# carpedkm/disentangled-subject-to-vid

Measured on AMD Instinct MI355X. Metric: denoise steps/sec (CogVideoX-5B, 49f 720x480; one step = CFG-pair transformer forward + CFG + scheduler step), higher is better.
Workload: dtype bf16

## Files before the change

### disentangled-subject-to-vid_amd/build.py

```python
import hashlib
import os
import subprocess
import sys

HERE = os.path.dirname(os.path.abspath(__file__))
CSRC = os.path.join(HERE, "csrc")
LIB = os.path.join(HERE, "libs2v_hip.so")
SOURCES = ["api.hip", "gemm.hip", "gemm_g4.hip", "gemm_g4t.hip", "gemm_g4f.hip", "gemm_f32m.hip", "attention.hip", "attention_f32m.hip", "attention_q4.hip", "elementwise.hip", "vae.hip", "vae_api.hip", "t5.hip", "rccl.hip", "ulysses.hip"]
FLAGS = ["--offload-arch=gfx950", "-O3", "-std=c++17", "-fPIC", "-fvisibility=hidden", "-Wno-unused-result", "-Wno-unused-value", "-Wno-inline-asm"]
EXTRA = {"attention_q4.hip": ["-fno-slp-vectorize"], "gemm_g4.hip": ["-fno-slp-vectorize"], "gemm_g4t.hip": ["-fno-slp-vectorize"], "gemm_g4f.hip": ["-fno-slp-vectorize"], "elementwise.hip": ["-ffp-contract=off", "-DS2V_TU_FP_CONTRACT_OFF"], "vae.hip": ["-ffp-contract=off", "-DS2V_TU_FP_CONTRACT_OFF"],
         "t5.hip": ["-ffp-contract=off", "-DS2V_TU_FP_CONTRACT_OFF"]}


def _stale(out, deps):
    if not os.path.exists(out):
        return True
    t = os.path.getmtime(out)
    return any(os.path.getmtime(d) > t for d in deps)


def _digest(paths, extra=()):
    h = hashlib.sha256()
    for e in extra:
        h.update(str(e).encode() + b"\0")
    for p in sorted(paths):
        h.update(os.path.basename(p).encode() + b"\0")
        with open(p, "rb") as f:
            h.update(f.read())
    return h.hexdigest()


def _read(path):
    try:
        with open(path) as f:
            return f.read().strip()
    except OSError:
        return None


DIAG_LIB = os.path.join(HERE, "libs2v_hip_diag.so")
GENERATORS = [("gen_attn_q4.py", ["attn_q4_body.inc", "attn_q4h_body.inc", "attn_q4f_body.inc", "attn_q4fh_body.inc", "attn_q4hh_body.inc", "attn_q8_body.inc", "attn_q4_regs.h"]),
              ("gen_gemm_g4.py", ["gemm_g4_body.inc", "gemm_g4_body_f16.inc", "gemm_g4_sk_sum.inc", "gemm_g4_regs.h"]),
              ("gen_gemm_g4t.py", ["gemm_g4t_body_gelu.inc", "gemm_g4t_body_bias.inc", "gemm_g4t_body_qknorm.inc", "gemm_g4t_regs.h"]),
              ("gen_gemm_g4f.py", ["gemm_g4f_body_a3.inc", "gemm_g4f_body_mx.inc", "gemm_g4f_regs.h"])]


def build_library(force=False, verbose=True, diag=False):
    force = force or os.environ.get("S2V_FORCE_BUILD", "0") == "1"
    hipcc = os.environ.get("HIPCC", "/opt/rocm/bin/hipcc")
    objdir = os.path.join(HERE, "build_diag" if diag else "build")
    LIB = DIAG_LIB if diag else globals()["LIB"]
    FLAGS = globals()["FLAGS"] + (["-DS2V_DIAG"] if diag else [])
    gens = GENERATORS
    headers = [os.path.join(CSRC, h) for h in sorted(os.listdir(CSRC)) if h.endswith((".h", ".inc"))]
    headers.append(os.path.join(HERE, "..", "include", "s2v_hip.h"))
    srcs = [os.path.join(CSRC, s) for s in SOURCES if os.path.exists(os.path.join(CSRC, s))]
    gen_srcs = [os.path.join(CSRC, g) for g, _ in gens]
    whole = _digest(srcs + headers + gen_srcs, FLAGS + [f"{k}:{v}" for k, v in sorted(EXTRA.items())])
    if not force and os.path.exists(LIB) and _read(LIB + ".stamp") == whole:
        if verbose:
            print(f"up to date (content hash {whole[:12]}): {LIB}", flush=True)
        return LIB
    os.makedirs(objdir, exist_ok=True)
    for g, outs in gens:
        gp, ops = os.path.join(CSRC, g), [os.path.join(CSRC, o) for o in outs]
        stamp = os.path.join(objdir, g + ".stamp")
        d = _digest([gp])
        missing = [o for o in ops if not os.path.exists(o)]
        if force or missing or (_read(stamp) != d and any(_stale(o, [gp]) for o in ops)):
            if verbose:
                print(f"{sys.executable} {gp}", flush=True)
            subprocess.check_call([sys.executable, gp])
            with open(stamp, "w") as f:
                f.write(d)
    headers = [os.path.join(CSRC, h) for h in sorted(os.listdir(CSRC)) if h.endswith((".h", ".inc"))]
    headers.append(os.path.join(HERE, "..", "include", "s2v_hip.h"))
    whole = _digest(srcs + headers + gen_srcs, FLAGS + [f"{k}:{v}" for k, v in sorted(EXTRA.items())])
    objs = []
    procs = []
    for sp in srcs:
        src = os.path.basename(sp)
        obj = os.path.join(objdir, src.replace(".hip", ".o"))
        objs.append(obj)
        cmd = [hipcc] + FLAGS + EXTRA.get(src, []) + ["-c", sp, "-o", obj]
        d = _digest([sp] + headers, cmd[1:-3])
        if force or not os.path.exists(obj) or _read(obj + ".stamp") != d:
            if verbose:
                print(" ".join(cmd), flush=True)
            procs.append((src, obj, d, subprocess.Popen(cmd)))
    for src, obj, d, p in procs:
        if p.wait() != 0:
            raise RuntimeError(f"hipcc failed on {src}")
        with open(obj + ".stamp", "w") as f:
            f.write(d)
    cmd = [hipcc, "--offload-arch=gfx950", "-shared", "-fPIC", "-o", LIB] + objs
    if verbose:
        print(" ".join(cmd), flush=True)
    subprocess.check_call(cmd)
    with open(LIB + ".stamp", "w") as f:
        f.write(whole)
    if verbose:
        print(f"built {len(procs)} of {len(objs)} translation units, linked {LIB} (content hash {whole[:12]})", flush=True)
    return LIB


if __name__ == "__main__":
    print(build_library(force="--force" in sys.argv, diag="--diag" in sys.argv))
```

### disentangled-subject-to-vid_amd/csrc/api.hip

```cpp
#define S2V_HOST
#include "common.h"
#include "kernels.h"
#include "../../include/s2v_hip.h"

#include <algorithm>
#include <cstdio>
#include <cstring>
#include <string>
#include <unordered_map>
#include <vector>

thread_local std::string g_s2v_err;
int s2v_fail(const char* file, int line, const char* msg, int code) {
    char buf[512];
    snprintf(buf, sizeof(buf), "%s:%d: %s", file, line, msg);
    g_s2v_err = buf;
    return code;
}

static inline int64_t rup(int64_t x, int64_t m) { return (x + m - 1) / m * m; }

struct Slot {
    char* dst = nullptr;
    int64_t rows = 0, cols = 0, ld = 0;
// ... 457 lines not shown
        std::string m = std::string("s2v_weight_slot: unknown tensor name: ") + name;
        return s2v_fail(__FILE__, __LINE__, m.c_str(), -3);
    }
    const Slot& s = it->second;
    *offset_bytes = (int64_t)(s.dst - c->arena);
    *rows = s.rows; *cols = s.cols; *ld = s.ld;
    return 0;
}

extern "C" int s2v_weight_arena(s2v_ctx* c, void** dev_ptr, int64_t* bytes) {
    S2V_REQUIRE(c && dev_ptr && bytes, "s2v_weight_arena: null argument");
    *dev_ptr = c->arena;
    *bytes = c->arena_bytes;
    return 0;
}
extern "C" int s2v_mark_weights_loaded(s2v_ctx* c) {
    S2V_REQUIRE(c, "null context");
    S2V_REQUIRE(c->kind != S2V_CTX_ATTN_WORKSPACE, "s2v_mark_weights_loaded: a workspace context (S2V_CTX_ATTN_WORKSPACE) holds no weights");
    for (auto& kv : c->slots) kv.second.loaded = true;
    c->finalized = true;
    return 0;
}

static inline void shard_range(int n, int p, int r, int* begin, int* len) {
    const int b = (int)((int64_t)r * n / p), e = (int)((int64_t)(r + 1) * n / p);
    *begin = b; *len = e - b;
}

extern "C" int s2v_set_shard(s2v_ctx* c, int32_t world, int32_t rank) {
    S2V_REQUIRE(c, "null context");
    S2V_REQUIRE(c->kind == S2V_CTX_MODEL, "s2v_set_shard: attention-only contexts (S2V_CTX_ATTN_*) are not sharded");
    S2V_REQUIRE(world >= 1 && rank >= 0 && rank < world, "s2v_set_shard: need world >= 1 and 0 <= rank < world");
    S2V_REQUIRE(c->cfg.num_heads % world == 0, "s2v_set_shard: the world size must divide num_heads (attention runs num_heads / world heads per rank)");
    S2V_REQUIRE(c->cfg.weight_format == 0 || (c->D / world) % 128 == 0,
                "s2v_set_shard: fp8 weight formats need an even number of heads per rank, (inner_dim / world) % 128 == 0 (the MX block-scale dwords of "
                "the attention output hold two heads each)");
    S2V_REQUIRE(c->cfg.out_channels * 4 * c->esz % 16 == 0, "s2v_set_shard: the projected rows must be a multiple of 16 bytes (out_channels * 4 * element size)");
    if (c->shard && c->sp == world && c->sr == rank) return 0;
    S2V_CHECK_HIP(hipDeviceSynchronize());
    if (c->gexec) { hipGraphExecDestroy(c->gexec); c->gexec = nullptr; }
    if (c->ws) { hipFree(c->ws); c->ws = nullptr; }
    c->B = 0;
    c->shard = true; c->sp = world; c->sr = rank;
    c->sh_pending = 0;
    return 0;
}

static bool attn_mx_out(const s2v_ctx* c);

extern "C" int s2v_set_geometry(s2v_ctx* c, int32_t B, int32_t T, int32_t F, int32_t H, int32_t W) {
    S2V_REQUIRE(c, "null context");
    S2V_REQUIRE(c->kind != S2V_CTX_ATTN_WEIGHTS, "s2v_set_geometry: an attention-weights context (S2V_CTX_ATTN_WEIGHTS) never carves a workspace");
    S2V_REQUIRE(B >= 1 && B <= 4, "s2v_set_geometry: batch must be 1..4");
    S2V_REQUIRE(T >= 0 && F >= 1 && H >= 2 && W >= 2 && H % 2 == 0 && W % 2 == 0, "s2v_set_geometry: bad geometry");
    if (c->ws && B == c->B && T == c->gT && F == c->F && H == c->H && W == c->W) return 0;
    if (c->shard) S2V_REQUIRE(F * (H / 2) * (W / 2) >= c->sp, "s2v_set_geometry: every rank of a shard needs at least one video row");
    S2V_CHECK_HIP(hipDeviceSynchronize());
    if (c->gexec) { hipGraphExecDestroy(c->gexec); c->gexec = nullptr; }
    if (c->ws) { hipFree(c->ws); c->ws = nullptr; }
    c->B = B; c->T = T; c->F = F; c->H = H; c->W = W;
    c->R = (H / 2) * (W / 2);
    c->V = F * c->R;
    c->Ntok = T + c->R + c->V;
    c->gT = c->T; c->gR = c->R; c->gV = c->V; c->gN = c->Ntok;
    c->t0 = c->r0 = c->v0 = 0;
    if (c->shard) {
        shard_range(c->gT, c->sp, c->sr, &c->t0, &c->T);
        shard_range(c->gR, c->sp, c->sr, &c->r0, &c->R);
        shard_range(c->gV, c->sp, c->sr, &c->v0, &c->V);
        c->Ntok = c->T + c->R + c->V;
    }
    c->Vmax = (c->gV + c->sp - 1) / c->sp;
    c->sh_pending = 0;
    c->fp8_qk = c->cfg.weight_format == 2 || (c->cfg.weight_format == 3 && c->gN >= S2V_FP8_QK_AUTO_TOKENS);
    c->ntok_pad = (int)rup(c->gN, 64);
    c->M = (int64_t)B * c->Ntok;
    c->Mpad = rup(c->M, 256) + 256;
    c->have_rope = c->have_pos = c->have_cond = false;
    c->split_kind = -1;
    const int64_t D = c->D, E = c->esz;
    const int64_t Cin4 = c->cfg.in_channels * 4, Cout4 = c->cfg.out_channels * 4;
    const int64_t BVp = rup((int64_t)B * c->V, 256) + 256;
    const int64_t BVg = rup((int64_t)B * c->gV, 256) + 256;
    int64_t off = 0;
    auto carve = [&](int64_t bytes) { int64_t o = off; off += rup(bytes, 256); return o; };
    const int64_t oX = carve(c->Mpad * D * E), oXn = carve(c->Mpad * D * E), oQKV = carve(c->Mpad * 3 * D * E);
    const int64_t oH = carve(c->Mpad * 4 * D * E);
    const int64_t oVT = carve((int64_t)B * (c->cfg.num_heads / c->sp) * 64 * c->ntok_pad * 2);
    const int64_t oe0 = carve(rup((int64_t)B * T + 128, 128) * D * E), oe1 = carve(rup(c->gR + 128, 128) * D * E);
    const int64_t opat = carve(BVg * Cin4 * E), otail = carve(BVp * D * E), oproj = carve(BVp * Cout4 * E);
    const int64_t omod = carve((int64_t)B * c->mod_rows * E);
    const int64_t ote = carve(((int64_t)B * D + (int64_t)B * c->temb) * E), oemb = carve((int64_t)B * c->temb * E);
    const int64_t onp = carve((int64_t)std::max(B, 2) * F * c->cfg.out_channels * H * W * E);
    const int64_t ocos = carve((int64_t)(c->R + c->V) * 64 * 4), osin = carve((int64_t)(c->R + c->V) * 64 * 4);
    const int64_t opk = carve((int64_t)(c->R + c->V) * 64 * 4);
    const int64_t opos = carve((int64_t)c->V * D * E);
    const int64_t oaq = carve(c->fp8 ? c->Mpad * 4 * D : 0), oaqs = carve(c->fp8 ? c->Mpad * 4 : 0);
    const int64_t ohq = carve(c->fp8 ? c->Mpad * 4 * D : 0), ohs = carve(c->fp8 ? c->Mpad * 4 * D / 32 : 0);
    const int64_t BH = (int64_t)B * (c->cfg.num_heads / c->sp);
    const int64_t oq8 = carve(c->fp8_qk ? BH * c->gN * 64 : 0), oq8s = carve(c->fp8_qk ? BH * c->gN * 2 : 0);
    const int64_t ok8 = carve(c->fp8_qk ? BH * c->ntok_pad * 64 : 0), ok8s = carve(c->fp8_qk ? BH * c->ntok_pad * 4 : 0);
    c->sk_tiles = (!c->shard && c->mfma && ((c->M + 255) / 256) * ((D + 255) / 256) * 2 <= c->num_cus) ? c->num_cus : 0;
    const int64_t osk = carve((int64_t)c->sk_tiles * 262144), oskc = carve((int64_t)c->sk_tiles * 4);
    const int64_t P = c->sp, Dp = D / P, Mg = (int64_t)B * c->gN, Mgpad = rup(Mg, 256) + 256;
    c->o_mx = c->shard && attn_mx_out(c);
    const bool omx = c->o_mx;
    auto o_bytes = [&](int64_t n) { return omx ? n * Dp + rup(n * Dp / 32, 16) : n * Dp * E; };
    const int64_t oQh = carve(c->shard ? Mgpad * 3 * Dp * E : 0), oOh = carve(c->shard ? Mgpad * Dp * E : 0);
    const int64_t osb = carve(c->shard ? std::max(c->M * 3 * D * E, o_bytes(Mg) + 16 * P) : 0);
    const int64_t orb = carve(c->shard ? std::max(Mg * 3 * Dp * E, P * o_bytes(c->M)) : 0);
    const int64_t oOs = carve(omx ? Dp / 128 * Mgpad * 4 : 0), oomap = carve(omx ? 2 * Mg * 4 : 0);
    const int64_t ons = carve(c->shard ? (int64_t)B * c->Vmax * Cout4 * E : 0), onr = carve(c->shard ? P * B * c->Vmax * Cout4 * E : 0);
    const int64_t opf = carve(c->shard ? (int64_t)B * c->gV * Cout4 * E : 0);
    const int64_t ormap = carve(c->shard ? Mg * 4 : 0), onmap = carve(c->shard ? P * B * c->Vmax * 4 : 0);
    c->ws_bytes = off;
    S2V_CHECK_HIP(hipMalloc((void**)&c->ws, c->ws_bytes));
    S2V_CHECK_HIP(hipMemset(c->ws, 0, c->ws_bytes));
    char* w = c->ws;
    c->X = w + oX; c->Xn = w + oXn; c->QKV = w + oQKV; c->Hb = w + oH; c->VT = w + oVT; c->e0 = w + oe0; c->e1 = w + oe1;
    c->patches = w + opat; c->tailn = w + otail; c->proj = w + oproj; c->mod = w + omod; c->tmp_te = w + ote;
    c->emb = w + oemb; c->noise_pred = w + onp; c->rope_cos = (float*)(w + ocos); c->rope_sin = (float*)(w + osin);
    c->pos_tab = w + opos; c->rope_pk = (float*)(w + opk); c->rope_paired = false;
    c->aq = w + oaq; c->aq_scale = (float*)(w + oaqs);
    c->hq = (unsigned char*)(w + ohq); c->hs = (unsigned char*)(w + ohs);
    c->q8 = (unsigned char*)(w + oq8); c->q8s = (unsigned short*)(w + oq8s); c->k8 = (unsigned char*)(w + ok8); c->k8s = (unsigned*)(w + ok8s);
    c->sk_ws = (float*)(w + osk); c->sk_cnt = (unsigned*)(w + oskc);
    if (c->shard) {
        c->QKVh = w + oQh; c->Oh = w + oOh; c->sbuf = w + osb; c->rbuf = w + orb; c->nsend = w + ons; c->nrecv = w + onr; c->proj_full = w + opf;
        c->rmap = (int*)(w + ormap); c->nmap = (int*)(w + onmap);
        c->Os = omx ? (unsigned char*)(w + oOs) : nullptr; c->Os_rows = Mgpad; c->omap = omx ? (int*)(w + oomap) : nullptr;
        std::vector<int> rmap, nmap;
        rmap.reserve(Mg);
        nmap.assign((size_t)P * B * c->Vmax, -1);
        std::vector<int64_t> ntok(P);
        for (int g = 0; g < P; ++g) {
            int ts, tl, rs, rl, vs, vl;
            shard_range(c->gT, (int)P, g, &ts, &tl); shard_range(c->gR, (int)P, g, &rs, &rl); shard_range(c->gV, (int)P, g, &vs, &vl);
            ntok[g] = tl + rl + vl;
            for (int b = 0; b < B; ++b) {
                const int base = b * c->gN;
                for (int i = 0; i < tl; ++i) rmap.push_back(base + ts + i);
                for (int i = 0; i < rl; ++i) rmap.push_back(base + c->gT + rs + i);
                for (int i = 0; i < vl; ++i) rmap.push_back(base + c->gT + c->gR + vs + i);
                for (int i = 0; i < vl; ++i) nmap[((size_t)g * B + b) * c->Vmax + i] = b * c->gV + vs + i;
            }
        }
        S2V_CHECK_HIP(hipMemcpy(c->rmap, rmap.data(), rmap.size() * 4, hipMemcpyHostToDevice));
        S2V_CHECK_HIP(hipMemcpy(c->nmap, nmap.data(), nmap.size() * 4, hipMemcpyHostToDevice));
        for (auto& k : c->xcnt) for (auto& v : k) v.assign(P, 0);
        int64_t rq = 0, so = 0;
        std::vector<int> omap(omx ? 2 * Mg : 0);
        for (int g = 0, i = 0; g < P; ++g) {
            c->xcnt[0][0][g] = c->M * 3 * Dp * E; c->xcnt[0][1][g] = g * c->M * 3 * Dp * E;
            c->xcnt[0][2][g] = B * ntok[g] * 3 * Dp * E; c->xcnt[0][3][g] = rq; rq += c->xcnt[0][2][g];
            const int64_t n = B * ntok[g];
            if (omx)
                for (int64_t j = 0; j < n; ++j, ++i) { omap[i] = (int)((so + j * Dp) / 16); omap[Mg + i] = (int)((so + n * Dp) / 4 + j * (Dp / 128)); }
            c->xcnt[1][0][g] = o_bytes(n); c->xcnt[1][1][g] = so; so += c->xcnt[1][0][g];
            c->xcnt[1][2][g] = o_bytes(c->M); c->xcnt[1][3][g] = g * o_bytes(c->M);
            c->xcnt[2][0][g] = (int64_t)B * c->Vmax * Cout4 * E; c->xcnt[2][1][g] = 0;
            c->xcnt[2][2][g] = c->xcnt[2][0][g]; c->xcnt[2][3][g] = g * c->xcnt[2][0][g];
        }
        if (omx) S2V_CHECK_HIP(hipMemcpy(c->omap, omap.data(), omap.size() * 4, hipMemcpyHostToDevice));
    }
    return 0;
}

extern "C" int s2v_fp8_qk_active(s2v_ctx* c, int32_t* active) {
    S2V_REQUIRE(c && active, "s2v_fp8_qk_active: null argument");
    *active = c->fp8_qk ? 1 : 0;
    return 0;
}

extern "C" int s2v_set_rope(s2v_ctx* c, const float* cos_dev, const float* sin_dev, s2v_stream stream) {
    S2V_REQUIRE(c && c->ws, "s2v_set_rope: call s2v_set_geometry first");
    auto drop_graph = [&]() { if (c->gexec) { hipGraphExecDestroy(c->gexec); c->gexec = nullptr; } };
    if (!cos_dev || !sin_dev) {
        if (c->have_rope) drop_graph();
        c->have_rope = false;
        return 0;
    }
    const bool had_rope = c->have_rope, was_paired = c->rope_paired;
    const size_t bytes = (size_t)(c->R + c->V) * 64 * 4;
    if (c->shard) {
        const size_t row = 64 * 4, rb = (size_t)c->R * row, vb = (size_t)c->V * row;
        const size_t ro = (size_t)c->r0 * row, vo = ((size_t)c->gR + c->v0) * row;
        S2V_CHECK_HIP(hipMemcpyAsync(c->rope_cos, (const char*)cos_dev + ro, rb, hipMemcpyDeviceToDevice, (hipStream_t)stream));
        S2V_CHECK_HIP(hipMemcpyAsync(c->rope_sin, (const char*)sin_dev + ro, rb, hipMemcpyDeviceToDevice, (hipStream_t)stream));
        S2V_CHECK_HIP(hipMemcpyAsync((char*)c->rope_cos + rb, (const char*)cos_dev + vo, vb, hipMemcpyDeviceToDevice, (hipStream_t)stream));
        S2V_CHECK_HIP(hipMemcpyAsync((char*)c->rope_sin + rb, (const char*)sin_dev + vo, vb, hipMemcpyDeviceToDevice, (hipStream_t)stream));
    } else {
        S2V_CHECK_HIP(hipMemcpyAsync(c->rope_cos, cos_dev, bytes, hipMemcpyDeviceToDevice, (hipStream_t)stream));
        S2V_CHECK_HIP(hipMemcpyAsync(c->rope_sin, sin_dev, bytes, hipMemcpyDeviceToDevice, (hipStream_t)stream));
    }
    c->have_rope = true;
    const size_t n = (size_t)(c->R + c->V) * 64;
    std::vector<float> hc(n), hs(n), pk(n);
    S2V_CHECK_HIP(hipStreamSynchronize((hipStream_t)stream));
    S2V_CHECK_HIP(hipMemcpy(hc.data(), c->rope_cos, bytes, hipMemcpyDeviceToHost));
    S2V_CHECK_HIP(hipMemcpy(hs.data(), c->rope_sin, bytes, hipMemcpyDeviceToHost));
    bool paired = true;
    for (size_t i = 0; i < n && paired; i += 2) paired = hc[i] == hc[i + 1] && hs[i] == hs[i + 1];
    c->rope_paired = paired;
    if (!had_rope || was_paired != paired) drop_graph();
    if (paired) {
        for (size_t p = 0; p < n / 64; ++p)
            for (int k = 0; k < 32; ++k) {
                pk[p * 64 + k] = hc[p * 64 + 2 * k];
                pk[p * 64 + 32 + k] = hs[p * 64 + 2 * k];
            }
        S2V_CHECK_HIP(hipMemcpy(c->rope_pk, pk.data(), bytes, hipMemcpyHostToDevice));
    }
    return 0;
}

extern "C" int s2v_set_pos_embed(s2v_ctx* c, const void* table_dev, s2v_stream stream) {
    S2V_REQUIRE(c && c->ws, "s2v_set_pos_embed: call s2v_set_geometry first");
    if (!table_dev) { c->have_pos = false; return 0; }
    S2V_CHECK_HIP(hipMemcpyAsync(c->pos_tab, (const char*)table_dev + (size_t)c->v0 * c->D * c->esz, (size_t)c->V * c->D * c->esz,
                                 hipMemcpyDeviceToDevice, (hipStream_t)stream));
    c->have_pos = true;
    return 0;
}

static int linear(s2v_ctx* c, const GemmArgs& g0, int epi, hipStream_t st) {
    GemmArgs g = g0;
    g.clk = c->clk_cur;
    g.a_rows_padded = (int)(rup(g.M, 256));
    g.w_rows_padded = (int)(rup(g.N, 256));
    if ((c->mfma || c->h16) && g.K % 64 == 0 && g.lda % 8 == 0 && g.ldw % 8 == 0) {
        g.f16 = c->h16 ? 1 : 0;
        const GemmPlan p = gemm_plan(g, epi, c->num_cus, c->sk_tiles);
        g.tile = p.tile;
        if (p.splitk > 1) { g.splitk = p.splitk; g.sk_ws = c->sk_ws; g.sk_cnt = c->sk_cnt; }
        if (p.tail != GEMM_NONE) {
            GemmArgs gm = g, gt = g;
            gt.clk = nullptr;
            gm.M = p.m_main;
            gt.m_begin = p.m_main;
            S2V_CHECK_HIP(hipEventRecord(c->ev_fork, st));
            S2V_CHECK_HIP(hipStreamWaitEvent(c->side, c->ev_fork, 0));
            S2V_TRY(launch_gemm_bf16(gt, epi, c->side));
            S2V_CHECK_HIP(hipEventRecord(c->ev_join, c->side));
            S2V_TRY(launch_gemm_bf16(gm, epi, st));
            S2V_CHECK_HIP(hipStreamWaitEvent(st, c->ev_join, 0));
            return 0;
        }
        return launch_gemm_bf16(g, epi, st);
    }
    g.valu_only = c->cfg.force_simple;
    return launch_gemm_simple(g, epi, c->dtype, st);
}

static int linear_fp8(s2v_ctx* c, const GemmArgs& g0, int epi, const char* wq, const float* wscale, hipStream_t st, bool prequant = false) {
    GemmArgs g = g0;
    g.clk = c->clk_cur;
    g.a_scale = nullptr;
    if (!g.mx_a_s) {
        if (!prequant) S2V_TRY(launch_quant_rows_fp8(g.A, g.lda, g.M, g.K, c->aq, c->aq_scale, st));
        g.A = c->aq; g.a_scale = c->aq_scale;
    }
    g.lda = g.K; g.W = wq; g.ldw = g.K; g.w_scale = wscale;
    g.a_rows_padded = (int)rup(g.M, 256);
    g.w_rows_padded = (int)rup(g.N, 256);
    return launch_gemm_fp8(g, epi, st);
}

extern "C" int s2v_set_conditioning(s2v_ctx* c, const void* text_dev, const void* ref_latent_dev, s2v_stream stream) {
    S2V_REQUIRE(c && c->ws && c->finalized, "s2v_set_conditioning: geometry and weights must be set first");
    S2V_REQUIRE(text_dev && ref_latent_dev, "s2v_set_conditioning: null input");
    hipStream_t st = (hipStream_t)stream;
    const int D = c->D;
    const int TX = c->cfg.text_embed_dim;
    if (c->T > 0) {
        if (c->shard) {
            for (int b = 0; b < c->B; ++b)
                S2V_TRY(launch_convert2d((const char*)text_dev + ((int64_t)b * c->gT + c->t0) * TX * c->esz, c->dtype, TX,
                                         c->Hb + (int64_t)b * c->T * TX * c->esz, c->dtype, TX, c->T, TX, st));
        } else {
            S2V_TRY(launch_convert2d(text_dev, c->dtype, TX, c->Hb, c->dtype, TX, (int64_t)c->B * c->T, TX, st));
        }
        GemmArgs g{};
        g.A = c->Hb; g.lda = TX; g.W = c->text_w; g.ldw = TX; g.bias = c->text_b;
        g.C = c->e0; g.ldc = D; g.M = c->B * c->T; g.N = D; g.K = TX;
        S2V_TRY(linear(c, g, EPI_BIAS, st));
    }
    const int K = c->cfg.in_channels * 4;
    S2V_TRY(launch_patchify(ref_latent_dev, 0, 1, 1, c->cfg.in_channels, c->H, c->W, c->patches, c->dtype, st));
    GemmArgs g{};
    g.A = c->patches + (int64_t)c->r0 * K * c->esz; g.lda = K; g.W = c->patch_w; g.ldw = K; g.bias = c->patch_b;
    g.C = c->e1; g.ldc = D; g.M = c->R; g.N = D; g.K = K;
    if (c->R > 0) S2V_TRY(linear(c, g, EPI_BIAS, st));
    c->have_cond = true;
    return 0;
}

#ifdef S2V_DIAG
static int g_fp8_mx = 1;
extern "C" __attribute__((visibility("default"))) int s2v_set_fp8_mx(int on) { g_fp8_mx = on; return 0; }
static int g_fused_q8 = 1;
extern "C" __attribute__((visibility("default"))) int s2v_set_fused_q8(int on) { g_fused_q8 = on; return 0; }
static int g_fused_qk = 1;
extern "C" __attribute__((visibility("default"))) int s2v_set_fused_qk(int on) { g_fused_qk = on; return 0; }
extern "C" __attribute__((visibility("default"))) int s2v_diag_qkv_qknorm(const void* A, const void* W, const void* bias, const void* nq_w, const void* nq_b,
                                                                           const void* nk_w, const void* nk_b, const float* cs, void* C, int32_t M, int32_t D,
                                                                           int32_t K, int32_t tok_per_batch, int32_t text_len, float eps, s2v_stream stream) {
    S2V_REQUIRE(A && W && bias && C && nq_w && nq_b && nk_w && nk_b, "s2v_diag_qkv_qknorm: null argument");
    GemmArgs g{};
    g.A = A; g.lda = K; g.W = W; g.ldw = K; g.bias = bias; g.C = C; g.ldc = 3 * D; g.M = M; g.N = 3 * D; g.K = K;
    g.a_rows_padded = (int)rup(M, 256); g.w_rows_padded = (int)rup(3 * D, 256);
    g.tok_per_batch = tok_per_batch; g.text_len = text_len;
    g.qk_w[0] = nq_w; g.qk_b[0] = nq_b; g.qk_w[1] = nk_w; g.qk_b[1] = nk_b; g.qk_cs = cs; g.qk_D = D; g.qk_eps = eps;
    return launch_gemm_bf16(g, EPI_BIAS_QKNORM, (hipStream_t)stream);
}
#endif
static bool attn_mx_out(const s2v_ctx* c) {
    bool mx = c->fp8 && c->mfma && c->D % 128 == 0;
#ifdef S2V_DIAG
    mx = mx && g_fp8_mx;
#endif
    return mx;
}
static int run_attention(s2v_ctx* c, const LayerW& w, hipStream_t st, bool prequant = false) {
    const int D = c->D;
    GemmArgs g{};
    g.A = c->Xn; g.lda = D; g.W = w.wqkv; g.ldw = D; g.bias = w.bqkv;
    g.C = c->QKV; g.ldc = 3 * D; g.M = (int)c->M; g.N = 3 * D; g.K = D;
#ifdef S2V_DIAG
    const bool fuse_any = (c->mfma || c->h16) && D % 64 == 0 && (!c->have_rope || c->rope_paired) && g_fused_qk != 0;
    const bool norm_in_quant = fuse_any && c->fp8_qk && g_fused_qk != 3;
#else
    const bool fuse_any = (c->mfma || c->h16) && D % 64 == 0 && (!c->have_rope || c->rope_paired);
    const bool norm_in_quant = fuse_any && c->fp8_qk;
#endif
    const bool fused_qk = fuse_any && !norm_in_quant;
    if (fused_qk) {
        g.tok_per_batch = c->Ntok; g.text_len = c->T;
        g.qk_w[0] = w.nq_w; g.qk_b[0] = w.nq_b; g.qk_w[1] = w.nk_w; g.qk_b[1] = w.nk_b;
        g.qk_cs = c->have_rope ? c->rope_pk : nullptr;
        g.qk_D = D; g.qk_eps = 1e-6f;
    }
    {
        ProfScope ps(c, PK_QKV, st);
        const int epi = fused_qk ? EPI_BIAS_QKNORM : EPI_BIAS;
        if (c->fp8) S2V_TRY(linear_fp8(c, g, epi, w.q_qkv, w.s_qkv, st, prequant));
        else S2V_TRY(linear(c, g, epi, st));
    }
    const bool p16 = c->attn_p16 && c->mfma && (c->fp8_qk || attn_runs_q4(c->Ntok, attn_mx_out(c)));
    if (fused_qk || norm_in_quant) {
        ProfScope ps(c, PK_QKNORM, st);
        S2V_TRY(launch_v_transpose(c->QKV, 3 * D, c->B, c->cfg.num_heads, c->Ntok, c->VT, c->ntok_pad, st, p16));
    } else {
        QkNormRopeArgs q{};
        q.qkv = c->QKV; q.ld_qkv = 3 * D; q.B = c->B; q.H = c->cfg.num_heads; q.Ntok = c->Ntok; q.text_len = c->T;
        q.nq_w = w.nq_w; q.nq_b = w.nq_b; q.nk_w = w.nk_w; q.nk_b = w.nk_b; q.eps = 1e-6f;
        q.cos = c->have_rope ? c->rope_cos : nullptr; q.sin = c->have_rope ? c->rope_sin : nullptr;
        q.vt = (c->mfma || c->h16) ? c->VT : nullptr; q.ntok_pad = c->ntok_pad; q.vt_f16 = p16 ? 1 : 0;
        ProfScope ps(c, PK_QKNORM, st);
        S2V_TRY(launch_qk_norm_rope(q, c->dtype, st));
    }
    AttnArgs a{};
    a.qkv = c->QKV; a.ld_qkv = 3 * D; a.vt = c->VT; a.ntok_pad = c->ntok_pad; a.out = c->Xn; a.ld_out = D;
    a.B = c->B; a.H = c->cfg.num_heads; a.Ntok = c->Ntok; a.scale = 0.125f;
    a.queue = c->attn_queue; a.num_cus = c->num_cus;
    a.p16 = p16 ? 1 : 0;
    a.stats = c->attn_stats;
    a.valu_only = c->cfg.force_simple;
    a.stagger = c->attn_stagger;
    a.order = c->attn_order;
    if (attn_mx_out(c)) { a.mx_q = (unsigned char*)c->aq; a.mx_s = c->hs; a.mx_rows = (int)c->Mpad; }
    if (c->fp8_qk) {
        {
            ProfScope ps(c, PK_QKNORM, st);
            if (norm_in_quant) {
                QkNormRopeArgs q{};
                q.qkv = c->QKV; q.ld_qkv = 3 * D; q.B = c->B; q.H = c->cfg.num_heads; q.Ntok = c->Ntok; q.text_len = c->T; q.ntok_pad = c->ntok_pad;
                q.nq_w = w.nq_w; q.nq_b = w.nq_b; q.nk_w = w.nk_w; q.nk_b = w.nk_b; q.eps = 1e-6f;
                q.cos = c->have_rope ? c->rope_cos : nullptr; q.sin = c->have_rope ? c->rope_sin : nullptr;
                S2V_TRY(launch_qk_norm_quant_mx(q, a.scale * 1.4426950408889634f, c->q8, c->q8s, c->k8, c->k8s, st));
            } else {
                S2V_TRY(launch_qk_quant_mx(c->QKV, 3 * D, c->B, c->cfg.num_heads, c->Ntok, c->ntok_pad, a.scale * 1.4426950408889634f, c->q8, c->q8s, c->k8,
                                           c->k8s, st));
            }
        }
        a.q8 = c->q8; a.q8s = c->q8s; a.k8 = c->k8; a.k8s = c->k8s;
        ProfScope ps(c, PK_ATTN, st);
        a.clk = c->clk_cur;
        return launch_attn_q4f(a, true, st);
    }
    ProfScope ps(c, PK_ATTN, st);
    a.clk = c->clk_cur;
    if (c->mfma) S2V_TRY(launch_attn_bf16(a, st));
    else if (c->h16) S2V_TRY(launch_attn_f16(a, st));
    else S2V_TRY(launch_attn_simple(a, c->dtype, st));
    return 0;
}

static int block_norm(s2v_ctx* c, int l, int half, const char* mod_base , int64_t mod_stride,
                      hipStream_t st, bool* prequant_out) {
    const LayerW& w = c->layers[l];
    const int D = c->D;
    const int64_t E = c->esz;
    const char* mb = mod_base + (int64_t)half * c->mc * D * E;
    LnModArgs n{};
    n.x = c->X; n.ldx = D; n.y = c->Xn; n.ldy = D;
    n.w = half ? w.ln2_w : w.ln1_w; n.b = half ? w.ln2_b : w.ln1_b; n.eps = c->cfg.norm_eps;
    n.shift_vid = mb; n.scale_vid = mb + D * E; n.shift_txt = mb + 3 * D * E; n.scale_txt = mb + 4 * D * E;
    n.mod_stride = (int)mod_stride; n.B = c->B; n.Ntok = c->Ntok; n.text_len = c->T; n.D = D;
    if (c->mc == 9) { n.shift_ref = mb + 6 * D * E; n.scale_ref = mb + 7 * D * E; n.ref_len = c->R; }
    bool prequant = c->fp8;
#ifdef S2V_DIAG
    prequant = prequant && g_fused_q8;
#endif
    if (prequant) { n.q8 = c->aq; n.q8_scale = c->aq_scale; }
    *prequant_out = prequant;
    ProfScope ps(c, PK_LNMOD, st);
    return launch_ln_modulate(n, c->dtype, st);
}

static GemmArgs block_gate(const s2v_ctx* c, int half, const char* mod_base, int64_t mod_stride) {
    const int D = c->D;
    const int64_t E = c->esz;
    const char* mb = mod_base + (int64_t)half * c->mc * D * E;
    GemmArgs g{};
    g.X = c->X; g.ldx = D; g.gate_vid = mb + 2 * D * E; g.gate_txt = mb + 5 * D * E; g.gate_stride = (int)mod_stride;
    g.tok_per_batch = c->Ntok; g.text_len = c->T; g.M = (int)c->M; g.N = D;
    if (c->mc == 9) { g.gate_ref = mb + 8 * D * E; g.ref_len = c->R; }
    return g;
}

static int block_out_proj(s2v_ctx* c, int l, GemmArgs g, hipStream_t st) {
    const LayerW& w = c->layers[l];
    const int D = c->D;
    g.A = c->Xn; g.lda = D; g.W = w.wo; g.ldw = D; g.bias = w.bo; g.K = D;
    if (attn_mx_out(c)) { g.A = c->aq; g.mx_a_s = c->hs; g.mx_rows = (int)c->Mpad; }
    ProfScope ps(c, PK_OUT, st);
    if (c->fp8) return linear_fp8(c, g, EPI_BIAS_GATE_RES, w.q_o, w.s_o, st);
    return linear(c, g, EPI_BIAS_GATE_RES, st);
}

static int block_ff(s2v_ctx* c, int l, GemmArgs g, bool prequant, hipStream_t st) {
    const LayerW& w = c->layers[l];
    const int D = c->D;
    GemmArgs f{};
    f.A = c->Xn; f.lda = D; f.W = w.w1; f.ldw = D; f.bias = w.b1; f.C = c->Hb; f.ldc = 4 * D;
    f.M = (int)c->M; f.N = 4 * D; f.K = D;
    bool mx = c->fp8 && (4 * D) % 128 == 0;
#ifdef S2V_DIAG
    mx = mx && g_fp8_mx;
#endif
    if (mx) { f.mx_out_q = c->hq; f.mx_out_s = c->hs; f.mx_rows = (int)c->Mpad; }
    {
        ProfScope ps(c, PK_FF1, st);
        if (c->fp8) S2V_TRY(linear_fp8(c, f, EPI_BIAS_GELU, w.q_1, w.s_1, st, prequant));
        else S2V_TRY(linear(c, f, EPI_BIAS_GELU, st));
    }
    g.A = c->Hb; g.lda = 4 * D; g.W = w.w2; g.ldw = 4 * D; g.bias = w.b2; g.K = 4 * D;
    if (mx) { g.A = c->hq; g.mx_a_s = c->hs; g.mx_rows = (int)c->Mpad; }
    ProfScope ps(c, PK_FF2, st);
    if (c->fp8) return linear_fp8(c, g, EPI_BIAS_GATE_RES, w.q_2, w.s_2, st);
    return linear(c, g, EPI_BIAS_GATE_RES, st);
}

static int run_block(s2v_ctx* c, int l, const char* mod_base ,
                     int64_t mod_stride, hipStream_t st) {
    for (int half = 0; half < 2; ++half) {
        bool prequant = false;
        S2V_TRY(block_norm(c, l, half, mod_base, mod_stride, st, &prequant));
        const GemmArgs g = block_gate(c, half, mod_base, mod_stride);
        if (half == 0) {
            S2V_TRY(run_attention(c, c->layers[l], st, prequant));
            S2V_TRY(block_out_proj(c, l, g, st));
        } else {
            S2V_TRY(block_ff(c, l, g, prequant, st));
        }
    }
    return 0;
}

static int embed_streams(s2v_ctx* c, const void* latents, int64_t lat_bstride, const float* t_dev, hipStream_t st) {
    const int D = c->D, B = c->B;
    const int64_t E = c->esz;
    S2V_TRY(launch_time_embed(t_dev, B, D, c->te1_w, c->te1_b, c->te2_w, c->te2_b, c->temb, c->tmp_te, c->emb, c->dtype, st));
    {
        ProfScope ps(c, PK_OTHER, st);
        S2V_TRY(launch_mod_gemv(c->emb, B, c->temb, c->mod_w, c->mod_b, c->mod_rows, c->mod, c->dtype, st));
    }
    const int K = c->cfg.in_channels * 4;
    S2V_TRY(launch_patchify(latents, lat_bstride, B, c->F, c->cfg.in_channels, c->H, c->W, c->patches, c->dtype, st));
    for (int b = 0; b < B; ++b) {
        char* xb = c->X + (int64_t)b * c->Ntok * D * E;
        S2V_TRY(launch_copy_rows(c->e0 + (int64_t)b * c->T * D * E, D, nullptr, 0, xb, D, c->T, D, c->dtype, st));
        S2V_TRY(launch_copy_rows(c->e1, D, nullptr, 0, xb + (int64_t)c->T * D * E, D, c->R, D, c->dtype, st));
        char* xv = xb + (int64_t)(c->T + c->R) * D * E;
        GemmArgs g{};
        g.A = c->patches + ((int64_t)b * c->gV + c->v0) * K * E; g.lda = K; g.W = c->patch_w; g.ldw = K; g.bias = c->patch_b;
        g.C = xv; g.ldc = D; g.M = c->V; g.N = D; g.K = K;
        S2V_TRY(linear(c, g, EPI_BIAS, st));
        if (!c->cfg.use_rope) S2V_TRY(launch_copy_rows(xv, D, c->pos_tab, D, xv, D, c->V, D, c->dtype, st));
    }
    return 0;
}

static int tail_proj(s2v_ctx* c, hipStream_t st) {
    const int D = c->D, B = c->B;
    const int64_t E = c->esz;
    const char* mo = c->mod + (int64_t)2 * c->L * c->mc * D * E;
    TailNormArgs t{};
    t.x = c->X; t.ldx = D; t.y = c->tailn; t.ldy = D; t.w1 = c->nf_w; t.b1 = c->nf_b; t.w2 = c->no_w; t.b2 = c->no_b;
    t.eps = c->cfg.norm_eps; t.shift = mo; t.scale = mo + D * E; t.mod_stride = (int)c->mod_rows;
    t.B = B; t.Ntok = c->Ntok; t.row0 = c->T + c->R; t.V = c->V; t.D = D;
    S2V_TRY(launch_tail_norm(t, c->dtype, st));
    const int Co = c->cfg.out_channels * 4;
    GemmArgs g{};
    g.A = c->tailn; g.lda = D; g.W = c->po_w; g.ldw = D; g.bias = c->po_b; g.C = c->proj; g.ldc = Co;
    g.M = B * c->V; g.N = Co; g.K = D;
    return linear(c, g, EPI_BIAS, st);
}

static int forward_impl(s2v_ctx* c, const void* latents, int64_t lat_bstride, const float* t_dev, void* out,
                        hipStream_t st) {
    S2V_REQUIRE(c->ws && c->finalized && c->have_cond, "transformer_forward: geometry, weights and conditioning required");
    S2V_REQUIRE(!c->cfg.use_rope || c->have_rope, "transformer_forward: RoPE tables missing (s2v_set_rope)");
    S2V_REQUIRE(c->cfg.use_rope || c->have_pos, "transformer_forward: sincos table missing (s2v_set_pos_embed)");
    S2V_REQUIRE(!c->shard, "transformer_forward: a shard context (s2v_set_shard) runs the staged step only (s2v_shard_step_* / s2v_denoise_step_ulysses)");
    const int D = c->D;
    const int64_t E = c->esz;
    S2V_TRY(embed_streams(c, latents, lat_bstride, t_dev, st));
    for (int l = 0; l < c->L; ++l)
        S2V_TRY(run_block(c, l, c->mod + (int64_t)(2 * l) * c->mc * D * E, c->mod_rows, st));
    S2V_TRY(tail_proj(c, st));
    const int Co = c->cfg.out_channels * 4;
    S2V_TRY(launch_unpatchify(c->proj, Co, c->V, out, c->B, c->F, c->cfg.out_channels, c->H, c->W, c->dtype, st));
    return 0;
}

extern "C" int s2v_transformer_forward(s2v_ctx* c, const void* latents, int64_t lat_bstride, const float* timesteps_dev,
                                       void* out, s2v_stream stream) {
    S2V_REQUIRE(c && latents && timesteps_dev && out, "s2v_transformer_forward: null argument");
    return forward_impl(c, latents, lat_bstride, timesteps_dev, out, (hipStream_t)stream);
}

extern "C" int s2v_block_forward(s2v_ctx* c, int32_t layer, const void* hidden, const void* enc0, const void* enc1,
                                 const void* temb, void* out_hidden, void* out_enc0, void* out_enc1, s2v_stream stream) {
    S2V_REQUIRE(c && c->ws && c->finalized, "s2v_block_forward: geometry and weights required");
    S2V_REQUIRE(!c->shard, "s2v_block_forward: a shard context (s2v_set_shard) runs the staged step only");
    S2V_REQUIRE(layer >= 0 && layer < c->L, "s2v_block_forward: bad layer");
    S2V_REQUIRE(hidden && enc1 && temb && out_hidden && out_enc1, "s2v_block_forward: null argument");
    hipStream_t st = (hipStream_t)stream;
    const int D = c->D, B = c->B;
    const int64_t E = c->esz;
    const int64_t r0 = (int64_t)(2 * layer) * c->mc * D;
    char* modl = c->mod;
    S2V_TRY(launch_mod_gemv(temb, B, c->temb, c->mod_w + r0 * c->temb * E, c->mod_b + r0 * E, 2 * c->mc * D, modl, c->dtype, st));
    for (int b = 0; b < B; ++b) {
        char* xb = c->X + (int64_t)b * c->Ntok * D * E;
        if (c->T) S2V_TRY(launch_copy_rows((const char*)enc0 + (int64_t)b * c->T * D * E, D, nullptr, 0, xb, D, c->T, D, c->dtype, st));
        S2V_TRY(launch_copy_rows((const char*)enc1 + (int64_t)b * c->R * D * E, D, nullptr, 0, xb + (int64_t)c->T * D * E, D, c->R, D, c->dtype, st));
        S2V_TRY(launch_copy_rows((const char*)hidden + (int64_t)b * c->V * D * E, D, nullptr, 0, xb + (int64_t)(c->T + c->R) * D * E, D, c->V, D, c->dtype, st));
    }
    S2V_TRY(run_block(c, layer, modl, 2 * c->mc * D, st));
    for (int b = 0; b < B; ++b) {
        const char* xb = c->X + (int64_t)b * c->Ntok * D * E;
        if (c->T) S2V_TRY(launch_copy_rows(xb, D, nullptr, 0, (char*)out_enc0 + (int64_t)b * c->T * D * E, D, c->T, D, c->dtype, st));
        S2V_TRY(launch_copy_rows(xb + (int64_t)c->T * D * E, D, nullptr, 0, (char*)out_enc1 + (int64_t)b * c->R * D * E, D, c->R, D, c->dtype, st));
        S2V_TRY(launch_copy_rows(xb + (int64_t)(c->T + c->R) * D * E, D, nullptr, 0, (char*)out_hidden + (int64_t)b * c->V * D * E, D, c->V, D, c->dtype, st));
    }
    return 0;
}

static int attn_forward_impl(s2v_ctx* c, const LayerW& w, const void* hidden, const void* encoder, void* out_hidden, void* out_encoder,
                             hipStream_t st) {
    const int D = c->D, B = c->B, TR = c->T + c->R;
    const int64_t E = c->esz;
    for (int b = 0; b < B; ++b) {
        char* xb = c->Xn + (int64_t)b * c->Ntok * D * E;
        S2V_TRY(launch_copy_rows((const char*)encoder + (int64_t)b * TR * D * E, D, nullptr, 0, xb, D, TR, D, c->dtype, st));
        S2V_TRY(launch_copy_rows((const char*)hidden + (int64_t)b * c->V * D * E, D, nullptr, 0, xb + (int64_t)TR * D * E, D, c->V, D, c->dtype, st));
    }
    S2V_TRY(run_attention(c, w, st));
    GemmArgs g{};
    g.A = c->Xn; g.lda = D; g.W = w.wo; g.ldw = D; g.bias = w.bo; g.C = c->Hb; g.ldc = D; g.M = (int)c->M; g.N = D; g.K = D;
    if (attn_mx_out(c)) { g.A = c->aq; g.mx_a_s = c->hs; g.mx_rows = (int)c->Mpad; }
    if (c->fp8) S2V_TRY(linear_fp8(c, g, EPI_BIAS, w.q_o, w.s_o, st));
    else S2V_TRY(linear(c, g, EPI_BIAS, st));
    for (int b = 0; b < B; ++b) {
        const char* xb = c->Hb + (int64_t)b * c->Ntok * D * E;
        S2V_TRY(launch_copy_rows(xb, D, nullptr, 0, (char*)out_encoder + (int64_t)b * TR * D * E, D, TR, D, c->dtype, st));
        S2V_TRY(launch_copy_rows(xb + (int64_t)TR * D * E, D, nullptr, 0, (char*)out_hidden + (int64_t)b * c->V * D * E, D, c->V, D, c->dtype, st));
    }
    return 0;
}

extern "C" int s2v_attn_forward(s2v_ctx* c, int32_t layer, const void* hidden, const void* encoder, void* out_hidden,
                                void* out_encoder, s2v_stream stream) {
    S2V_REQUIRE(c && c->ws && c->finalized, "s2v_attn_forward: geometry and weights required");
    S2V_REQUIRE(!c->shard, "s2v_attn_forward: a shard context (s2v_set_shard) runs the staged step only");
    S2V_REQUIRE(layer >= 0 && layer < c->L, "s2v_attn_forward: bad layer");
    S2V_REQUIRE(hidden && encoder && out_hidden && out_encoder, "s2v_attn_forward: null argument");
    return attn_forward_impl(c, c->layers[layer], hidden, encoder, out_hidden, out_encoder, (hipStream_t)stream);
}

extern "C" int s2v_attn_forward_with(s2v_ctx* c, const s2v_ctx* wc, int32_t layer, const void* hidden, const void* encoder, void* out_hidden,
                                     void* out_encoder, s2v_stream stream) {
    S2V_REQUIRE(c && wc, "s2v_attn_forward_with: null context");
    S2V_REQUIRE(c->ws, "s2v_attn_forward_with: the workspace context has no geometry (s2v_set_geometry)");
    S2V_REQUIRE(!c->shard && !wc->shard, "s2v_attn_forward_with: a shard context (s2v_set_shard) runs the staged step only");
    S2V_REQUIRE(wc->finalized && wc->kind != S2V_CTX_ATTN_WORKSPACE, "s2v_attn_forward_with: the weights are not loaded (s2v_finalize_weights)");
    S2V_REQUIRE(wc->dtype == c->dtype, "s2v_attn_forward_with: the weights context has another dtype");
    S2V_REQUIRE(wc->cfg.num_heads == c->cfg.num_heads && wc->D == c->D, "s2v_attn_forward_with: the weights context has another num_heads / inner dim");
    S2V_REQUIRE(wc->cfg.weight_format == c->cfg.weight_format, "s2v_attn_forward_with: the weights context has another weight_format");
    S2V_REQUIRE(layer >= 0 && layer < (int)wc->layers.size(), "s2v_attn_forward_with: bad layer");
    S2V_REQUIRE(hidden && encoder && out_hidden && out_encoder, "s2v_attn_forward_with: null argument");
    return attn_forward_impl(c, wc->layers[layer], hidden, encoder, out_hidden, out_encoder, (hipStream_t)stream);
}

// ... 644 lines not shown
```

### disentangled-subject-to-vid_amd/csrc/gemm_epi.h

```cpp
#pragma once
#include "common.h"
#include "kernels.h"
#include <type_traits>

#pragma clang fp contract(off)

template <typename T, int EPI>
__device__ __forceinline__ void epilogue4(const GemmArgs& a, int m, int n, const float v[4]) {
    if (m >= a.M) return;
    const T* bias = (const T*)a.bias;
    float y[4];
#pragma unroll
    for (int i = 0; i < 4; ++i) {
        float bv = (bias && n + i < a.N) ? ET<T>::ld(bias + n + i) : 0.f;
        y[i] = ET<T>::rnd(v[i] + bv);
    }
    if (EPI == EPI_BIAS_GELU) {
#pragma unroll
        for (int i = 0; i < 4; ++i) y[i] = ET<T>::rnd(gelu_tanh_f(y[i]));
    }
    if (EPI == EPI_BIAS_GATE_RES) {
        const int b = m / a.tok_per_batch;
        const int r = m - b * a.tok_per_batch;
        const void* gsel = r < a.text_len ? a.gate_txt : (a.gate_ref != nullptr && r < a.text_len + a.ref_len) ? a.gate_ref : a.gate_vid;
        const T* gate = (const T*)gsel + (size_t)b * a.gate_stride;
        T* x = (T*)a.X + (size_t)m * a.ldx + n;
#pragma unroll
        for (int i = 0; i < 4; ++i) {
            if (n + i < a.N) {
                float t = ET<T>::rnd(ET<T>::ld(gate + n + i) * y[i]);
                ET<T>::st(x + i, ET<T>::ld(x + i) + t);
            }
        }
        return;
    }
    if (EPI == EPI_BIAS_ADD) {
        const T* r = (const T*)a.R + (size_t)m * a.ldr + n;
#pragma unroll
        for (int i = 0; i < 4; ++i)
            if (n + i < a.N) y[i] = y[i] + ET<T>::ld(r + i);
    }
    T* c = (T*)a.C + (size_t)m * a.ldc + n;
    if (n + 3 < a.N && (a.ldc & 3) == 0) {
        if constexpr (std::is_same<T, bf16_t>::value) {
            u32x2 p;
            p.x = pack2bf(y[0], y[1]);
            p.y = pack2bf(y[2], y[3]);
            *(u32x2*)c = p;
        } else if constexpr (std::is_same<T, f16_t>::value) {
            u32x2 p;
            p.x = pack2h(y[0], y[1]);
            p.y = pack2h(y[2], y[3]);
            *(u32x2*)c = p;
        } else {
            *(f32x4*)c = (f32x4){y[0], y[1], y[2], y[3]};
        }
    } else {
#pragma unroll
        for (int i = 0; i < 4; ++i)
            if (n + i < a.N) ET<T>::st(c + i, y[i]);
    }
}

__device__ __forceinline__ float oct_sum(float v) {
    v += __int_as_float(__builtin_amdgcn_update_dpp(0, __float_as_int(v), 0xB1, 0xf, 0xf, true));
    v += __int_as_float(__builtin_amdgcn_update_dpp(0, __float_as_int(v), 0x4E, 0xf, 0xf, true));
    v += __int_as_float(__builtin_amdgcn_update_dpp(0, __float_as_int(v), 0x141, 0xf, 0xf, true));
    return v;
}

__device__ __forceinline__ void load_bias64(const GemmArgs& a, int nw, int hi, u32x2 (&bvec)[8]) {
    const bf16_t* bias = (const bf16_t*)a.bias;
    if (bias && nw + 64 <= a.N) {
#pragma unroll
        for (int q = 0; q < 8; ++q) bvec[q] = *(const u32x2*)(bias + nw + (q >> 2) * 32 + 8 * (q & 3) + 4 * hi);
    } else {
#pragma unroll
        for (int q = 0; q < 8; ++q) {
            const int nl = (q >> 2) * 32 + 8 * (q & 3) + 4 * hi;
            unsigned short t[4] = {0, 0, 0, 0};
#pragma unroll
            for (int e = 0; e < 4; ++e)
                if (bias && nw + nl + e < a.N) t[e] = ((const unsigned short*)bias)[nw + nl + e];
            bvec[q] = u32x2{(unsigned)t[0] | ((unsigned)t[1] << 16), (unsigned)t[2] | ((unsigned)t[3] << 16)};
        }
    }
}

template <typename T16> struct H2;
template <> struct H2<bf16_t> {
    static __device__ __forceinline__ float lo(unsigned w) { return __uint_as_float(w << 16); }
    static __device__ __forceinline__ float hi(unsigned w) { return __uint_as_float(w & 0xffff0000u); }
    static __device__ __forceinline__ unsigned pack(float a, float b) { return pack2bf(a, b); }
    static __device__ __forceinline__ float rnd(float v) { return bf2f(f2bf(v)); }
};
template <> struct H2<f16_t> {
    static __device__ __forceinline__ float lo(unsigned w) { return (float)__builtin_bit_cast(f16x2_t, w)[0]; }
    static __device__ __forceinline__ float hi(unsigned w) { return (float)__builtin_bit_cast(f16x2_t, w)[1]; }
    static __device__ __forceinline__ unsigned pack(float a, float b) { return pack2h(a, b); }
    static __device__ __forceinline__ float rnd(float v) { return (float)(f16_t)v; }
};
template <int EPI, int MB, bool SC = false, int GRP = 4, typename T16 = bf16_t>
__device__ __forceinline__ void epilogue_wave_b(const GemmArgs& a, const f32x16 (&acc)[2][MB], int mw, int nw, char* patch, int lane,
                                                const u32x2 (&bvec)[8]) {
    const int fr = lane & 31, hi = lane >> 5;
    const int c16 = lane & 7;
    const bool qk_head = EPI == EPI_BIAS_QKNORM && nw < 2 * a.qk_D;
    const bool qk_rot = qk_head && a.qk_cs != nullptr;
    float qw[8], qb[8];
    f32x4 rc[2][GRP], rs[2][GRP];
    bool rope[2][GRP];
    auto rot_load = [&](int it0, int buf) {
        const float inv_tok = 1.0f / (float)a.tok_per_batch;
#pragma unroll
        for (int u = 0; u < GRP; ++u) {
            const int m = min(mw + (it0 + u) * 8 + (lane >> 3), a.M - 1);
            int b = (int)((float)m * inv_tok);
            int r = m - b * a.tok_per_batch;
            if (r < 0) r += a.tok_per_batch;
            if (r >= a.tok_per_batch) r -= a.tok_per_batch;
            rope[buf][u] = qk_rot && r >= a.text_len;
            const float* tp = a.qk_cs + (size_t)(rope[buf][u] ? r - a.text_len : 0) * 64 + c16 * 4;
            if (qk_rot) {
                rc[buf][u] = *(const f32x4*)tp;
                rs[buf][u] = *(const f32x4*)(tp + 32);
            }
        }
    };
    if (EPI == EPI_BIAS_QKNORM) {
        const int which = nw >= a.qk_D;
        const u32x4 w4 = *(const u32x4*)((const bf16_t*)a.qk_w[which] + c16 * 8), b4 = *(const u32x4*)((const bf16_t*)a.qk_b[which] + c16 * 8);
#pragma unroll
        for (int e = 0; e < 4; ++e) {
            qw[2 * e] = H2<T16>::lo(w4[e]); qw[2 * e + 1] = H2<T16>::hi(w4[e]);
            qb[2 * e] = H2<T16>::lo(b4[e]); qb[2 * e + 1] = H2<T16>::hi(b4[e]);
        }
        rot_load(0, 0);
    }
    constexpr bool PRE = EPI == EPI_BIAS_ADD && MB == 2;
    u32x4 xpre[PRE ? MB * 4 : 1];
    if (PRE) {
        const int npre = nw + c16 * 8 < a.N ? nw + c16 * 8 : 0;
#pragma unroll
        for (int it = 0; it < MB * 4; ++it)
            xpre[it] = *(const u32x4*)((const bf16_t*)a.R + (size_t)min(mw + it * 8 + (lane >> 3), a.M - 1) * a.ldr + npre);
        __builtin_amdgcn_sched_barrier(0);
    }
    float sa[MB];
#pragma unroll
    for (int j = 0; j < MB; ++j) sa[j] = (SC && a.a_scale) ? a.a_scale[min(mw + j * 32 + fr, a.M - 1)] : 1.f;
#pragma unroll
    for (int i = 0; i < 2; ++i)
#pragma unroll
        for (int rq = 0; rq < 4; ++rq) {
            const int nl = i * 32 + 8 * rq + 4 * hi;
            const u32x2 bq = bvec[i * 4 + rq];
            f32x4 sw = {1.f, 1.f, 1.f, 1.f};
            if (SC) sw = *(const f32x4*)(a.w_scale + nw + nl);
            const float bv[4] = {H2<T16>::lo(bq.x), H2<T16>::hi(bq.x), H2<T16>::lo(bq.y),
                                 H2<T16>::hi(bq.y)};
#pragma unroll
            for (int j = 0; j < MB; ++j) {
                float y[4];
#pragma unroll
                for (int e = 0; e < 4; ++e) y[e] = (SC ? acc[i][j][rq * 4 + e] * (sa[j] * sw[e]) : acc[i][j][rq * 4 + e]) + bv[e];
                const int row = j * 32 + fr;
                u32x2 p;
                p.x = H2<T16>::pack(y[0], y[1]);
                p.y = H2<T16>::pack(y[2], y[3]);
                if (EPI == EPI_BIAS_GELU) {
                    p.x = H2<T16>::pack(gelu_tanh_fast(H2<T16>::lo(p.x)), gelu_tanh_fast(H2<T16>::hi(p.x)));
                    p.y = H2<T16>::pack(gelu_tanh_fast(H2<T16>::lo(p.y)), gelu_tanh_fast(H2<T16>::hi(p.y)));
                }
                *(u32x2*)(patch + row * 128 + ((((nl >> 3) ^ (row & 7))) << 4) + (nl & 4) * 2) = p;
            }
        }
    const int n = nw + c16 * 8;
    const bool n_ok = n < a.N;
    const int nc = n_ok ? n : 0;
#pragma unroll
    for (int it0 = 0; it0 < MB * 4; it0 += GRP) {
        u32x4 v[GRP], g[GRP], xo[GRP];
        int mrow[GRP];
        const int cur = (it0 / GRP) & 1;
        if (EPI == EPI_BIAS_QKNORM && it0 + GRP < MB * 4) rot_load(it0 + GRP, cur ^ 1);
#pragma unroll
        for (int u = 0; u < GRP; ++u) {
            const int row = (it0 + u) * 8 + (lane >> 3);
            mrow[u] = mw + row;
            v[u] = *(const u32x4*)(patch + row * 128 + ((c16 ^ (row & 7)) << 4));
            const int m = min(mrow[u], a.M - 1);
            if (EPI == EPI_BIAS_GATE_RES) {
                const int b = m / a.tok_per_batch;
                const int r = m - b * a.tok_per_batch;
                const void* gsel = r < a.text_len ? a.gate_txt : (a.gate_ref != nullptr && r < a.text_len + a.ref_len) ? a.gate_ref : a.gate_vid;
                g[u] = *(const u32x4*)((const bf16_t*)gsel + (size_t)b * a.gate_stride + nc);
                xo[u] = *(const u32x4*)((const bf16_t*)a.X + (size_t)m * a.ldx + nc);
            } else if (EPI == EPI_BIAS_ADD) {
                if (PRE) xo[u] = xpre[PRE ? it0 + u : 0];
                else xo[u] = *(const u32x4*)((const bf16_t*)a.R + (size_t)m * a.ldr + nc);
            }
        }
#pragma unroll
        for (int u = 0; u < GRP; ++u) {
            u32x4 o = v[u];
            if (EPI == EPI_BIAS_QKNORM && qk_head) {
                float x[8];
#pragma unroll
                for (int e = 0; e < 4; ++e) { x[2 * e] = H2<T16>::lo(v[u][e]); x[2 * e + 1] = H2<T16>::hi(v[u][e]); }
                float s = 0.f;
#pragma unroll
                for (int e = 0; e < 8; ++e) s += x[e];
                s = oct_sum(s);
                const float mean = s * (1.0f / 64.0f);
                float q = 0.f;
#pragma unroll
                for (int e = 0; e < 8; ++e) { const float d = x[e] - mean; q += d * d; }
                q = oct_sum(q);
                const float rstd = 1.0f / sqrtf(q * (1.0f / 64.0f) + a.qk_eps);
#pragma unroll
                for (int e = 0; e < 8; ++e) x[e] = H2<T16>::rnd(((x[e] - mean) * rstd * qw[e] + qb[e]));
                if (rope[cur][u]) {
#pragma unroll
                    for (int e = 0; e < 8; e += 2) {
                        const float x0 = x[e], x1 = x[e + 1];
                        const float cc = rc[cur][u][e >> 1], ss = rs[cur][u][e >> 1];
                        x[e] = H2<T16>::rnd((x0 * cc + (-x1) * ss));
                        x[e + 1] = H2<T16>::rnd((x1 * cc + x0 * ss));
                    }
                }
#pragma unroll
                for (int e = 0; e < 4; ++e) o[e] = H2<T16>::pack(x[2 * e], x[2 * e + 1]);
            }
            if (EPI == EPI_BIAS_GATE_RES) {
#pragma unroll
                for (int e = 0; e < 4; ++e) {
                    const float t0 = H2<T16>::rnd((H2<T16>::lo(g[u][e]) * H2<T16>::lo(v[u][e])));
                    const float t1 = H2<T16>::rnd((H2<T16>::hi(g[u][e]) * H2<T16>::hi(v[u][e])));
                    o[e] = H2<T16>::pack(H2<T16>::lo(xo[u][e]) + t0, H2<T16>::hi(xo[u][e]) + t1);
                }
            } else if (EPI == EPI_BIAS_ADD) {
#pragma unroll
                for (int e = 0; e < 4; ++e)
                    o[e] = H2<T16>::pack(H2<T16>::lo(v[u][e]) + H2<T16>::lo(xo[u][e]),
                                   H2<T16>::hi(v[u][e]) + H2<T16>::hi(xo[u][e]));
            }
            if (EPI == EPI_BIAS_GELU && a.mx_out_q) {
                typedef unsigned short u16x2_t __attribute__((ext_vector_type(2)));
                u16x2_t pm = __builtin_bit_cast(u16x2_t, o[0] & 0x7fff7fffu);
#pragma unroll
                for (int e = 1; e < 4; ++e) pm = __builtin_elementwise_max(pm, __builtin_bit_cast(u16x2_t, o[e] & 0x7fff7fffu));
                int amb = (int)max((unsigned)pm[0], (unsigned)pm[1]) << 16;
                amb = max(amb, __builtin_amdgcn_update_dpp(0, amb, 0xB1, 0xf, 0xf, true));
                amb = max(amb, __builtin_amdgcn_update_dpp(0, amb, 0x4E, 0xf, 0xf, true));
                unsigned eb = (__float_as_uint(__int_as_float(amb) * (1.0f / 448.0f)) + 0x7fffffu) >> 23;
                eb = min(max(eb, 1u), 254u);
                const float bscale = __uint_as_float(eb << 23);
                unsigned w0 = 0, w1 = 0;
                asm volatile("v_cvt_scalef32_pk_fp8_bf16 %0, %1, %2" : "+v"(w0) : "v"(o[0]), "v"(bscale));
                asm volatile("v_cvt_scalef32_pk_fp8_bf16 %0, %1, %2 op_sel:[0,0,1]" : "+v"(w0) : "v"(o[1]), "v"(bscale));
                asm volatile("v_cvt_scalef32_pk_fp8_bf16 %0, %1, %2" : "+v"(w1) : "v"(o[2]), "v"(bscale));
                asm volatile("v_cvt_scalef32_pk_fp8_bf16 %0, %1, %2 op_sel:[0,0,1]" : "+v"(w1) : "v"(o[3]), "v"(bscale));
                const unsigned e2 = eb | ((unsigned)__builtin_amdgcn_update_dpp(0, (int)eb, 0x104, 0xf, 0xf, true) << 8);
                if (mrow[u] < a.M && n_ok) {
                    *(u32x2*)(a.mx_out_q + (size_t)mrow[u] * a.N + n) = u32x2{w0, w1};
                    if (c16 == 0) *(unsigned short*)(a.mx_out_s + ((size_t)(n >> 7) * a.mx_rows + mx_perm_row(mrow[u])) * 4 + ((n >> 5) & 3)) = (unsigned short)e2;
                }
            } else if (mrow[u] < a.M && n_ok) {
                if (EPI == EPI_BIAS_GATE_RES) *(u32x4*)((bf16_t*)a.X + (size_t)mrow[u] * a.ldx + n) = o;
                else *(u32x4*)((bf16_t*)a.C + (size_t)mrow[u] * a.ldc + n) = o;
            }
        }
    }
}
template <int EPI, int MB, bool SC = false, typename T16 = bf16_t>
__device__ __forceinline__ void epilogue_wave(const GemmArgs& a, const f32x16 (&acc)[2][MB], int mw, int nw, char* patch, int lane) {
    u32x2 bvec[8];
    load_bias64(a, nw, lane >> 5, bvec);
    epilogue_wave_b<EPI, MB, SC, 4, T16>(a, acc, mw, nw, patch, lane, bvec);
}
template <int EPI>
__device__ __forceinline__ void epilogue_wave64(const GemmArgs& a, const f32x16 (&acc)[2][2], int mw, int nw, char* patch,
                                                int lane) {
    epilogue_wave<EPI, 2>(a, acc, mw, nw, patch, lane);
}
__host__ __device__ __forceinline__ bool epi_vec_ok(const GemmArgs& a, int epi) {
    if ((a.N & 7) != 0) return false;
    if (epi == EPI_BIAS_GATE_RES) return (a.ldx & 7) == 0 && (a.gate_stride & 7) == 0;
    if (epi == EPI_BIAS_ADD && (a.ldr & 7) != 0) return false;
    return (a.ldc & 7) == 0;
}


#ifdef S2V_TU_FP_CONTRACT_OFF
#pragma clang fp contract(off)
#else
#pragma clang fp contract(fast)
#endif
```

### disentangled-subject-to-vid_amd/csrc/gemm_g4.hip

```cpp
#define S2V_HOST
#include "common.h"
#include "kernels.h"
#include "gemm_epi.h"
#include "epi_dispatch.h"
#include "gemm_g4_regs.h"
#include <cstdlib>
#include <type_traits>

typedef __attribute__((ext_vector_type(32))) float f32x32;
typedef __attribute__((ext_vector_type(16))) unsigned int u32x16;
typedef __attribute__((ext_vector_type(8))) unsigned int u32x8;

#ifdef S2V_DIAG
__device__ unsigned long long g_g4_dbg[8];
extern "C" __attribute__((visibility("default"))) int s2v_g4_debug_read(unsigned long long* out, int reset) {
    if (hipMemcpyFromSymbol(out, HIP_SYMBOL(g_g4_dbg), sizeof(g_g4_dbg)) != hipSuccess) return -1;
    if (reset) {
        const unsigned long long z[8] = {0, 0, 0, 0, 0, 0, 0, 0};
        if (hipMemcpyToSymbol(HIP_SYMBOL(g_g4_dbg), z, sizeof(z)) != hipSuccess) return -1;
    }
    return 0;
}
#define G4_STAMP(i) const long long g4_t##i = (long long)__builtin_amdgcn_s_memtime()
#else
#define G4_STAMP(i) do { } while (0)
#endif

template <int EPI, typename T16 = bf16_t>
__global__ __launch_bounds__(256, 1) void gemm_g4(const GemmArgs a, int tiles_m, int tiles_n) {
    extern __shared__ __attribute__((aligned(16))) char smem[];
    const int tid = threadIdx.x, lane = tid & 63;
    clk_stamp(a.clk, gridDim.x >> 1, 0);
    G4_STAMP(0);
#ifdef S2V_DIAG
    const long long g4_r0 = (long long)__builtin_amdgcn_s_memrealtime();
#endif
    const int wave = __builtin_amdgcn_readfirstlane(tid >> 6);
    const int wm = wave >> 1, wn = wave & 1;
    const int fr = lane & 31, hi = lane >> 5;

    const int nwg = gridDim.x, bid = blockIdx.x;
    const int q = nwg >> 3, r = nwg & 7, xcd = bid & 7, idx = bid >> 3;
    const int wg_all = (xcd < r ? xcd * (q + 1) : r * (q + 1) + (xcd - r) * q) + idx;
    const int S = a.splitk > 1 ? a.splitk : 1, ntile = tiles_m * tiles_n;
    const int z = wg_all / ntile, wg = wg_all - z * ntile;
    const int Ks = a.K / S;
    const int GM = a.gm > 0 ? a.gm : 4;
    const int per_group = GM * tiles_n;
    const int group = wg / per_group;
    const int first_m = group * GM;
    const int gsz = min(tiles_m - first_m, GM);
    const int in_g = wg - group * per_group;
    const int m0 = (first_m + in_g % gsz) * 256, n0 = (in_g / gsz) * 256;

    const unsigned lds0 = __builtin_amdgcn_readfirstlane(lds_base_u32(smem));
    u32x16 vaddr, voff;
#pragma unroll
    for (int g = 0; g < 2; ++g)
#pragma unroll
        for (int s = 0; s < 4; ++s) {
            const unsigned inrow = (unsigned)(((s * 2 + hi) ^ ((fr >> 1) & 7)) << 4);
            vaddr[4 * g + s] = lds0 + g * G4_A_STRIDE + (wm * 128 + fr) * 128 + inrow;
            vaddr[8 + 4 * g + s] = lds0 + G4_W_BASE + g * G4_W_STRIDE + (wn * 128 + fr) * 128 + inrow;
        }
    const int srow = wave * 8 + (lane >> 3);
    const int scol = ((lane & 7) ^ ((srow >> 1) & 7)) * 8;
#pragma unroll
    for (int p = 0; p < 8; ++p) {
        voff[p] = (unsigned)(2 * ((int64_t)(srow + p * 32) * a.lda + scol));
        voff[8 + p] = (unsigned)(2 * ((int64_t)(srow + p * 32) * a.ldw + scol));
    }
    u32x2 vpf;
    vpf[0] = (unsigned)(2 * (int64_t)((lane & 7) * 32 + srow) * a.lda);
    vpf[1] = (unsigned)(2 * (int64_t)((lane & 7) * 32 + srow) * a.ldw);
    const unsigned long long ap = (unsigned long long)((const char*)a.A + 2 * ((int64_t)m0 * a.lda + (int64_t)z * Ks));
    const unsigned long long wp = (unsigned long long)((const char*)a.W + 2 * ((int64_t)n0 * a.ldw + (int64_t)z * Ks));
    u32x4 ptr;
    ptr[0] = (unsigned)__builtin_amdgcn_readfirstlane((int)(unsigned)ap);
    ptr[1] = (unsigned)__builtin_amdgcn_readfirstlane((int)(unsigned)(ap >> 32));
    ptr[2] = (unsigned)__builtin_amdgcn_readfirstlane((int)(unsigned)wp);
    ptr[3] = (unsigned)__builtin_amdgcn_readfirstlane((int)(unsigned)(wp >> 32));
    u32x2 sin = {lds0 + wave * 1024, (unsigned)((Ks / 64 - 2 - (G4_PF > 2 ? G4_PF : 2)) / 2)};

    const int tile = (m0 >> 8) * tiles_n + (n0 >> 8);
    const unsigned long long ub = (unsigned long long)(a.sk_ws + ((size_t)tile * S * 4 + wave) * 16384), zb = ub + (unsigned long long)z * 262144;
    const unsigned voff16 = lane * 16;
    u32x4 sk;
    sk[0] = (unsigned)__builtin_amdgcn_readfirstlane((int)(unsigned)zb);
    sk[1] = (unsigned)__builtin_amdgcn_readfirstlane((int)(unsigned)(zb >> 32));
    sk[2] = (unsigned)__builtin_amdgcn_readfirstlane(S);
    sk[3] = 0;

    G4_STAMP(1);
    f32x32 AC[8];
    if constexpr (std::is_same<T16, f16_t>::value) {
        asm volatile(
#include "gemm_g4_body_f16.inc"
            : "=" G4_ACC0(AC[0]), "=" G4_ACC1(AC[1]), "=" G4_ACC2(AC[2]), "=" G4_ACC3(AC[3]), "=" G4_ACC4(AC[4]), "=" G4_ACC5(AC[5]),
              "=" G4_ACC6(AC[6]), "=" G4_ACC7(AC[7]), "+" G4_PTR(ptr), "+" G4_SIN(sin), "+" G4_VADDR(vaddr)
            : G4_VOFF(voff), G4_VPF(vpf), G4_SK(sk), G4_VSK(voff16)
            : G4_CLOBBERS);
    } else {
        asm volatile(
#include "gemm_g4_body.inc"
            : "=" G4_ACC0(AC[0]), "=" G4_ACC1(AC[1]), "=" G4_ACC2(AC[2]), "=" G4_ACC3(AC[3]), "=" G4_ACC4(AC[4]), "=" G4_ACC5(AC[5]),
              "=" G4_ACC6(AC[6]), "=" G4_ACC7(AC[7]), "+" G4_PTR(ptr), "+" G4_SIN(sin), "+" G4_VADDR(vaddr)
            : G4_VOFF(voff), G4_VPF(vpf), G4_SK(sk), G4_VSK(voff16)
            : G4_CLOBBERS);
    }
    G4_STAMP(2);
    __builtin_amdgcn_s_barrier();

    if (S > 1) {
        __syncthreads();
        unsigned* flag = (unsigned*)smem;
        if (tid == 0) *flag = __hip_atomic_fetch_add(a.sk_cnt + tile, 1u, __ATOMIC_RELAXED, __HIP_MEMORY_SCOPE_AGENT);
        __syncthreads();
        if (*flag != (unsigned)(S - 1)) return;
        __syncthreads();
        if (tid == 0) __hip_atomic_store(a.sk_cnt + tile, 0u, __ATOMIC_RELAXED, __HIP_MEMORY_SCOPE_AGENT);
        {
            const unsigned lo = (unsigned)__builtin_amdgcn_readfirstlane((int)(unsigned)ub), hi = (unsigned)__builtin_amdgcn_readfirstlane((int)(unsigned)(ub >> 32));
            const unsigned ns = (unsigned)__builtin_amdgcn_readfirstlane(S), zs = (unsigned)__builtin_amdgcn_readfirstlane(z);
            asm volatile(
#include "gemm_g4_sk_sum.inc"
                : "+" G4_ACC0(AC[0]), "+" G4_ACC1(AC[1]), "+" G4_ACC2(AC[2]), "+" G4_ACC3(AC[3]), "+" G4_ACC4(AC[4]), "+" G4_ACC5(AC[5]),
                  "+" G4_ACC6(AC[6]), "+" G4_ACC7(AC[7])
                : [lo] "s"(lo), [hi] "s"(hi), [voff] "v"(voff16), [ns] "s"(ns), [z] "s"(zs)
                : G4_SK_CLOBBERS);
        }
    }

    char* patch = smem + wave * 16384;
#pragma unroll
    for (int h = 0; h < 2; ++h) {
        f32x16 acc[2][4];
#pragma unroll
        for (int i = 0; i < 2; ++i)
#pragma unroll
            for (int j = 0; j < 4; ++j)
#pragma unroll
                for (int e = 0; e < 16; ++e) acc[i][j][e] = AC[2 * (2 * h + i) + (j >> 1)][(j & 1) * 16 + e];
        epilogue_wave<EPI, 4, false, T16>(a, acc, m0 + wm * 128, n0 + wn * 128 + h * 64, patch, lane);
    }
#ifdef S2V_DIAG
    asm volatile("s_waitcnt vmcnt(0)" ::: "memory");
    G4_STAMP(3);
    if (tid == 0) {
        atomicAdd(&g_g4_dbg[0], (unsigned long long)(g4_t1 - g4_t0));
        atomicAdd(&g_g4_dbg[1], (unsigned long long)(g4_t2 - g4_t1));
        atomicAdd(&g_g4_dbg[2], (unsigned long long)(g4_t3 - g4_t2));
        atomicAdd(&g_g4_dbg[3], 1ull);
        if (blockIdx.x == 100) {
            g_g4_dbg[4] = (unsigned long long)(g4_t3 - g4_t0);
            g_g4_dbg[5] = (unsigned long long)((long long)__builtin_amdgcn_s_memrealtime() - g4_r0);
        }
    }
#endif
    clk_stamp(a.clk, gridDim.x >> 1, 1);
}

template <int EPI, typename T16 = bf16_t>
static int launch_g4_t(const GemmArgs& a_in, hipStream_t st) {
    GemmArgs a = a_in;
    const int tiles_m = (a.M + 255) / 256, tiles_n = (a.N + 255) / 256;
    if (a.gm <= 0) {
        a.gm = (tiles_n <= 16 && tiles_m >= 32 && a.K >= 8192) ? 1 : 4;
#ifdef S2V_DIAG
        if (const char* e = getenv("S2V_G4_GM")) a.gm = atoi(e);
#endif
    }
    const void* fn = (const void*)gemm_g4<EPI, T16>;
    S2V_TRY(ensure_lds_attr(fn, G4_LDS_BYTES));
    void* args[] = {(void*)&a, (void*)&tiles_m, (void*)&tiles_n};
    const int S = a.splitk > 1 ? a.splitk : 1;
    S2V_REQUIRE(S == 1 || (a.sk_ws && a.sk_cnt), "gemm_g4: split K needs the partial workspace and the arrival counters");
    S2V_CHECK_HIP(hipLaunchKernel(fn, dim3(tiles_m * tiles_n * S), dim3(256), args, G4_LDS_BYTES, st));
    return 0;
}

bool gemm_g4_ok(const GemmArgs& a, int epi) {
    const int S = a.splitk > 1 ? a.splitk : 1;
    const int nT = a.K / S / 64;
    return !a.conv && a.K % (128 * S) == 0 && nT >= (G4_PF > 2 ? G4_PF : 2) + 2 && a.lda % 8 == 0 && a.ldw % 8 == 0 && epi_vec_ok(a, epi) && a.m_begin == 0 &&
           a.a_rows_padded >= ((a.M + 255) / 256) * 256;
}
int gemm_choose_splitk(int64_t tiles, int K, int64_t ncu) {
    if (tiles * 2 > ncu) return 1;
    int S = (int)(ncu / tiles < 4 ? ncu / tiles : 4);
    while (S > 1 && !(K % (128 * S) == 0 && K / (64 * S) >= 16)) --S;
    return S;
}
int launch_gemm_g4(const GemmArgs& a, int epi, hipStream_t st) {
    return epi_dispatch16<EPI_BIAS, EPI_BIAS_GELU, EPI_BIAS_GATE_RES, EPI_BIAS_ADD, EPI_BIAS_QKNORM>(
        epi, a.f16, "gemm_g4: bad epilogue", [&](auto e, auto t) { return launch_g4_t<decltype(e)::value, decltype(t)>(a, st); });
}
```

### disentangled-subject-to-vid_amd/csrc/gemm_g4_regs.h

```cpp
#pragma once
#define G4_PF 0
#define G4_LDS_BYTES 163840
#define G4_A_STRIDE 32768
#define G4_W_BASE 98304
#define G4_W_STRIDE 32768
#define G4_ACC0 "{a[0:31]}"
#define G4_ACC1 "{a[32:63]}"
#define G4_ACC2 "{a[64:95]}"
#define G4_ACC3 "{a[96:127]}"
#define G4_ACC4 "{a[128:159]}"
#define G4_ACC5 "{a[160:191]}"
#define G4_ACC6 "{a[192:223]}"
#define G4_ACC7 "{a[224:255]}"
#define G4_VADDR "{v[64:79]}"
#define G4_VOFF "{v[80:95]}"
#define G4_VPF "{v[96:97]}"
#define G4_PTR "{s[36:39]}"
#define G4_SIN "{s[40:41]}"
#define G4_SK "{s[44:47]}"
#define G4_VSK "{v98}"
#define G4_SK_CLOBBERS "v100", "v101", "v102", "v103", "v104", "v105", "v106", "v107", "v108", "v109", "v110", "v111", "v112", "v113", "v114", "v115", "v116", "v117", "v118", "v119", "v120", "v121", "v122", "v123", "v124", "v125", "v126", "v127", "v128", "v129", "v130", "v131", "v132", "v133", "v134", "v135", "v136", "v137", "v138", "v139", "v140", "v141", "v142", "v143", "v144", "v145", "v146", "v147", "v148", "v149", "v150", "v151", "v152", "v153", "v154", "v155", "v156", "v157", "v158", "v159", "v160", "v161", "v162", "v163", "v164", "v165", "v166", "v167", "v168", "v169", "v170", "v171", "v172", "v173", "v174", "v175", "v176", "v177", "v178", "v179", "v180", "v181", "v182", "v183", "v184", "v185", "v186", "v187", "v188", "v189", "v190", "v191", "v192", "v193", "v194", "v195", "v196", "v197", "v198", "v199", "v200", "v201", "v202", "v203", "v204", "v205", "v206", "v207", "v208", "v209", "v210", "v211", "v212", "v213", "v214", "v215", "v216", "v217", "v218", "v219", "v220", "v221", "v222", "v223", "v224", "v225", "v226", "v227", "s50", "s51", "scc", "memory"
#define G4_CLOBBERS "v0", "v1", "v2", "v3", "v4", "v5", "v6", "v7", "v8", "v9", "v10", "v11", "v12", "v13", "v14", "v15", "v16", "v17", "v18", "v19", "v20", "v21", "v22", "v23", "v24", "v25", "v26", "v27", "v28", "v29", "v30", "v31", "v32", "v33", "v34", "v35", "v36", "v37", "v38", "v39", "v40", "v41", "v42", "v43", "v44", "v45", "v46", "v47", "v48", "v49", "v50", "v51", "v52", "v53", "v54", "v55", "v56", "v57", "v58", "v59", "v60", "v61", "v62", "v63", "v98", "v99", "v100", "v101", "v102", "v103", "s42", "s43", "s48", "s50", "s51", "vcc", "scc", "m0", "memory"
```

### disentangled-subject-to-vid_amd/csrc/gen_gemm_g4.py

```python
#!/usr/bin/env python3
import os

ACC, FRAG, VADDR, VOFF, VPF, VPFD = 0, 0, 64, 80, 96, 98
S_A, S_W, S_M0W, S_CNT = 36, 38, 40, 41
ABLATE = set(filter(None, os.environ.get("G4_ABLATE", "").split(",")))
STAGE = os.environ.get("G4_STAGE", "dma")
VREG, VWR = 100, 228
W3 = os.environ.get("G4_W3", "0") == "1"
A3 = os.environ.get("G4_A3", "1") == "1" and os.environ.get("G4_W3", "0") != "1" and os.environ.get("G4_STAGE", "dma") == "dma"
assert not (A3 and W3)
S_WNEXT, S_WDMA, S_WM0, WBASE = 42, 43, 48, 100
A_STRIDE, W_BASE, W_STRIDE = (32768, 65536, 32768) if W3 else (32768, 98304, 32768) if A3 else (65536, 32768, 65536)
A_POL = (" " + os.environ["G4_A_POL"]) if os.environ.get("G4_A_POL") else ""
W_POL = (" " + os.environ["G4_W_POL"]) if os.environ.get("G4_W_POL") else ""
PF = int(os.environ.get("G4_PF", "0"))


def vr(b, n=1):
    return f"v{b}" if n == 1 else f"v[{b}:{b + n - 1}]"


def ar(b, n):
    return f"a[{b}:{b + n - 1}]"


def wf(buf, i):
    return FRAG + 32 * buf + 4 * i


def af(buf, j):
    return FRAG + 32 * buf + 16 + 4 * j


def vaddr(is_w, g, s):
    return VADDR + (8 if is_w else 0) + 4 * g + s


def ktile(emit, g, first=False, dma_w=True, dma_a=True, last=False, prefetch=False):
    if A3:
        return ktile_a3(emit, g, first, dma_w, dma_a, last)
    for s in range(4):
        cur, nxt = s & 1, (s & 1) ^ 1
        if s == 3 and not last:
            emit(f"s_waitcnt vmcnt({8 if (W3 and dma_w) else 2 if (prefetch and PF) else 0}) lgkmcnt(0)")
            emit("s_barrier")
        else:
            emit("s_waitcnt lgkmcnt(0)")
        if W3 and s == 0 and dma_w:
            emit(f"s_add_u32 s{S_WM0}, s{S_M0W}, s{S_WDMA}")
        for k in range(16):
            i, j = k >> 2, k & 3
            acc = ar(ACC + 64 * i + 16 * j, 16)
            c = "0" if (first and s == 0) else acc
            emit(f"v_mfma_f32_32x32x16_bf16 {acc}, {vr(wf(cur, i), 4)}, {vr(af(cur, j), 4)}, {c}")
            if k < 8 and not (last and s == 3):
                gs, ss = (g, s + 1) if s < 3 else (g ^ 1, 0)
                if k < 4:
                    emit(f"ds_read_b128 {vr(wf(nxt, k), 4)}, {vr(vaddr(True, gs, ss))} offset:{k * 4096}")
                else:
                    emit(f"ds_read_b128 {vr(af(nxt, k - 4), 4)}, {vr(vaddr(False, gs, ss))} offset:{(k - 4) * 4096}")
            p = k >> 1
            if s == 0 and dma_w:
                if k & 1 == 0:
                    if W3:
                        emit(f"s_add_u32 m0, s{S_WM0}, {W_BASE + p * 4096}")
                    else:
                        emit(f"s_add_u32 m0, s{S_M0W}, {(g ^ 1) * 65536 + 32768 + p * 4096}")
                else:
                    emit(f"global_load_lds_dwordx4 {vr(VOFF + 8 + p)}, s[{S_W}:{S_W + 1}]{W_POL}")
            if W3 and s == 1 and not last and k >= 12:
                emit(f"v_add_u32 {vr(vaddr(True, g ^ 1, k - 12))}, s{S_WNEXT}, {vr(WBASE + k - 12)}")
            if s == 3 and dma_a:
                if k & 1 == 0:
                    emit(f"s_add_u32 m0, s{S_M0W}, {g * A_STRIDE + p * 4096}")
                else:
                    emit(f"global_load_lds_dwordx4 {vr(VOFF + p)}, s[{S_A}:{S_A + 1}]{A_POL}")
            if s == 1 and prefetch and PF:
                if k == 3:
                    emit(f"global_load_dword {vr(VPFD)}, {vr(VPF)}, s[{S_A}:{S_A + 1}] offset:{(PF - 2) * 128}")
                if k == 11:
                    emit(f"global_load_dword {vr(VPFD + 1)}, {vr(VPF + 1)}, s[{S_W}:{S_W + 1}] offset:{(PF - 2) * 128}")
        if s == 0 and dma_w:
            emit(f"s_add_u32 s{S_W}, s{S_W}, 128")
            emit(f"s_addc_u32 s{S_W + 1}, s{S_W + 1}, 0")
        if W3 and s == 1 and not last:
            emit(f"s_mov_b32 s{S_WNEXT}, s{S_WDMA}")
            emit(f"s_add_u32 s{S_WDMA}, s{S_WDMA}, {W_STRIDE}")
            emit(f"s_cmp_ge_u32 s{S_WDMA}, {3 * W_STRIDE}")
            emit(f"s_cselect_b32 s{S_WDMA}, 0, s{S_WDMA}")
        if s == 3 and dma_a:
            emit(f"s_add_u32 s{S_A}, s{S_A}, 128")
            emit(f"s_addc_u32 s{S_A + 1}, s{S_A + 1}, 0")


def ktile_a3(emit, g, first, dma_w, dma_a, last):
    for s in range(4):
        cur, nxt = s & 1, (s & 1) ^ 1
        if s == 3 and not last:
            emit(f"s_waitcnt vmcnt({8 if dma_a else 0}) lgkmcnt(0)")
            emit("s_barrier")
        else:
            emit("s_waitcnt lgkmcnt(0)")
        if s == 0 and dma_a:
            emit(f"s_add_u32 s{S_WM0}, s{S_M0W}, s{S_WDMA}")
        for k in range(16):
            i, j = k >> 2, k & 3
            acc = ar(ACC + 64 * i + 16 * j, 16)
            c = "0" if (first and s == 0) else acc
            emit(f"v_mfma_f32_32x32x16_bf16 {acc}, {vr(wf(cur, i), 4)}, {vr(af(cur, j), 4)}, {c}")
            if k < 8 and not (last and s == 3):
                gs, ss = (g, s + 1) if s < 3 else (g ^ 1, 0)
                if k < 4:
                    emit(f"ds_read_b128 {vr(wf(nxt, k), 4)}, {vr(vaddr(True, gs, ss))} offset:{k * 4096}")
                else:
                    emit(f"ds_read_b128 {vr(af(nxt, k - 4), 4)}, {vr(vaddr(False, gs, ss))} offset:{(k - 4) * 4096}")
            p = k >> 1
            if s == 0 and dma_a:
                if k & 1 == 0:
                    emit(f"s_add_u32 m0, s{S_WM0}, {p * 4096}")
                else:
                    emit(f"global_load_lds_dwordx4 {vr(VOFF + p)}, s[{S_A}:{S_A + 1}]{A_POL}")
            if s == 1 and not last and k >= 12:
                emit(f"v_add_u32 {vr(vaddr(False, g ^ 1, k - 12))}, s{S_WNEXT}, {vr(WBASE + k - 12)}")
            if s == 3 and dma_w:
                if k & 1 == 0:
                    emit(f"s_add_u32 m0, s{S_M0W}, {W_BASE + g * W_STRIDE + p * 4096}")
                else:
                    emit(f"global_load_lds_dwordx4 {vr(VOFF + 8 + p)}, s[{S_W}:{S_W + 1}]{W_POL}")
        if s == 0 and dma_a:
            emit(f"s_add_u32 s{S_A}, s{S_A}, 128")
            emit(f"s_addc_u32 s{S_A + 1}, s{S_A + 1}, 0")
        if s == 1 and not last:
            emit(f"s_mov_b32 s{S_WNEXT}, s{S_WDMA}")
            emit(f"s_add_u32 s{S_WDMA}, s{S_WDMA}, {A_STRIDE}")
            emit(f"s_cmp_ge_u32 s{S_WDMA}, {3 * A_STRIDE}")
            emit(f"s_cselect_b32 s{S_WDMA}, 0, s{S_WDMA}")
        if s == 3 and dma_w:
            emit(f"s_add_u32 s{S_W}, s{S_W}, 128")
            emit(f"s_addc_u32 s{S_W + 1}, s{S_W + 1}, 0")


REGV = int(os.environ.get("G4_REGV", "0"))


def ktile_reg(emit, g, first=False, loads=True, writes=True, last=False):
    wsteps = (1, 2) if REGV >= 2 else (2,)
    for s in range(4):
        cur, nxt = s & 1, (s & 1) ^ 1
        if s == 3 and not last:
            emit("s_waitcnt lgkmcnt(0)")
            emit("s_barrier")
        elif s == wsteps[0] and writes:
            newer = 0 if not loads else (16 if REGV == 0 else 8 * s)
            emit(f"s_waitcnt vmcnt({newer}) lgkmcnt(0)")
        else:
            emit("s_waitcnt lgkmcnt(0)")
        for k in range(16):
            i, j = k >> 2, k & 3
            acc = ar(ACC + 64 * i + 16 * j, 16)
            c = "0" if (first and s == 0) else acc
            emit(f"v_mfma_f32_32x32x16_bf16 {acc}, {vr(wf(cur, i), 4)}, {vr(af(cur, j), 4)}, {c}")
            if k < 8 and not (last and s == 3):
                gs, ss = (g, s + 1) if s < 3 else (g ^ 1, 0)
                if k < 4:
                    emit(f"ds_read_b128 {vr(wf(nxt, k), 4)}, {vr(vaddr(True, gs, ss))} offset:{k * 4096}")
                else:
                    emit(f"ds_read_b128 {vr(af(nxt, k - 4), 4)}, {vr(vaddr(False, gs, ss))} offset:{(k - 4) * 4096}")
            pl = k if (REGV == 0 and s == 0) else (s * 8 + (k >> 1) if (REGV >= 1 and s < 2 and (k & 1)) else -1)
            if loads and pl >= 0:
                src = f"{vr(VOFF + pl)}, s[{S_A}:{S_A + 1}]" if pl < 8 else f"{vr(VOFF + pl)}, s[{S_W}:{S_W + 1}]"
                emit(f"global_load_dwordx4 {vr(VREG + 64 * g + 4 * pl, 4)}, {src}")
            pw = k if (REGV < 2 and s == 2) else ((s - 1) * 8 + (k >> 1) if (REGV >= 2 and s in (1, 2) and not (k & 1)) else -1)
            if writes and pw >= 0:
                off = pw * 4096 if pw < 8 else 32768 + (pw - 8) * 4096
                emit(f"ds_write_b128 {vr(VWR + (g ^ 1))}, {vr(VREG + 64 * (g ^ 1) + 4 * pw, 4)} offset:{off}")
        if loads and s == (0 if REGV == 0 else 1):
            for sp in (S_A, S_W):
                emit(f"s_add_u32 s{sp}, s{sp}, 128")
                emit(f"s_addc_u32 s{sp + 1}, s{sp + 1}, 0")


def gen_reg():
    L = []

    def emit(ln):
        op = ln.split()[0]
        if "nodma" in ABLATE and op in ("global_load_dwordx4", "ds_write_b128"):
            return
        if ("noload" in ABLATE and op == "global_load_dwordx4") or ("nowrite" in ABLATE and op == "ds_write_b128"):
            return
        if "noread" in ABLATE and op == "ds_read_b128":
            return
        if "nobar" in ABLATE and op == "s_barrier":
            return
        L.append(ln)

    emit("; ---- gemm_g4 K loop, register-staged operands (generated by gen_gemm_g4.py; do not edit)")
    emit(f"v_add_u32 {vr(VWR)}, s{S_M0W}, {vr(V_SK)}")
    emit(f"v_add_u32 {vr(VWR + 1)}, 0x10000, {vr(VWR)}")
    for t in range(2):
        for k in range(16):
            src = f"{vr(VOFF + k)}, s[{S_A}:{S_A + 1}]" if k < 8 else f"{vr(VOFF + k)}, s[{S_W}:{S_W + 1}]"
            emit(f"global_load_dwordx4 {vr(VREG + 64 * t + 4 * k, 4)}, {src}")
        for sp in (S_A, S_W):
            emit(f"s_add_u32 s{sp}, s{sp}, 128")
            emit(f"s_addc_u32 s{sp + 1}, s{sp + 1}, 0")
    emit("s_waitcnt vmcnt(16)")
    for k in range(16):
        off = k * 4096 if k < 8 else 32768 + (k - 8) * 4096
        emit(f"ds_write_b128 {vr(VWR)}, {vr(VREG + 4 * k, 4)} offset:{off}")
    emit("s_waitcnt lgkmcnt(0)")
    emit("s_barrier")
    for n in range(8):
        if n < 4:
            emit(f"ds_read_b128 {vr(wf(0, n), 4)}, {vr(vaddr(True, 0, 0))} offset:{n * 4096}")
        else:
            emit(f"ds_read_b128 {vr(af(0, n - 4), 4)}, {vr(vaddr(False, 0, 0))} offset:{(n - 4) * 4096}")
    ktile_reg(emit, 0, first=True)
    emit("L_g4_loop_%=:")
    emit(f"s_cmp_eq_u32 s{S_CNT}, 0")
    emit("s_cbranch_scc1 L_g4_nopf_%=")
    ktile_reg(emit, 1)
    ktile_reg(emit, 0)
    emit(f"s_sub_u32 s{S_CNT}, s{S_CNT}, 1")
    emit("s_branch L_g4_loop_%=")
    emit("L_g4_nopf_%=:")
    ktile_reg(emit, 1)
    ktile_reg(emit, 0, loads=False)
    ktile_reg(emit, 1, loads=False, writes=False, last=True)
    emit("s_nop 15")
    emit("s_nop 15")
    emit(f"s_cmp_lt_u32 s{S_SK + 2}, 2")
    emit("s_cbranch_scc1 L_g4_end_%=")
    for ln in gen_sk_store(f"s{S_SK}", f"s{S_SK + 1}", f"v{V_SK}"):
        emit(ln)
    emit("L_g4_end_%=:")
    return L


def gen():
    L = []

    def emit(ln):
        op = ln.split()[0]
        if "nodma" in ABLATE and op == "global_load_lds_dwordx4":
            return
        if "noread" in ABLATE and op == "ds_read_b128":
            return
        if "nobar" in ABLATE and op == "s_barrier":
            return
        L.append(ln)

    emit("; ---- gemm_g4 K loop (generated by gen_gemm_g4.py; do not edit)")
    if A3:
        return gen_a3(emit, L)
    for p in range(8):
        emit(f"s_add_u32 m0, s{S_M0W}, {p * 4096}")
        emit("s_nop 0")
        emit(f"global_load_lds_dwordx4 {vr(VOFF + p)}, s[{S_A}:{S_A + 1}]")
    for p in range(8):
        emit(f"s_add_u32 m0, s{S_M0W}, {W_BASE + p * 4096}")
        emit("s_nop 0")
        emit(f"global_load_lds_dwordx4 {vr(VOFF + 8 + p)}, s[{S_W}:{S_W + 1}]")
    emit(f"s_add_u32 s{S_A}, s{S_A}, 128")
    emit(f"s_addc_u32 s{S_A + 1}, s{S_A + 1}, 0")
    emit(f"s_add_u32 s{S_W}, s{S_W}, 128")
    emit(f"s_addc_u32 s{S_W + 1}, s{S_W + 1}, 0")
    for p in range(8):
        emit(f"s_add_u32 m0, s{S_M0W}, {A_STRIDE + p * 4096}")
        emit("s_nop 0")
        emit(f"global_load_lds_dwordx4 {vr(VOFF + p)}, s[{S_A}:{S_A + 1}]")
    emit(f"s_add_u32 s{S_A}, s{S_A}, 128")
    emit(f"s_addc_u32 s{S_A + 1}, s{S_A + 1}, 0")
    if W3:
        assert PF == 0
        for p in range(8):
            emit(f"s_add_u32 m0, s{S_M0W}, {W_BASE + W_STRIDE + p * 4096}")
            emit("s_nop 0")
            emit(f"global_load_lds_dwordx4 {vr(VOFF + 8 + p)}, s[{S_W}:{S_W + 1}]")
        emit(f"s_add_u32 s{S_W}, s{S_W}, 128")
        emit(f"s_addc_u32 s{S_W + 1}, s{S_W + 1}, 0")
        emit(f"s_mov_b32 s{S_WNEXT}, {W_STRIDE}")
        emit(f"s_mov_b32 s{S_WDMA}, {2 * W_STRIDE}")
        for x in range(4):
            emit(f"v_mov_b32 {vr(WBASE + x)}, {vr(vaddr(True, 0, x))}")
    for k in range(2, PF):
        emit(f"global_load_dword {vr(VPFD)}, {vr(VPF)}, s[{S_A}:{S_A + 1}] offset:{(k - 2) * 128}")
        emit(f"global_load_dword {vr(VPFD + 1)}, {vr(VPF + 1)}, s[{S_W}:{S_W + 1}] offset:{(k - 1) * 128}")
    emit(f"s_waitcnt vmcnt({16 if W3 else 8 + 2 * max(0, PF - 2)})")
    emit("s_barrier")
    for n in range(8):
        if n < 4:
            emit(f"ds_read_b128 {vr(wf(0, n), 4)}, {vr(vaddr(True, 0, 0))} offset:{n * 4096}")
        else:
            emit(f"ds_read_b128 {vr(af(0, n - 4), 4)}, {vr(vaddr(False, 0, 0))} offset:{(n - 4) * 4096}")
    emit("; K-tile 0")
    ktile(emit, 0, first=True, prefetch=True)
    emit("L_g4_loop_%=:")
    emit(f"s_cmp_eq_u32 s{S_CNT}, 0")
    emit("s_cbranch_scc1 L_g4_nopf_%=")
    ktile(emit, 1, prefetch=True)
    ktile(emit, 0, prefetch=True)
    emit(f"s_sub_u32 s{S_CNT}, s{S_CNT}, 1")
    emit("s_branch L_g4_loop_%=")
    emit("L_g4_nopf_%=:")
    for _ in range(max(0, PF // 2 - 1)):
        ktile(emit, 1)
        ktile(emit, 0)
    ktile(emit, 1)
    ktile(emit, 0, dma_a=False, dma_w=not W3)
    ktile(emit, 1, dma_w=False, dma_a=False, last=True)
    emit("s_waitcnt vmcnt(0)")
    emit("s_nop 15")
    emit("s_nop 15")
    emit(f"s_cmp_lt_u32 s{S_SK + 2}, 2")
    emit("s_cbranch_scc1 L_g4_end_%=")
    for ln in gen_sk_store(f"s{S_SK}", f"s{S_SK + 1}", f"v{V_SK}"):
        emit(ln)
    emit("L_g4_end_%=:")
    return L


def gen_a3(emit, L):
    assert PF == 0
    for t in range(2):
        for p in range(8):
            emit(f"s_add_u32 m0, s{S_M0W}, {t * A_STRIDE + p * 4096}")
            emit("s_nop 0")
            emit(f"global_load_lds_dwordx4 {vr(VOFF + p)}, s[{S_A}:{S_A + 1}]")
        for p in range(8):
            emit(f"s_add_u32 m0, s{S_M0W}, {W_BASE + t * W_STRIDE + p * 4096}")
            emit("s_nop 0")
            emit(f"global_load_lds_dwordx4 {vr(VOFF + 8 + p)}, s[{S_W}:{S_W + 1}]")
        for sp in (S_A, S_W):
            emit(f"s_add_u32 s{sp}, s{sp}, 128")
            emit(f"s_addc_u32 s{sp + 1}, s{sp + 1}, 0")
    emit(f"s_mov_b32 s{S_WNEXT}, {A_STRIDE}")
    emit(f"s_mov_b32 s{S_WDMA}, {2 * A_STRIDE}")
    for x in range(4):
        emit(f"v_mov_b32 {vr(WBASE + x)}, {vr(vaddr(False, 0, x))}")
    emit("s_waitcnt vmcnt(16)")
    emit("s_barrier")
    for n in range(8):
        if n < 4:
            emit(f"ds_read_b128 {vr(wf(0, n), 4)}, {vr(vaddr(True, 0, 0))} offset:{n * 4096}")
        else:
            emit(f"ds_read_b128 {vr(af(0, n - 4), 4)}, {vr(vaddr(False, 0, 0))} offset:{(n - 4) * 4096}")
    emit("; K-tile 0")
    ktile(emit, 0, first=True)
    emit("L_g4_loop_%=:")
    emit(f"s_cmp_eq_u32 s{S_CNT}, 0")
    emit("s_cbranch_scc1 L_g4_nopf_%=")
    ktile(emit, 1)
    ktile(emit, 0)
    emit(f"s_sub_u32 s{S_CNT}, s{S_CNT}, 1")
    emit("s_branch L_g4_loop_%=")
    emit("L_g4_nopf_%=:")
    ktile(emit, 1)
    ktile(emit, 0, dma_a=False, dma_w=False)
    ktile(emit, 1, dma_w=False, dma_a=False, last=True)
    emit("s_waitcnt vmcnt(0)")
    emit("s_nop 15")
    emit("s_nop 15")
    emit(f"s_cmp_lt_u32 s{S_SK + 2}, 2")
    emit("s_cbranch_scc1 L_g4_end_%=")
    for ln in gen_sk_store(f"s{S_SK}", f"s{S_SK + 1}", f"v{V_SK}"):
        emit(ln)
    emit("L_g4_end_%=:")
    return L


SK_S0, SK_V0, SK_ZSTRIDE = 50, 100, 262144


S_SK, V_SK = 44, 98


def gen_sk_store(lo, hi, voff):
    out = []
    for k in range(8):
        out.append(f"s_add_u32 s{SK_S0}, {lo}, {k * 8192 + 4096}")
        out.append(f"s_addc_u32 s{SK_S0 + 1}, {hi}, 0")
        for g in range(8):
            out.append(f"global_store_dwordx4 {voff}, a[{32 * k + 4 * g}:{32 * k + 4 * g + 3}], s[{SK_S0}:{SK_S0 + 1}] offset:{g * 1024 - 4096} sc1")
    out.append("s_waitcnt vmcnt(0)")
    return out


def gen_sk_sum():
    out = []
    for k in range(8):
        out.append(f"s_add_u32 s{SK_S0}, %[lo], {k * 8192 + 4096}")
        out.append(f"s_addc_u32 s{SK_S0 + 1}, %[hi], 0")
        for zz in range(4):
            if zz >= 2:
                out.append(f"s_cmp_lt_u32 %[ns], {zz + 1}")
                out.append(f"s_cbranch_scc1 L_sk_w{k}_%=")
            if zz:
                out.append(f"s_add_u32 s{SK_S0}, s{SK_S0}, {SK_ZSTRIDE}")
                out.append(f"s_addc_u32 s{SK_S0 + 1}, s{SK_S0 + 1}, 0")
            out.append(f"s_cmp_eq_u32 %[z], {zz}")
            out.append(f"s_cbranch_scc1 L_sk_o{k}_{zz}_%=")
            for g in range(8):
                v = SK_V0 + 32 * zz + 4 * g
                out.append(f"global_load_dwordx4 v[{v}:{v + 3}], %[voff], s[{SK_S0}:{SK_S0 + 1}] offset:{g * 1024 - 4096} sc1")
            out.append(f"s_branch L_sk_n{k}_{zz}_%=")
            out.append(f"L_sk_o{k}_{zz}_%=:")
            for i in range(32):
                out.append(f"v_accvgpr_read_b32 v{SK_V0 + 32 * zz + i}, a{32 * k + i}")
            out.append(f"L_sk_n{k}_{zz}_%=:")
        out.append(f"L_sk_w{k}_%=:")
        out.append("s_waitcnt vmcnt(0)")
        for zz in range(1, 4):
            if zz >= 2:
                out.append(f"s_cmp_lt_u32 %[ns], {zz + 1}")
                out.append(f"s_cbranch_scc1 L_sk_d{k}_%=")
            for i in range(32):
                out.append(f"v_add_f32 v{SK_V0 + i}, v{SK_V0 + i}, v{SK_V0 + 32 * zz + i}")
        out.append(f"L_sk_d{k}_%=:")
        for i in range(32):
            out.append(f"v_accvgpr_write_b32 a{32 * k + i}, v{SK_V0 + i}")
    return out


def main():
    here = os.environ.get("S2V_GEN_OUT") or os.path.dirname(os.path.abspath(__file__))
    body = gen_reg() if STAGE == "reg" else gen()
    with open(os.path.join(here, "gemm_g4_body.inc"), "w") as f:
        for ln in body:
            f.write('"' + ln + '\\n\\t"\n')
    with open(os.path.join(here, "gemm_g4_body_f16.inc"), "w") as f:
        for ln in body:
            f.write('"' + ln.replace("v_mfma_f32_32x32x16_bf16", "v_mfma_f32_32x32x16_f16") + '\\n\\t"\n')
    for name, body in (("gemm_g4_sk_sum.inc", gen_sk_sum()),):
        with open(os.path.join(here, name), "w") as f:
            for ln in body:
                f.write('"' + ln + '\\n\\t"\n')
    clob = [f"v{r}" for r in range(0, 64)] + ([f"v{r}" for r in range(VREG, VWR + 2)] if STAGE == "reg" else [f"v{VPFD}", f"v{VPFD + 1}"])
    if W3 or A3:
        clob += [f"v{WBASE + x}" for x in range(4)] + [f"s{S_WNEXT}", f"s{S_WDMA}", f"s{S_WM0}"]
    with open(os.path.join(here, "gemm_g4_regs.h"), "w") as f:
        f.write("// generated by gen_gemm_g4.py: the physical registers the K loop of gemm_g4 owns, and its LDS size\n#pragma once\n")
        f.write(f"#define G4_PF {PF}\n#define G4_LDS_BYTES {163840 if (W3 or A3) else 131072}\n")
        f.write(f"#define G4_A_STRIDE {A_STRIDE}\n#define G4_W_BASE {W_BASE}\n#define G4_W_STRIDE {W_STRIDE}  // LDS map of the operand stages: A stage g at g * A_STRIDE, W stage h at W_BASE + h * W_STRIDE\n")
        for k in range(8):
            f.write(f'#define G4_ACC{k} "{{a[{32 * k}:{32 * k + 31}]}}"\n')
        f.write(f'#define G4_VADDR "{{v[{VADDR}:{VADDR + 15}]}}"\n#define G4_VOFF "{{v[{VOFF}:{VOFF + 15}]}}"\n#define G4_VPF "{{v[{VPF}:{VPF + 1}]}}"\n')
        f.write(f'#define G4_PTR "{{s[{S_A}:{S_A + 3}]}}"\n#define G4_SIN "{{s[{S_M0W}:{S_M0W + 1}]}}"\n')
        f.write(f'#define G4_SK "{{s[{S_SK}:{S_SK + 3}]}}"\n#define G4_VSK "{{v{V_SK}}}"\n')
        f.write("#define G4_SK_CLOBBERS " + ", ".join(f'"v{r}"' for r in range(SK_V0, SK_V0 + 128)) + f', "s{SK_S0}", "s{SK_S0 + 1}", "scc", "memory"\n')
        f.write("#define G4_CLOBBERS " + ", ".join(f'"{c}"' for c in clob) + f', "s{SK_S0}", "s{SK_S0 + 1}", "vcc", "scc", "m0", "memory"\n')


if __name__ == "__main__":
    main()
```

Measured before the change: 1.552.

## Add 16x16x32 MFMA variant of the g4 GEMM main loop

```diff
diff --git a/disentangled-subject-to-vid_amd/build.py b/disentangled-subject-to-vid_amd/build.py
--- a/disentangled-subject-to-vid_amd/build.py
+++ b/disentangled-subject-to-vid_amd/build.py
@@ -40,7 +40,7 @@
 
 DIAG_LIB = os.path.join(HERE, "libs2v_hip_diag.so")
 GENERATORS = [("gen_attn_q4.py", ["attn_q4_body.inc", "attn_q4h_body.inc", "attn_q4f_body.inc", "attn_q4fh_body.inc", "attn_q4hh_body.inc", "attn_q8_body.inc", "attn_q4_regs.h"]),
-              ("gen_gemm_g4.py", ["gemm_g4_body.inc", "gemm_g4_body_f16.inc", "gemm_g4_sk_sum.inc", "gemm_g4_regs.h"]),
+              ("gen_gemm_g4.py", ["gemm_g4_body.inc", "gemm_g4_body_f16.inc", "gemm_g4_body_m16.inc", "gemm_g4_sk_sum.inc", "gemm_g4_regs.h"]),
               ("gen_gemm_g4t.py", ["gemm_g4t_body_gelu.inc", "gemm_g4t_body_bias.inc", "gemm_g4t_body_qknorm.inc", "gemm_g4t_regs.h"]),
               ("gen_gemm_g4f.py", ["gemm_g4f_body_a3.inc", "gemm_g4f_body_mx.inc", "gemm_g4f_regs.h"])]
 
diff --git a/disentangled-subject-to-vid_amd/csrc/api.hip b/disentangled-subject-to-vid_amd/csrc/api.hip
--- a/disentangled-subject-to-vid_amd/csrc/api.hip
+++ b/disentangled-subject-to-vid_amd/csrc/api.hip
@@ -783,6 +783,8 @@
 extern "C" __attribute__((visibility("default"))) int s2v_set_fused_q8(int on) { g_fused_q8 = on; return 0; }
 static int g_fused_qk = 1;
 extern "C" __attribute__((visibility("default"))) int s2v_set_fused_qk(int on) { g_fused_qk = on; return 0; }
+static int g_diag_qkv_f16 = 0;
+extern "C" __attribute__((visibility("default"))) int s2v_set_diag_qkv_f16(int on) { g_diag_qkv_f16 = on ? 1 : 0; return 0; }
 extern "C" __attribute__((visibility("default"))) int s2v_diag_qkv_qknorm(const void* A, const void* W, const void* bias, const void* nq_w, const void* nq_b,
                                                                            const void* nk_w, const void* nk_b, const float* cs, void* C, int32_t M, int32_t D,
                                                                            int32_t K, int32_t tok_per_batch, int32_t text_len, float eps, s2v_stream stream) {
@@ -792,7 +794,27 @@
     g.a_rows_padded = (int)rup(M, 256); g.w_rows_padded = (int)rup(3 * D, 256);
     g.tok_per_batch = tok_per_batch; g.text_len = text_len;
     g.qk_w[0] = nq_w; g.qk_b[0] = nq_b; g.qk_w[1] = nk_w; g.qk_b[1] = nk_b; g.qk_cs = cs; g.qk_D = D; g.qk_eps = eps;
+    g.f16 = g_diag_qkv_f16;
     return launch_gemm_bf16(g, EPI_BIAS_QKNORM, (hipStream_t)stream);
+}
+extern "C" __attribute__((visibility("default"))) int s2v_diag_linear_epi(const void* A, const void* W, const void* bias, void* C, void* X, const void* gates,
+                                                                           int32_t M, int32_t N, int32_t K, int32_t epi, int32_t dtype, int32_t tok_per_batch,
+                                                                           int32_t text_len, s2v_stream stream) {
+    S2V_REQUIRE(A && W && bias && (dtype == S2V_DTYPE_BF16 || dtype == S2V_DTYPE_F16), "s2v_diag_linear_epi: null argument or not a 16-bit dtype");
+    S2V_REQUIRE(epi == EPI_BIAS || epi == EPI_BIAS_GELU || epi == EPI_BIAS_GATE_RES || epi == EPI_BIAS_ADD, "s2v_diag_linear_epi: epilogue");
+    GemmArgs g{};
+    g.A = A; g.lda = K; g.W = W; g.ldw = K; g.bias = bias; g.C = C; g.ldc = N; g.M = M; g.N = N; g.K = K;
+    g.a_rows_padded = (int)rup(M, 256); g.w_rows_padded = (int)rup(N, 256);
+    if (epi == EPI_BIAS_GATE_RES) {
+        S2V_REQUIRE(X && gates && tok_per_batch > 0, "s2v_diag_linear_epi: the gated residual needs X, the gates and the tokens per sample");
+        const int B = (M + tok_per_batch - 1) / tok_per_batch;
+        g.X = X; g.ldx = N; g.gate_txt = gates; g.gate_vid = (const char*)gates + (size_t)B * N * 2; g.gate_stride = N;
+        g.tok_per_batch = tok_per_batch; g.text_len = text_len;
+    } else {
+        S2V_REQUIRE(C, "s2v_diag_linear_epi: null output");
+        if (epi == EPI_BIAS_ADD) { S2V_REQUIRE(X, "s2v_diag_linear_epi: the residual add needs X"); g.R = X; g.ldr = N; }
+    }
+    return dtype == S2V_DTYPE_F16 ? launch_gemm_f16(g, epi, (hipStream_t)stream) : launch_gemm_bf16(g, epi, (hipStream_t)stream);
 }
 #endif
 static bool attn_mx_out(const s2v_ctx* c) {
diff --git a/disentangled-subject-to-vid_amd/csrc/gemm_epi.h b/disentangled-subject-to-vid_amd/csrc/gemm_epi.h
--- a/disentangled-subject-to-vid_amd/csrc/gemm_epi.h
+++ b/disentangled-subject-to-vid_amd/csrc/gemm_epi.h
@@ -87,6 +87,39 @@
     }
 }
 
+template <int BLK> struct AccMap;
+template <> struct AccMap<32> {
+    typedef f32x16 blk_t;
+    static constexpr int NI = 2, NQ = 4, NV = 8;
+    static __device__ __forceinline__ int row(int lane) { return lane & 31; }
+    static __device__ __forceinline__ int col(int rq, int lane) { return 8 * rq + 4 * (lane >> 5); }
+};
+template <> struct AccMap<16> {
+    typedef f32x4 blk_t;
+    static constexpr int NI = 4, NQ = 1, NV = 4;
+    static __device__ __forceinline__ int row(int lane) { return lane & 15; }
+    static __device__ __forceinline__ int col(int, int lane) { return 4 * (lane >> 4); }
+};
+template <int BLK>
+__device__ __forceinline__ void load_bias64_m(const GemmArgs& a, int nw, int lane, u32x2 (&bvec)[AccMap<BLK>::NV]) {
+    typedef AccMap<BLK> MP;
+    const bf16_t* bias = (const bf16_t*)a.bias;
+    if (bias && nw + 64 <= a.N) {
+#pragma unroll
+        for (int q = 0; q < MP::NV; ++q) bvec[q] = *(const u32x2*)(bias + nw + (q / MP::NQ) * BLK + MP::col(q % MP::NQ, lane));
+    } else {
+#pragma unroll
+        for (int q = 0; q < MP::NV; ++q) {
+            const int nl = (q / MP::NQ) * BLK + MP::col(q % MP::NQ, lane);
+            unsigned short t[4] = {0, 0, 0, 0};
+#pragma unroll
+            for (int e = 0; e < 4; ++e)
+                if (bias && nw + nl + e < a.N) t[e] = ((const unsigned short*)bias)[nw + nl + e];
+            bvec[q] = u32x2{(unsigned)t[0] | ((unsigned)t[1] << 16), (unsigned)t[2] | ((unsigned)t[3] << 16)};
+        }
+    }
+}
+
 template <typename T16> struct H2;
 template <> struct H2<bf16_t> {
     static __device__ __forceinline__ float lo(unsigned w) { return __uint_as_float(w << 16); }
@@ -100,10 +133,12 @@
     static __device__ __forceinline__ unsigned pack(float a, float b) { return pack2h(a, b); }
     static __device__ __forceinline__ float rnd(float v) { return (float)(f16_t)v; }
 };
-template <int EPI, int MB, bool SC = false, int GRP = 4, typename T16 = bf16_t>
-__device__ __forceinline__ void epilogue_wave_b(const GemmArgs& a, const f32x16 (&acc)[2][MB], int mw, int nw, char* patch, int lane,
-                                                const u32x2 (&bvec)[8]) {
-    const int fr = lane & 31, hi = lane >> 5;
+template <int EPI, int MB, bool SC, int GRP, typename T16, int BLK>
+__device__ __forceinline__ void epilogue_wave_m(const GemmArgs& a, const typename AccMap<BLK>::blk_t (&acc)[AccMap<BLK>::NI][MB * 32 / BLK], int mw, int nw,
+                                                char* patch, int lane, const u32x2 (&bvec)[AccMap<BLK>::NV]) {
+    typedef AccMap<BLK> MP;
+    constexpr int NJ = MB * 32 / BLK;
+    const int fr = MP::row(lane);
     const int c16 = lane & 7;
     const bool qk_head = EPI == EPI_BIAS_QKNORM && nw < 2 * a.qk_D;
     const bool qk_rot = qk_head && a.qk_cs != nullptr;
@@ -146,25 +181,25 @@
             xpre[it] = *(const u32x4*)((const bf16_t*)a.R + (size_t)min(mw + it * 8 + (lane >> 3), a.M - 1) * a.ldr + npre);
         __builtin_amdgcn_sched_barrier(0);
     }
-    float sa[MB];
-#pragma unroll
-    for (int j = 0; j < MB; ++j) sa[j] = (SC && a.a_scale) ? a.a_scale[min(mw + j * 32 + fr, a.M - 1)] : 1.f;
-#pragma unroll
-    for (int i = 0; i < 2; ++i)
-#pragma unroll
-        for (int rq = 0; rq < 4; ++rq) {
-            const int nl = i * 32 + 8 * rq + 4 * hi;
-            const u32x2 bq = bvec[i * 4 + rq];
+    float sa[NJ];
+#pragma unroll
+    for (int j = 0; j < NJ; ++j) sa[j] = (SC && a.a_scale) ? a.a_scale[min(mw + j * BLK + fr, a.M - 1)] : 1.f;
+#pragma unroll
+    for (int i = 0; i < MP::NI; ++i)
+#pragma unroll
+        for (int rq = 0; rq < MP::NQ; ++rq) {
+            const int nl = i * BLK + MP::col(rq, lane);
+            const u32x2 bq = bvec[i * MP::NQ + rq];
             f32x4 sw = {1.f, 1.f, 1.f, 1.f};
             if (SC) sw = *(const f32x4*)(a.w_scale + nw + nl);
             const float bv[4] = {H2<T16>::lo(bq.x), H2<T16>::hi(bq.x), H2<T16>::lo(bq.y),
                                  H2<T16>::hi(bq.y)};
 #pragma unroll
-            for (int j = 0; j < MB; ++j) {
+            for (int j = 0; j < NJ; ++j) {
                 float y[4];
 #pragma unroll
                 for (int e = 0; e < 4; ++e) y[e] = (SC ? acc[i][j][rq * 4 + e] * (sa[j] * sw[e]) : acc[i][j][rq * 4 + e]) + bv[e];
-                const int row = j * 32 + fr;
+                const int row = j * BLK + fr;
                 u32x2 p;
                 p.x = H2<T16>::pack(y[0], y[1]);
                 p.y = H2<T16>::pack(y[2], y[3]);
@@ -273,6 +308,17 @@
         }
     }
 }
+template <int EPI, int MB, bool SC = false, int GRP = 4, typename T16 = bf16_t>
+__device__ __forceinline__ void epilogue_wave_b(const GemmArgs& a, const f32x16 (&acc)[2][MB], int mw, int nw, char* patch, int lane,
+                                                const u32x2 (&bvec)[8]) {
+    epilogue_wave_m<EPI, MB, SC, GRP, T16, 32>(a, acc, mw, nw, patch, lane, bvec);
+}
+template <int EPI, typename T16 = bf16_t>
+__device__ __forceinline__ void epilogue_wave16(const GemmArgs& a, const f32x4 (&acc)[4][8], int mw, int nw, char* patch, int lane) {
+    u32x2 bvec[4];
+    load_bias64_m<16>(a, nw, lane, bvec);
+    epilogue_wave_m<EPI, 4, false, 4, T16, 16>(a, acc, mw, nw, patch, lane, bvec);
+}
 template <int EPI, int MB, bool SC = false, typename T16 = bf16_t>
 __device__ __forceinline__ void epilogue_wave(const GemmArgs& a, const f32x16 (&acc)[2][MB], int mw, int nw, char* patch, int lane) {
     u32x2 bvec[8];
diff --git a/disentangled-subject-to-vid_amd/csrc/gemm_g4.hip b/disentangled-subject-to-vid_amd/csrc/gemm_g4.hip
--- a/disentangled-subject-to-vid_amd/csrc/gemm_g4.hip
+++ b/disentangled-subject-to-vid_amd/csrc/gemm_g4.hip
@@ -7,6 +7,13 @@
 #include <cstdlib>
 #include <type_traits>
 
+#ifndef G4_MFMA
+#define G4_MFMA 32
+#endif
+#if G4_MFMA == 16
+static_assert(G4_BLK == 16 && G4_ACC_AT(1, 1) == 36 && G4_ACC_ROW(37) == 5 && G4_ACC_COL(3, 37) == 11 && G4_FRAG_CHUNK(1, 37) == 6, "gemm_g4_regs.h: unexpected accumulator map");
+#endif
+
 typedef __attribute__((ext_vector_type(32))) float f32x32;
 typedef __attribute__((ext_vector_type(16))) unsigned int u32x16;
 typedef __attribute__((ext_vector_type(8))) unsigned int u32x8;
@@ -22,11 +29,13 @@
     return 0;
 }
 #define G4_STAMP(i) const long long g4_t##i = (long long)__builtin_amdgcn_s_memtime()
+static int g_g4_mfma = G4_MFMA;
+extern "C" __attribute__((visibility("default"))) int s2v_set_g4_mfma(int shape) { g_g4_mfma = shape == 32 ? 32 : G4_MFMA; return 0; }
 #else
 #define G4_STAMP(i) do { } while (0)
 #endif
 
-template <int EPI, typename T16 = bf16_t>
+template <int EPI, typename T16 = bf16_t, int BLK = G4_MFMA>
 __global__ __launch_bounds__(256, 1) void gemm_g4(const GemmArgs a, int tiles_m, int tiles_n) {
     extern __shared__ __attribute__((aligned(16))) char smem[];
     const int tid = threadIdx.x, lane = tid & 63;
@@ -37,7 +46,7 @@
 #endif
     const int wave = __builtin_amdgcn_readfirstlane(tid >> 6);
     const int wm = wave >> 1, wn = wave & 1;
-    const int fr = lane & 31, hi = lane >> 5;
+    const int fr = lane % BLK, hi = lane / BLK;
 
     const int nwg = gridDim.x, bid = blockIdx.x;
     const int q = nwg >> 3, r = nwg & 7, xcd = bid & 7, idx = bid >> 3;
@@ -54,12 +63,13 @@
     const int m0 = (first_m + in_g % gsz) * 256, n0 = (in_g / gsz) * 256;
 
     const unsigned lds0 = __builtin_amdgcn_readfirstlane(lds_base_u32(smem));
+    constexpr int NKS = BLK == 16 ? 2 : 4;
     u32x16 vaddr, voff;
 #pragma unroll
     for (int g = 0; g < 2; ++g)
 #pragma unroll
         for (int s = 0; s < 4; ++s) {
-            const unsigned inrow = (unsigned)(((s * 2 + hi) ^ ((fr >> 1) & 7)) << 4);
+            const unsigned inrow = (unsigned)((((s % NKS) * (8 / NKS) + hi) ^ ((fr >> 1) & 7)) << 4);
             vaddr[4 * g + s] = lds0 + g * G4_A_STRIDE + (wm * 128 + fr) * 128 + inrow;
             vaddr[8 + 4 * g + s] = lds0 + G4_W_BASE + g * G4_W_STRIDE + (wn * 128 + fr) * 128 + inrow;
         }
@@ -93,20 +103,48 @@
 
     G4_STAMP(1);
     f32x32 AC[8];
-    if constexpr (std::is_same<T16, f16_t>::value) {
-        asm volatile(
+#if G4_MFMA == 16
+    static_assert(BLK == 16 || BLK == 32, "gemm_g4: MFMA shape");
+    if constexpr (BLK == 16) {
+        if constexpr (std::is_same<T16, f16_t>::value) {
+#define G4_M16_T "_f16"
+            asm volatile(
+#include "gemm_g4_body_m16.inc"
+                : "=" G4_ACC0(AC[0]), "=" G4_ACC1(AC[1]), "=" G4_ACC2(AC[2]), "=" G4_ACC3(AC[3]), "=" G4_ACC4(AC[4]), "=" G4_ACC5(AC[5]),
+                  "=" G4_ACC6(AC[6]), "=" G4_ACC7(AC[7]), "+" G4_PTR(ptr), "+" G4_SIN(sin), "+" G4_VADDR(vaddr)
+                : G4_VOFF(voff), G4_VPF(vpf), G4_SK(sk), G4_VSK(voff16)
+                : G4_CLOBBERS);
+#undef G4_M16_T
+        } else {
+#define G4_M16_T "_bf16"
+            asm volatile(
+#include "gemm_g4_body_m16.inc"
+                : "=" G4_ACC0(AC[0]), "=" G4_ACC1(AC[1]), "=" G4_ACC2(AC[2]), "=" G4_ACC3(AC[3]), "=" G4_ACC4(AC[4]), "=" G4_ACC5(AC[5]),
+                  "=" G4_ACC6(AC[6]), "=" G4_ACC7(AC[7]), "+" G4_PTR(ptr), "+" G4_SIN(sin), "+" G4_VADDR(vaddr)
+                : G4_VOFF(voff), G4_VPF(vpf), G4_SK(sk), G4_VSK(voff16)
+                : G4_CLOBBERS);
+#undef G4_M16_T
+        }
+    } else
+#else
+    static_assert(BLK == 32, "gemm_g4_regs.h was generated without the 16-form");
+#endif
+    {
+        if constexpr (std::is_same<T16, f16_t>::value) {
+            asm volatile(
 #include "gemm_g4_body_f16.inc"
-            : "=" G4_ACC0(AC[0]), "=" G4_ACC1(AC[1]), "=" G4_ACC2(AC[2]), "=" G4_ACC3(AC[3]), "=" G4_ACC4(AC[4]), "=" G4_ACC5(AC[5]),
-              "=" G4_ACC6(AC[6]), "=" G4_ACC7(AC[7]), "+" G4_PTR(ptr), "+" G4_SIN(sin), "+" G4_VADDR(vaddr)
-            : G4_VOFF(voff), G4_VPF(vpf), G4_SK(sk), G4_VSK(voff16)
-            : G4_CLOBBERS);
-    } else {
-        asm volatile(
+                : "=" G4_ACC0(AC[0]), "=" G4_ACC1(AC[1]), "=" G4_ACC2(AC[2]), "=" G4_ACC3(AC[3]), "=" G4_ACC4(AC[4]), "=" G4_ACC5(AC[5]),
+                  "=" G4_ACC6(AC[6]), "=" G4_ACC7(AC[7]), "+" G4_PTR(ptr), "+" G4_SIN(sin), "+" G4_VADDR(vaddr)
+                : G4_VOFF(voff), G4_VPF(vpf), G4_SK(sk), G4_VSK(voff16)
+                : G4_CLOBBERS);
+        } else {
+            asm volatile(
 #include "gemm_g4_body.inc"
-            : "=" G4_ACC0(AC[0]), "=" G4_ACC1(AC[1]), "=" G4_ACC2(AC[2]), "=" G4_ACC3(AC[3]), "=" G4_ACC4(AC[4]), "=" G4_ACC5(AC[5]),
-              "=" G4_ACC6(AC[6]), "=" G4_ACC7(AC[7]), "+" G4_PTR(ptr), "+" G4_SIN(sin), "+" G4_VADDR(vaddr)
-            : G4_VOFF(voff), G4_VPF(vpf), G4_SK(sk), G4_VSK(voff16)
-            : G4_CLOBBERS);
+                : "=" G4_ACC0(AC[0]), "=" G4_ACC1(AC[1]), "=" G4_ACC2(AC[2]), "=" G4_ACC3(AC[3]), "=" G4_ACC4(AC[4]), "=" G4_ACC5(AC[5]),
+                  "=" G4_ACC6(AC[6]), "=" G4_ACC7(AC[7]), "+" G4_PTR(ptr), "+" G4_SIN(sin), "+" G4_VADDR(vaddr)
+                : G4_VOFF(voff), G4_VPF(vpf), G4_SK(sk), G4_VSK(voff16)
+                : G4_CLOBBERS);
+        }
     }
     G4_STAMP(2);
     __builtin_amdgcn_s_barrier();
@@ -134,14 +172,25 @@
     char* patch = smem + wave * 16384;
 #pragma unroll
     for (int h = 0; h < 2; ++h) {
-        f32x16 acc[2][4];
-#pragma unroll
-        for (int i = 0; i < 2; ++i)
-#pragma unroll
-            for (int j = 0; j < 4; ++j)
-#pragma unroll
-                for (int e = 0; e < 16; ++e) acc[i][j][e] = AC[2 * (2 * h + i) + (j >> 1)][(j & 1) * 16 + e];
-        epilogue_wave<EPI, 4, false, T16>(a, acc, m0 + wm * 128, n0 + wn * 128 + h * 64, patch, lane);
+        if constexpr (BLK == 16) {
+            f32x4 acc[4][8];
+#pragma unroll
+            for (int i = 0; i < 4; ++i)
+#pragma unroll
+                for (int j = 0; j < 8; ++j)
+#pragma unroll
+                    for (int e = 0; e < 4; ++e) acc[i][j][e] = AC[4 * h + i][4 * j + e];
+            epilogue_wave16<EPI, T16>(a, acc, m0 + wm * 128, n0 + wn * 128 + h * 64, patch, lane);
+        } else {
+            f32x16 acc[2][4];
+#pragma unroll
+            for (int i = 0; i < 2; ++i)
+#pragma unroll
+                for (int j = 0; j < 4; ++j)
+#pragma unroll
+                    for (int e = 0; e < 16; ++e) acc[i][j][e] = AC[2 * (2 * h + i) + (j >> 1)][(j & 1) * 16 + e];
+            epilogue_wave<EPI, 4, false, T16>(a, acc, m0 + wm * 128, n0 + wn * 128 + h * 64, patch, lane);
+        }
     }
 #ifdef S2V_DIAG
     asm volatile("s_waitcnt vmcnt(0)" ::: "memory");
@@ -171,6 +220,9 @@
 #endif
     }
     const void* fn = (const void*)gemm_g4<EPI, T16>;
+#if defined(S2V_DIAG) && G4_MFMA == 16
+    if (g_g4_mfma == 32) fn = (const void*)gemm_g4<EPI, T16, 32>;
+#endif
     S2V_TRY(ensure_lds_attr(fn, G4_LDS_BYTES));
     void* args[] = {(void*)&a, (void*)&tiles_m, (void*)&tiles_n};
     const int S = a.splitk > 1 ? a.splitk : 1;
diff --git a/disentangled-subject-to-vid_amd/csrc/gemm_g4_body_m16.inc b/disentangled-subject-to-vid_amd/csrc/gemm_g4_body_m16.inc
--- /dev/null
+++ b/disentangled-subject-to-vid_amd/csrc/gemm_g4_body_m16.inc
@@ -0,0 +1,1400 @@
+"; ---- gemm_g4 K loop (generated by gen_gemm_g4.py; do not edit)\n\t"
+".macro MF i, j\n\t"
+"v_mfma_f32_16x16x32" G4_M16_T " a[32*\\i+4*\\j:32*\\i+4*\\j+3], v[4*\\i:4*\\i+3], v[32+4*\\j:32+4*\\j+3], a[32*\\i+4*\\j:32*\\i+4*\\j+3]\n\t"
+".endm\n\t"
+".macro MZ i, j\n\t"
+"v_mfma_f32_16x16x32" G4_M16_T " a[32*\\i+4*\\j:32*\\i+4*\\j+3], v[4*\\i:4*\\i+3], v[32+4*\\j:32+4*\\j+3], 0\n\t"
+".endm\n\t"
+".macro RW i, addr\n\t"
+"ds_read_b128 v[4*\\i:4*\\i+3], \\addr offset:2048*\\i\n\t"
+".endm\n\t"
+".macro RA j, addr\n\t"
+"ds_read_b128 v[32+4*\\j:32+4*\\j+3], \\addr offset:2048*\\j\n\t"
+".endm\n\t"
+"s_add_u32 m0, s40, 0\n\t"
+"s_nop 0\n\t"
+"global_load_lds_dwordx4 v80, s[36:37]\n\t"
+"s_add_u32 m0, s40, 4096\n\t"
+"s_nop 0\n\t"
+"global_load_lds_dwordx4 v81, s[36:37]\n\t"
+"s_add_u32 m0, s40, 8192\n\t"
+"s_nop 0\n\t"
+"global_load_lds_dwordx4 v82, s[36:37]\n\t"
+"s_add_u32 m0, s40, 12288\n\t"
+"s_nop 0\n\t"
+"global_load_lds_dwordx4 v83, s[36:37]\n\t"
+"s_add_u32 m0, s40, 16384\n\t"
+"s_nop 0\n\t"
+"global_load_lds_dwordx4 v84, s[36:37]\n\t"
+"s_add_u32 m0, s40, 20480\n\t"
+"s_nop 0\n\t"
+"global_load_lds_dwordx4 v85, s[36:37]\n\t"
+"s_add_u32 m0, s40, 24576\n\t"
+"s_nop 0\n\t"
+"global_load_lds_dwordx4 v86, s[36:37]\n\t"
+"s_add_u32 m0, s40, 28672\n\t"
+"s_nop 0\n\t"
+"global_load_lds_dwordx4 v87, s[36:37]\n\t"
+"s_add_u32 m0, s40, 98304\n\t"
+"s_nop 0\n\t"
+"global_load_lds_dwordx4 v88, s[38:39]\n\t"
+"s_add_u32 m0, s40, 102400\n\t"
+"s_nop 0\n\t"
+"global_load_lds_dwordx4 v89, s[38:39]\n\t"
+"s_add_u32 m0, s40, 106496\n\t"
+"s_nop 0\n\t"
+"global_load_lds_dwordx4 v90, s[38:39]\n\t"
+"s_add_u32 m0, s40, 110592\n\t"
+"s_nop 0\n\t"
+"global_load_lds_dwordx4 v91, s[38:39]\n\t"
+"s_add_u32 m0, s40, 114688\n\t"
+"s_nop 0\n\t"
+"global_load_lds_dwordx4 v92, s[38:39]\n\t"
+"s_add_u32 m0, s40, 118784\n\t"
+"s_nop 0\n\t"
+"global_load_lds_dwordx4 v93, s[38:39]\n\t"
+"s_add_u32 m0, s40, 122880\n\t"
+"s_nop 0\n\t"
+"global_load_lds_dwordx4 v94, s[38:39]\n\t"
+"s_add_u32 m0, s40, 126976\n\t"
+"s_nop 0\n\t"
+"global_load_lds_dwordx4 v95, s[38:39]\n\t"
+"s_add_u32 s36, s36, 128\n\t"
+"s_addc_u32 s37, s37, 0\n\t"
+"s_add_u32 s38, s38, 128\n\t"
+"s_addc_u32 s39, s39, 0\n\t"
+"s_add_u32 m0, s40, 32768\n\t"
+"s_nop 0\n\t"
+"global_load_lds_dwordx4 v80, s[36:37]\n\t"
+"s_add_u32 m0, s40, 36864\n\t"
+"s_nop 0\n\t"
+"global_load_lds_dwordx4 v81, s[36:37]\n\t"
+"s_add_u32 m0, s40, 40960\n\t"
+"s_nop 0\n\t"
+"global_load_lds_dwordx4 v82, s[36:37]\n\t"
+"s_add_u32 m0, s40, 45056\n\t"
+"s_nop 0\n\t"
+"global_load_lds_dwordx4 v83, s[36:37]\n\t"
+"s_add_u32 m0, s40, 49152\n\t"
+"s_nop 0\n\t"
+"global_load_lds_dwordx4 v84, s[36:37]\n\t"
+"s_add_u32 m0, s40, 53248\n\t"
+"s_nop 0\n\t"
+"global_load_lds_dwordx4 v85, s[36:37]\n\t"
+"s_add_u32 m0, s40, 57344\n\t"
+"s_nop 0\n\t"
+"global_load_lds_dwordx4 v86, s[36:37]\n\t"
+"s_add_u32 m0, s40, 61440\n\t"
+"s_nop 0\n\t"
+"global_load_lds_dwordx4 v87, s[36:37]\n\t"
+"s_add_u32 m0, s40, 131072\n\t"
+"s_nop 0\n\t"
+"global_load_lds_dwordx4 v88, s[38:39]\n\t"
+"s_add_u32 m0, s40, 135168\n\t"
+"s_nop 0\n\t"
+"global_load_lds_dwordx4 v89, s[38:39]\n\t"
+"s_add_u32 m0, s40, 139264\n\t"
+"s_nop 0\n\t"
+"global_load_lds_dwordx4 v90, s[38:39]\n\t"
+"s_add_u32 m0, s40, 143360\n\t"
+"s_nop 0\n\t"
+"global_load_lds_dwordx4 v91, s[38:39]\n\t"
+"s_add_u32 m0, s40, 147456\n\t"
+"s_nop 0\n\t"
+"global_load_lds_dwordx4 v92, s[38:39]\n\t"
+"s_add_u32 m0, s40, 151552\n\t"
+"s_nop 0\n\t"
+"global_load_lds_dwordx4 v93, s[38:39]\n\t"
+"s_add_u32 m0, s40, 155648\n\t"
+"s_nop 0\n\t"
+"global_load_lds_dwordx4 v94, s[38:39]\n\t"
+"s_add_u32 m0, s40, 159744\n\t"
+"s_nop 0\n\t"
+"global_load_lds_dwordx4 v95, s[38:39]\n\t"
+"s_add_u32 s36, s36, 128\n\t"
+"s_addc_u32 s37, s37, 0\n\t"
+"s_add_u32 s38, s38, 128\n\t"
+"s_addc_u32 s39, s39, 0\n\t"
+"s_mov_b32 s42, 32768\n\t"
+"s_mov_b32 s43, 65536\n\t"
+"v_mov_b32 v100, v64\n\t"
+"v_mov_b32 v101, v65\n\t"
+"s_waitcnt vmcnt(16)\n\t"
+"s_barrier\n\t"
+"RW 0, v72\n\t"
+"RW 1, v72\n\t"
+"RW 2, v72\n\t"
+"RW 3, v72\n\t"
+"RW 4, v72\n\t"
+"RW 5, v72\n\t"
+"RW 6, v72\n\t"
+"RA 0, v64\n\t"
+"RA 1, v64\n\t"
+"RA 2, v64\n\t"
+"RA 3, v64\n\t"
+"; K-tile 0\n\t"
+"s_waitcnt lgkmcnt(0)\n\t"
+"s_add_u32 s48, s40, s43\n\t"
+"MZ 0, 0\n\t"
+"RW 7, v72\n\t"
+"MZ 0, 1\n\t"
+"RA 4, v64\n\t"
+"s_add_u32 m0, s48, 0\n\t"
+"MZ 0, 2\n\t"
+"RA 5, v64\n\t"
+"MZ 0, 3\n\t"
+"RA 6, v64\n\t"
+"global_load_lds_dwordx4 v80, s[36:37]\n\t"
+"MZ 1, 0\n\t"
+"RA 7, v64\n\t"
+"MZ 1, 1\n\t"
+"s_add_u32 m0, s48, 4096\n\t"
+"MZ 1, 2\n\t"
+"MZ 1, 3\n\t"
+"global_load_lds_dwordx4 v81, s[36:37]\n\t"
+"MZ 2, 0\n\t"
+"MZ 2, 1\n\t"
+"s_add_u32 m0, s48, 8192\n\t"
+"MZ 2, 2\n\t"
+"MZ 2, 3\n\t"
+"global_load_lds_dwordx4 v82, s[36:37]\n\t"
+"MZ 3, 0\n\t"
+"MZ 3, 1\n\t"
+"s_add_u32 m0, s48, 12288\n\t"
+"MZ 3, 2\n\t"
+"MZ 3, 3\n\t"
+"global_load_lds_dwordx4 v83, s[36:37]\n\t"
+"MZ 4, 0\n\t"
+"MZ 4, 1\n\t"
+"s_add_u32 m0, s48, 16384\n\t"
+"MZ 4, 2\n\t"
+"MZ 4, 3\n\t"
+"global_load_lds_dwordx4 v84, s[36:37]\n\t"
+"MZ 5, 0\n\t"
+"MZ 5, 1\n\t"
+"s_add_u32 m0, s48, 20480\n\t"
+"MZ 5, 2\n\t"
+"MZ 5, 3\n\t"
+"global_load_lds_dwordx4 v85, s[36:37]\n\t"
+"MZ 6, 0\n\t"
+"MZ 6, 1\n\t"
+"s_add_u32 m0, s48, 24576\n\t"
+"MZ 6, 2\n\t"
+"MZ 6, 3\n\t"
+"global_load_lds_dwordx4 v86, s[36:37]\n\t"
+"s_waitcnt lgkmcnt(0)\n\t"
+"MZ 7, 0\n\t"
+"MZ 7, 1\n\t"
+"s_add_u32 m0, s48, 28672\n\t"
+"MZ 7, 2\n\t"
+"MZ 7, 3\n\t"
+"global_load_lds_dwordx4 v87, s[36:37]\n\t"
+"s_add_u32 s36, s36, 128\n\t"
+"s_addc_u32 s37, s37, 0\n\t"
+"s_waitcnt lgkmcnt(0)\n\t"
+"MZ 0, 4\n\t"
+"RA 0, v65\n\t"
+"MZ 0, 5\n\t"
+"RA 1, v65\n\t"
+"MZ 0, 6\n\t"
+"RA 2, v65\n\t"
+"MZ 0, 7\n\t"
+"RA 3, v65\n\t"
+"MZ 1, 4\n\t"
+"RW 0, v73\n\t"
+"MZ 1, 5\n\t"
+"MZ 1, 6\n\t"
+"MZ 1, 7\n\t"
+"MZ 2, 4\n\t"
+"RW 1, v73\n\t"
+"MZ 2, 5\n\t"
+"MZ 2, 6\n\t"
+"MZ 2, 7\n\t"
+"MZ 3, 4\n\t"
+"RW 2, v73\n\t"
+"MZ 3, 5\n\t"
+"MZ 3, 6\n\t"
+"MZ 3, 7\n\t"
+"MZ 4, 4\n\t"
+"RW 3, v73\n\t"
+"MZ 4, 5\n\t"
+"MZ 4, 6\n\t"
+"MZ 4, 7\n\t"
+"MZ 5, 4\n\t"
+"RW 4, v73\n\t"
+"MZ 5, 5\n\t"
+"MZ 5, 6\n\t"
+"MZ 5, 7\n\t"
+"MZ 6, 4\n\t"
+"RW 5, v73\n\t"
+"MZ 6, 5\n\t"
+"v_add_u32 v68, s42, v100\n\t"
+"MZ 6, 6\n\t"
+"MZ 6, 7\n\t"
+"v_add_u32 v69, s42, v101\n\t"
+"MZ 7, 4\n\t"
+"RW 6, v73\n\t"
+"MZ 7, 5\n\t"
+"MZ 7, 6\n\t"
+"MZ 7, 7\n\t"
+"s_mov_b32 s42, s43\n\t"
+"s_add_u32 s43, s43, 32768\n\t"
+"s_cmp_ge_u32 s43, 98304\n\t"
+"s_cselect_b32 s43, 0, s43\n\t"
+"s_waitcnt lgkmcnt(0)\n\t"
+"MF 0, 0\n\t"
+"RW 7, v73\n\t"
+"MF 0, 1\n\t"
+"RA 4, v65\n\t"
+"MF 0, 2\n\t"
+"RA 5, v65\n\t"
+"MF 0, 3\n\t"
+"RA 6, v65\n\t"
+"MF 1, 0\n\t"
+"RA 7, v65\n\t"
+"MF 1, 1\n\t"
+"MF 1, 2\n\t"
+"MF 1, 3\n\t"
+"MF 2, 0\n\t"
+"MF 2, 1\n\t"
+"MF 2, 2\n\t"
+"MF 2, 3\n\t"
+"MF 3, 0\n\t"
+"MF 3, 1\n\t"
+"MF 3, 2\n\t"
+"MF 3, 3\n\t"
+"MF 4, 0\n\t"
+"MF 4, 1\n\t"
+"MF 4, 2\n\t"
+"MF 4, 3\n\t"
+"MF 5, 0\n\t"
+"MF 5, 1\n\t"
+"MF 5, 2\n\t"
+"MF 5, 3\n\t"
+"MF 6, 0\n\t"
+"MF 6, 1\n\t"
+"MF 6, 2\n\t"
+"MF 6, 3\n\t"
+"s_waitcnt lgkmcnt(0)\n\t"
+"MF 7, 0\n\t"
+"MF 7, 1\n\t"
+"MF 7, 2\n\t"
+"MF 7, 3\n\t"
+"s_waitcnt vmcnt(8) lgkmcnt(0)\n\t"
+"s_barrier\n\t"
+"MF 0, 4\n\t"
+"RA 0, v68\n\t"
+"MF 0, 5\n\t"
+"RA 1, v68\n\t"
+"s_add_u32 m0, s40, 98304\n\t"
+"MF 0, 6\n\t"
+"RA 2, v68\n\t"
+"MF 0, 7\n\t"
+"RA 3, v68\n\t"
+"global_load_lds_dwordx4 v88, s[38:39]\n\t"
+"MF 1, 4\n\t"
+"RW 0, v76\n\t"
+"MF 1, 5\n\t"
+"s_add_u32 m0, s40, 102400\n\t"
+"MF 1, 6\n\t"
+"MF 1, 7\n\t"
+"global_load_lds_dwordx4 v89, s[38:39]\n\t"
+"MF 2, 4\n\t"
+"RW 1, v76\n\t"
+"MF 2, 5\n\t"
+"s_add_u32 m0, s40, 106496\n\t"
+"MF 2, 6\n\t"
+"MF 2, 7\n\t"
+"global_load_lds_dwordx4 v90, s[38:39]\n\t"
+"MF 3, 4\n\t"
+"RW 2, v76\n\t"
+"MF 3, 5\n\t"
+"s_add_u32 m0, s40, 110592\n\t"
+"MF 3, 6\n\t"
+"MF 3, 7\n\t"
+"global_load_lds_dwordx4 v91, s[38:39]\n\t"
+"MF 4, 4\n\t"
+"RW 3, v76\n\t"
+"MF 4, 5\n\t"
+"s_add_u32 m0, s40, 114688\n\t"
+"MF 4, 6\n\t"
+"MF 4, 7\n\t"
+"global_load_lds_dwordx4 v92, s[38:39]\n\t"
+"MF 5, 4\n\t"
+"RW 4, v76\n\t"
+"MF 5, 5\n\t"
+"s_add_u32 m0, s40, 118784\n\t"
+"MF 5, 6\n\t"
+"MF 5, 7\n\t"
+"global_load_lds_dwordx4 v93, s[38:39]\n\t"
+"MF 6, 4\n\t"
+"RW 5, v76\n\t"
+"MF 6, 5\n\t"
+"s_add_u32 m0, s40, 122880\n\t"
+"MF 6, 6\n\t"
+"MF 6, 7\n\t"
+"global_load_lds_dwordx4 v94, s[38:39]\n\t"
+"MF 7, 4\n\t"
+"RW 6, v76\n\t"
+"MF 7, 5\n\t"
+"s_add_u32 m0, s40, 126976\n\t"
+"MF 7, 6\n\t"
+"MF 7, 7\n\t"
+"global_load_lds_dwordx4 v95, s[38:39]\n\t"
+"s_add_u32 s38, s38, 128\n\t"
+"s_addc_u32 s39, s39, 0\n\t"
+"L_g4_loop_%=:\n\t"
+"s_cmp_eq_u32 s41, 0\n\t"
+"s_cbranch_scc1 L_g4_nopf_%=\n\t"
+"s_waitcnt lgkmcnt(0)\n\t"
+"s_add_u32 s48, s40, s43\n\t"
+"MF 0, 0\n\t"
+"RW 7, v76\n\t"
+"MF 0, 1\n\t"
+"RA 4, v68\n\t"
+"s_add_u32 m0, s48, 0\n\t"
+"MF 0, 2\n\t"
+"RA 5, v68\n\t"
+"MF 0, 3\n\t"
+"RA 6, v68\n\t"
+"global_load_lds_dwordx4 v80, s[36:37]\n\t"
+"MF 1, 0\n\t"
+"RA 7, v68\n\t"
+"MF 1, 1\n\t"
+"s_add_u32 m0, s48, 4096\n\t"
+"MF 1, 2\n\t"
+"MF 1, 3\n\t"
+"global_load_lds_dwordx4 v81, s[36:37]\n\t"
+"MF 2, 0\n\t"
+"MF 2, 1\n\t"
+"s_add_u32 m0, s48, 8192\n\t"
+"MF 2, 2\n\t"
+"MF 2, 3\n\t"
+"global_load_lds_dwordx4 v82, s[36:37]\n\t"
+"MF 3, 0\n\t"
+"MF 3, 1\n\t"
+"s_add_u32 m0, s48, 12288\n\t"
+"MF 3, 2\n\t"
+"MF 3, 3\n\t"
+"global_load_lds_dwordx4 v83, s[36:37]\n\t"
+"MF 4, 0\n\t"
+"MF 4, 1\n\t"
+"s_add_u32 m0, s48, 16384\n\t"
+"MF 4, 2\n\t"
+"MF 4, 3\n\t"
+"global_load_lds_dwordx4 v84, s[36:37]\n\t"
+"MF 5, 0\n\t"
+"MF 5, 1\n\t"
+"s_add_u32 m0, s48, 20480\n\t"
+"MF 5, 2\n\t"
+"MF 5, 3\n\t"
+"global_load_lds_dwordx4 v85, s[36:37]\n\t"
+"MF 6, 0\n\t"
+"MF 6, 1\n\t"
+"s_add_u32 m0, s48, 24576\n\t"
+"MF 6, 2\n\t"
+"MF 6, 3\n\t"
+"global_load_lds_dwordx4 v86, s[36:37]\n\t"
+"s_waitcnt lgkmcnt(0)\n\t"
+"MF 7, 0\n\t"
+"MF 7, 1\n\t"
+"s_add_u32 m0, s48, 28672\n\t"
+"MF 7, 2\n\t"
+"MF 7, 3\n\t"
+"global_load_lds_dwordx4 v87, s[36:37]\n\t"
+"s_add_u32 s36, s36, 128\n\t"
+"s_addc_u32 s37, s37, 0\n\t"
+"s_waitcnt lgkmcnt(0)\n\t"
+"MF 0, 4\n\t"
+"RA 0, v69\n\t"
+"MF 0, 5\n\t"
+"RA 1, v69\n\t"
+"MF 0, 6\n\t"
+"RA 2, v69\n\t"
+"MF 0, 7\n\t"
+"RA 3, v69\n\t"
+"MF 1, 4\n\t"
+"RW 0, v77\n\t"
+"MF 1, 5\n\t"
+"MF 1, 6\n\t"
+"MF 1, 7\n\t"
+"MF 2, 4\n\t"
+"RW 1, v77\n\t"
+"MF 2, 5\n\t"
+"MF 2, 6\n\t"
+"MF 2, 7\n\t"
+"MF 3, 4\n\t"
+"RW 2, v77\n\t"
+"MF 3, 5\n\t"
+"MF 3, 6\n\t"
+"MF 3, 7\n\t"
+"MF 4, 4\n\t"
+"RW 3, v77\n\t"
+"MF 4, 5\n\t"
+"MF 4, 6\n\t"
+"MF 4, 7\n\t"
+"MF 5, 4\n\t"
+"RW 4, v77\n\t"
+"MF 5, 5\n\t"
+"MF 5, 6\n\t"
+"MF 5, 7\n\t"
+"MF 6, 4\n\t"
+"RW 5, v77\n\t"
+"MF 6, 5\n\t"
+"v_add_u32 v64, s42, v100\n\t"
+"MF 6, 6\n\t"
+"MF 6, 7\n\t"
+"v_add_u32 v65, s42, v101\n\t"
+"MF 7, 4\n\t"
+"RW 6, v77\n\t"
+"MF 7, 5\n\t"
+"MF 7, 6\n\t"
+"MF 7, 7\n\t"
+"s_mov_b32 s42, s43\n\t"
+"s_add_u32 s43, s43, 32768\n\t"
+"s_cmp_ge_u32 s43, 98304\n\t"
+"s_cselect_b32 s43, 0, s43\n\t"
+"s_waitcnt lgkmcnt(0)\n\t"
+"MF 0, 0\n\t"
+"RW 7, v77\n\t"
+"MF 0, 1\n\t"
+"RA 4, v69\n\t"
+"MF 0, 2\n\t"
+"RA 5, v69\n\t"
+"MF 0, 3\n\t"
+"RA 6, v69\n\t"
+"MF 1, 0\n\t"
+"RA 7, v69\n\t"
+"MF 1, 1\n\t"
+"MF 1, 2\n\t"
+"MF 1, 3\n\t"
+"MF 2, 0\n\t"
+"MF 2, 1\n\t"
+"MF 2, 2\n\t"
+"MF 2, 3\n\t"
+"MF 3, 0\n\t"
+"MF 3, 1\n\t"
+"MF 3, 2\n\t"
+"MF 3, 3\n\t"
+"MF 4, 0\n\t"
+"MF 4, 1\n\t"
+"MF 4, 2\n\t"
+"MF 4, 3\n\t"
+"MF 5, 0\n\t"
+"MF 5, 1\n\t"
+"MF 5, 2\n\t"
+"MF 5, 3\n\t"
+"MF 6, 0\n\t"
+"MF 6, 1\n\t"
+"MF 6, 2\n\t"
+"MF 6, 3\n\t"
+"s_waitcnt lgkmcnt(0)\n\t"
+"MF 7, 0\n\t"
+"MF 7, 1\n\t"
+"MF 7, 2\n\t"
+"MF 7, 3\n\t"
+"s_waitcnt vmcnt(8) lgkmcnt(0)\n\t"
+"s_barrier\n\t"
+"MF 0, 4\n\t"
+"RA 0, v64\n\t"
+"MF 0, 5\n\t"
+"RA 1, v64\n\t"
+"s_add_u32 m0, s40, 131072\n\t"
+"MF 0, 6\n\t"
+"RA 2, v64\n\t"
+"MF 0, 7\n\t"
+"RA 3, v64\n\t"
+"global_load_lds_dwordx4 v88, s[38:39]\n\t"
+"MF 1, 4\n\t"
+"RW 0, v72\n\t"
+"MF 1, 5\n\t"
+"s_add_u32 m0, s40, 135168\n\t"
+"MF 1, 6\n\t"
+"MF 1, 7\n\t"
+"global_load_lds_dwordx4 v89, s[38:39]\n\t"
+"MF 2, 4\n\t"
+"RW 1, v72\n\t"
+"MF 2, 5\n\t"
+"s_add_u32 m0, s40, 139264\n\t"
+"MF 2, 6\n\t"
+"MF 2, 7\n\t"
+"global_load_lds_dwordx4 v90, s[38:39]\n\t"
+"MF 3, 4\n\t"
+"RW 2, v72\n\t"
+"MF 3, 5\n\t"
+"s_add_u32 m0, s40, 143360\n\t"
+"MF 3, 6\n\t"
+"MF 3, 7\n\t"
+"global_load_lds_dwordx4 v91, s[38:39]\n\t"
+"MF 4, 4\n\t"
+"RW 3, v72\n\t"
+"MF 4, 5\n\t"
+"s_add_u32 m0, s40, 147456\n\t"
+"MF 4, 6\n\t"
+"MF 4, 7\n\t"
+"global_load_lds_dwordx4 v92, s[38:39]\n\t"
+"MF 5, 4\n\t"
+"RW 4, v72\n\t"
+"MF 5, 5\n\t"
+"s_add_u32 m0, s40, 151552\n\t"
+"MF 5, 6\n\t"
+"MF 5, 7\n\t"
+"global_load_lds_dwordx4 v93, s[38:39]\n\t"
+"MF 6, 4\n\t"
+"RW 5, v72\n\t"
+"MF 6, 5\n\t"
+"s_add_u32 m0, s40, 155648\n\t"
+"MF 6, 6\n\t"
+"MF 6, 7\n\t"
+"global_load_lds_dwordx4 v94, s[38:39]\n\t"
+"MF 7, 4\n\t"
+"RW 6, v72\n\t"
+"MF 7, 5\n\t"
+"s_add_u32 m0, s40, 159744\n\t"
+"MF 7, 6\n\t"
+"MF 7, 7\n\t"
+"global_load_lds_dwordx4 v95, s[38:39]\n\t"
+"s_add_u32 s38, s38, 128\n\t"
+"s_addc_u32 s39, s39, 0\n\t"
+"s_waitcnt lgkmcnt(0)\n\t"
+"s_add_u32 s48, s40, s43\n\t"
+"MF 0, 0\n\t"
+"RW 7, v72\n\t"
+"MF 0, 1\n\t"
+"RA 4, v64\n\t"
+"s_add_u32 m0, s48, 0\n\t"
+"MF 0, 2\n\t"
+"RA 5, v64\n\t"
+"MF 0, 3\n\t"
+"RA 6, v64\n\t"
+"global_load_lds_dwordx4 v80, s[36:37]\n\t"
+"MF 1, 0\n\t"
+"RA 7, v64\n\t"
+"MF 1, 1\n\t"
+"s_add_u32 m0, s48, 4096\n\t"
+"MF 1, 2\n\t"
+"MF 1, 3\n\t"
+"global_load_lds_dwordx4 v81, s[36:37]\n\t"
+"MF 2, 0\n\t"
+"MF 2, 1\n\t"
+"s_add_u32 m0, s48, 8192\n\t"
+"MF 2, 2\n\t"
+"MF 2, 3\n\t"
+"global_load_lds_dwordx4 v82, s[36:37]\n\t"
+"MF 3, 0\n\t"
+"MF 3, 1\n\t"
+"s_add_u32 m0, s48, 12288\n\t"
+"MF 3, 2\n\t"
+"MF 3, 3\n\t"
+"global_load_lds_dwordx4 v83, s[36:37]\n\t"
+"MF 4, 0\n\t"
+"MF 4, 1\n\t"
+"s_add_u32 m0, s48, 16384\n\t"
+"MF 4, 2\n\t"
+"MF 4, 3\n\t"
+"global_load_lds_dwordx4 v84, s[36:37]\n\t"
+"MF 5, 0\n\t"
+"MF 5, 1\n\t"
+"s_add_u32 m0, s48, 20480\n\t"
+"MF 5, 2\n\t"
+"MF 5, 3\n\t"
+"global_load_lds_dwordx4 v85, s[36:37]\n\t"
+"MF 6, 0\n\t"
+"MF 6, 1\n\t"
+"s_add_u32 m0, s48, 24576\n\t"
+"MF 6, 2\n\t"
+"MF 6, 3\n\t"
+"global_load_lds_dwordx4 v86, s[36:37]\n\t"
+"s_waitcnt lgkmcnt(0)\n\t"
+"MF 7, 0\n\t"
+"MF 7, 1\n\t"
+"s_add_u32 m0, s48, 28672\n\t"
+"MF 7, 2\n\t"
+"MF 7, 3\n\t"
+"global_load_lds_dwordx4 v87, s[36:37]\n\t"
+"s_add_u32 s36, s36, 128\n\t"
+"s_addc_u32 s37, s37, 0\n\t"
+"s_waitcnt lgkmcnt(0)\n\t"
+"MF 0, 4\n\t"
+"RA 0, v65\n\t"
+"MF 0, 5\n\t"
+"RA 1, v65\n\t"
+"MF 0, 6\n\t"
+"RA 2, v65\n\t"
+"MF 0, 7\n\t"
+"RA 3, v65\n\t"
+"MF 1, 4\n\t"
+"RW 0, v73\n\t"
+"MF 1, 5\n\t"
+"MF 1, 6\n\t"
+"MF 1, 7\n\t"
+"MF 2, 4\n\t"
+"RW 1, v73\n\t"
+"MF 2, 5\n\t"
+"MF 2, 6\n\t"
+"MF 2, 7\n\t"
+"MF 3, 4\n\t"
+"RW 2, v73\n\t"
+"MF 3, 5\n\t"
+"MF 3, 6\n\t"
+"MF 3, 7\n\t"
+"MF 4, 4\n\t"
+"RW 3, v73\n\t"
+"MF 4, 5\n\t"
+"MF 4, 6\n\t"
+"MF 4, 7\n\t"
+"MF 5, 4\n\t"
+"RW 4, v73\n\t"
+"MF 5, 5\n\t"
+"MF 5, 6\n\t"
+"MF 5, 7\n\t"
+"MF 6, 4\n\t"
+"RW 5, v73\n\t"
+"MF 6, 5\n\t"
+"v_add_u32 v68, s42, v100\n\t"
+"MF 6, 6\n\t"
+"MF 6, 7\n\t"
+"v_add_u32 v69, s42, v101\n\t"
+"MF 7, 4\n\t"
+"RW 6, v73\n\t"
+"MF 7, 5\n\t"
+"MF 7, 6\n\t"
+"MF 7, 7\n\t"
+"s_mov_b32 s42, s43\n\t"
+"s_add_u32 s43, s43, 32768\n\t"
+"s_cmp_ge_u32 s43, 98304\n\t"
+"s_cselect_b32 s43, 0, s43\n\t"
+"s_waitcnt lgkmcnt(0)\n\t"
+"MF 0, 0\n\t"
+"RW 7, v73\n\t"
+"MF 0, 1\n\t"
+"RA 4, v65\n\t"
+"MF 0, 2\n\t"
+"RA 5, v65\n\t"
+"MF 0, 3\n\t"
+"RA 6, v65\n\t"
+"MF 1, 0\n\t"
+"RA 7, v65\n\t"
+"MF 1, 1\n\t"
+"MF 1, 2\n\t"
+"MF 1, 3\n\t"
+"MF 2, 0\n\t"
+"MF 2, 1\n\t"
+"MF 2, 2\n\t"
+"MF 2, 3\n\t"
+"MF 3, 0\n\t"
+"MF 3, 1\n\t"
+"MF 3, 2\n\t"
+"MF 3, 3\n\t"
+"MF 4, 0\n\t"
+"MF 4, 1\n\t"
+"MF 4, 2\n\t"
+"MF 4, 3\n\t"
+"MF 5, 0\n\t"
+"MF 5, 1\n\t"
+"MF 5, 2\n\t"
+"MF 5, 3\n\t"
+"MF 6, 0\n\t"
+"MF 6, 1\n\t"
+"MF 6, 2\n\t"
+"MF 6, 3\n\t"
+"s_waitcnt lgkmcnt(0)\n\t"
+"MF 7, 0\n\t"
+"MF 7, 1\n\t"
+"MF 7, 2\n\t"
+"MF 7, 3\n\t"
+"s_waitcnt vmcnt(8) lgkmcnt(0)\n\t"
+"s_barrier\n\t"
+"MF 0, 4\n\t"
+"RA 0, v68\n\t"
+"MF 0, 5\n\t"
+"RA 1, v68\n\t"
+"s_add_u32 m0, s40, 98304\n\t"
+"MF 0, 6\n\t"
+"RA 2, v68\n\t"
+"MF 0, 7\n\t"
+"RA 3, v68\n\t"
+"global_load_lds_dwordx4 v88, s[38:39]\n\t"
+"MF 1, 4\n\t"
+"RW 0, v76\n\t"
+"MF 1, 5\n\t"
+"s_add_u32 m0, s40, 102400\n\t"
+"MF 1, 6\n\t"
+"MF 1, 7\n\t"
+"global_load_lds_dwordx4 v89, s[38:39]\n\t"
+"MF 2, 4\n\t"
+"RW 1, v76\n\t"
+"MF 2, 5\n\t"
+"s_add_u32 m0, s40, 106496\n\t"
+"MF 2, 6\n\t"
+"MF 2, 7\n\t"
+"global_load_lds_dwordx4 v90, s[38:39]\n\t"
+"MF 3, 4\n\t"
+"RW 2, v76\n\t"
+"MF 3, 5\n\t"
+"s_add_u32 m0, s40, 110592\n\t"
+"MF 3, 6\n\t"
+"MF 3, 7\n\t"
+"global_load_lds_dwordx4 v91, s[38:39]\n\t"
+"MF 4, 4\n\t"
+"RW 3, v76\n\t"
+"MF 4, 5\n\t"
+"s_add_u32 m0, s40, 114688\n\t"
+"MF 4, 6\n\t"
+"MF 4, 7\n\t"
+"global_load_lds_dwordx4 v92, s[38:39]\n\t"
+"MF 5, 4\n\t"
+"RW 4, v76\n\t"
+"MF 5, 5\n\t"
+"s_add_u32 m0, s40, 118784\n\t"
+"MF 5, 6\n\t"
+"MF 5, 7\n\t"
+"global_load_lds_dwordx4 v93, s[38:39]\n\t"
+"MF 6, 4\n\t"
+"RW 5, v76\n\t"
+"MF 6, 5\n\t"
+"s_add_u32 m0, s40, 122880\n\t"
+"MF 6, 6\n\t"
+"MF 6, 7\n\t"
+"global_load_lds_dwordx4 v94, s[38:39]\n\t"
+"MF 7, 4\n\t"
+"RW 6, v76\n\t"
+"MF 7, 5\n\t"
+"s_add_u32 m0, s40, 126976\n\t"
+"MF 7, 6\n\t"
+"MF 7, 7\n\t"
+"global_load_lds_dwordx4 v95, s[38:39]\n\t"
+"s_add_u32 s38, s38, 128\n\t"
+"s_addc_u32 s39, s39, 0\n\t"
+"s_sub_u32 s41, s41, 1\n\t"
+"s_branch L_g4_loop_%=\n\t"
+"L_g4_nopf_%=:\n\t"
+"s_waitcnt lgkmcnt(0)\n\t"
+"s_add_u32 s48, s40, s43\n\t"
+"MF 0, 0\n\t"
+"RW 7, v76\n\t"
+"MF 0, 1\n\t"
+"RA 4, v68\n\t"
+"s_add_u32 m0, s48, 0\n\t"
+"MF 0, 2\n\t"
+"RA 5, v68\n\t"
+"MF 0, 3\n\t"
+"RA 6, v68\n\t"
+"global_load_lds_dwordx4 v80, s[36:37]\n\t"
+"MF 1, 0\n\t"
+"RA 7, v68\n\t"
+"MF 1, 1\n\t"
+"s_add_u32 m0, s48, 4096\n\t"
+"MF 1, 2\n\t"
+"MF 1, 3\n\t"
+"global_load_lds_dwordx4 v81, s[36:37]\n\t"
+"MF 2, 0\n\t"
+"MF 2, 1\n\t"
+"s_add_u32 m0, s48, 8192\n\t"
+"MF 2, 2\n\t"
+"MF 2, 3\n\t"
+"global_load_lds_dwordx4 v82, s[36:37]\n\t"
+"MF 3, 0\n\t"
+"MF 3, 1\n\t"
+"s_add_u32 m0, s48, 12288\n\t"
+"MF 3, 2\n\t"
+"MF 3, 3\n\t"
+"global_load_lds_dwordx4 v83, s[36:37]\n\t"
+"MF 4, 0\n\t"
+"MF 4, 1\n\t"
+"s_add_u32 m0, s48, 16384\n\t"
+"MF 4, 2\n\t"
+"MF 4, 3\n\t"
+"global_load_lds_dwordx4 v84, s[36:37]\n\t"
+"MF 5, 0\n\t"
+"MF 5, 1\n\t"
+"s_add_u32 m0, s48, 20480\n\t"
+"MF 5, 2\n\t"
+"MF 5, 3\n\t"
+"global_load_lds_dwordx4 v85, s[36:37]\n\t"
+"MF 6, 0\n\t"
+"MF 6, 1\n\t"
+"s_add_u32 m0, s48, 24576\n\t"
+"MF 6, 2\n\t"
+"MF 6, 3\n\t"
+"global_load_lds_dwordx4 v86, s[36:37]\n\t"
+"s_waitcnt lgkmcnt(0)\n\t"
+"MF 7, 0\n\t"
+"MF 7, 1\n\t"
+"s_add_u32 m0, s48, 28672\n\t"
+"MF 7, 2\n\t"
+"MF 7, 3\n\t"
+"global_load_lds_dwordx4 v87, s[36:37]\n\t"
+"s_add_u32 s36, s36, 128\n\t"
+"s_addc_u32 s37, s37, 0\n\t"
+"s_waitcnt lgkmcnt(0)\n\t"
+"MF 0, 4\n\t"
+"RA 0, v69\n\t"
+"MF 0, 5\n\t"
+"RA 1, v69\n\t"
+"MF 0, 6\n\t"
+"RA 2, v69\n\t"
+"MF 0, 7\n\t"
+"RA 3, v69\n\t"
+"MF 1, 4\n\t"
+"RW 0, v77\n\t"
+"MF 1, 5\n\t"
+"MF 1, 6\n\t"
+"MF 1, 7\n\t"
+"MF 2, 4\n\t"
+"RW 1, v77\n\t"
+"MF 2, 5\n\t"
+"MF 2, 6\n\t"
+"MF 2, 7\n\t"
+"MF 3, 4\n\t"
+"RW 2, v77\n\t"
+"MF 3, 5\n\t"
+"MF 3, 6\n\t"
+"MF 3, 7\n\t"
+"MF 4, 4\n\t"
+"RW 3, v77\n\t"
+"MF 4, 5\n\t"
+"MF 4, 6\n\t"
+"MF 4, 7\n\t"
+"MF 5, 4\n\t"
+"RW 4, v77\n\t"
+"MF 5, 5\n\t"
+"MF 5, 6\n\t"
+"MF 5, 7\n\t"
+"MF 6, 4\n\t"
+"RW 5, v77\n\t"
+"MF 6, 5\n\t"
+"v_add_u32 v64, s42, v100\n\t"
+"MF 6, 6\n\t"
+"MF 6, 7\n\t"
+"v_add_u32 v65, s42, v101\n\t"
+"MF 7, 4\n\t"
+"RW 6, v77\n\t"
+"MF 7, 5\n\t"
+"MF 7, 6\n\t"
+"MF 7, 7\n\t"
+"s_mov_b32 s42, s43\n\t"
+"s_add_u32 s43, s43, 32768\n\t"
+"s_cmp_ge_u32 s43, 98304\n\t"
+"s_cselect_b32 s43, 0, s43\n\t"
+"s_waitcnt lgkmcnt(0)\n\t"
+"MF 0, 0\n\t"
+"RW 7, v77\n\t"
+"MF 0, 1\n\t"
+"RA 4, v69\n\t"
+"MF 0, 2\n\t"
+"RA 5, v69\n\t"
+"MF 0, 3\n\t"
+"RA 6, v69\n\t"
+"MF 1, 0\n\t"
+"RA 7, v69\n\t"
+"MF 1, 1\n\t"
+"MF 1, 2\n\t"
+"MF 1, 3\n\t"
+"MF 2, 0\n\t"
+"MF 2, 1\n\t"
+"MF 2, 2\n\t"
+"MF 2, 3\n\t"
+"MF 3, 0\n\t"
+"MF 3, 1\n\t"
+"MF 3, 2\n\t"
+"MF 3, 3\n\t"
+"MF 4, 0\n\t"
+"MF 4, 1\n\t"
+"MF 4, 2\n\t"
+"MF 4, 3\n\t"
+"MF 5, 0\n\t"
+"MF 5, 1\n\t"
+"MF 5, 2\n\t"
+"MF 5, 3\n\t"
+"MF 6, 0\n\t"
+"MF 6, 1\n\t"
+"MF 6, 2\n\t"
+"MF 6, 3\n\t"
+"s_waitcnt lgkmcnt(0)\n\t"
+"MF 7, 0\n\t"
+"MF 7, 1\n\t"
+"MF 7, 2\n\t"
+"MF 7, 3\n\t"
+"s_waitcnt vmcnt(8) lgkmcnt(0)\n\t"
+"s_barrier\n\t"
+"MF 0, 4\n\t"
+"RA 0, v64\n\t"
+"MF 0, 5\n\t"
+"RA 1, v64\n\t"
+"s_add_u32 m0, s40, 131072\n\t"
+"MF 0, 6\n\t"
+"RA 2, v64\n\t"
+"MF 0, 7\n\t"
+"RA 3, v64\n\t"
+"global_load_lds_dwordx4 v88, s[38:39]\n\t"
+"MF 1, 4\n\t"
+"RW 0, v72\n\t"
+"MF 1, 5\n\t"
+"s_add_u32 m0, s40, 135168\n\t"
+"MF 1, 6\n\t"
+"MF 1, 7\n\t"
+"global_load_lds_dwordx4 v89, s[38:39]\n\t"
+"MF 2, 4\n\t"
+"RW 1, v72\n\t"
+"MF 2, 5\n\t"
+"s_add_u32 m0, s40, 139264\n\t"
+"MF 2, 6\n\t"
+"MF 2, 7\n\t"
+"global_load_lds_dwordx4 v90, s[38:39]\n\t"
+"MF 3, 4\n\t"
+"RW 2, v72\n\t"
+"MF 3, 5\n\t"
+"s_add_u32 m0, s40, 143360\n\t"
+"MF 3, 6\n\t"
+"MF 3, 7\n\t"
+"global_load_lds_dwordx4 v91, s[38:39]\n\t"
+"MF 4, 4\n\t"
+"RW 3, v72\n\t"
+"MF 4, 5\n\t"
+"s_add_u32 m0, s40, 147456\n\t"
+"MF 4, 6\n\t"
+"MF 4, 7\n\t"
+"global_load_lds_dwordx4 v92, s[38:39]\n\t"
+"MF 5, 4\n\t"
+"RW 4, v72\n\t"
+"MF 5, 5\n\t"
+"s_add_u32 m0, s40, 151552\n\t"
+"MF 5, 6\n\t"
+"MF 5, 7\n\t"
+"global_load_lds_dwordx4 v93, s[38:39]\n\t"
+"MF 6, 4\n\t"
+"RW 5, v72\n\t"
+"MF 6, 5\n\t"
+"s_add_u32 m0, s40, 155648\n\t"
+"MF 6, 6\n\t"
+"MF 6, 7\n\t"
+"global_load_lds_dwordx4 v94, s[38:39]\n\t"
+"MF 7, 4\n\t"
+"RW 6, v72\n\t"
+"MF 7, 5\n\t"
+"s_add_u32 m0, s40, 159744\n\t"
+"MF 7, 6\n\t"
+"MF 7, 7\n\t"
+"global_load_lds_dwordx4 v95, s[38:39]\n\t"
+"s_add_u32 s38, s38, 128\n\t"
+"s_addc_u32 s39, s39, 0\n\t"
+"s_waitcnt lgkmcnt(0)\n\t"
+"MF 0, 0\n\t"
+"RW 7, v72\n\t"
+"MF 0, 1\n\t"
+"RA 4, v64\n\t"
+"MF 0, 2\n\t"
+"RA 5, v64\n\t"
+"MF 0, 3\n\t"
+"RA 6, v64\n\t"
+"MF 1, 0\n\t"
+"RA 7, v64\n\t"
+"MF 1, 1\n\t"
+"MF 1, 2\n\t"
+"MF 1, 3\n\t"
+"MF 2, 0\n\t"
+"MF 2, 1\n\t"
+"MF 2, 2\n\t"
+"MF 2, 3\n\t"
+"MF 3, 0\n\t"
+"MF 3, 1\n\t"
+"MF 3, 2\n\t"
+"MF 3, 3\n\t"
+"MF 4, 0\n\t"
+"MF 4, 1\n\t"
+"MF 4, 2\n\t"
+"MF 4, 3\n\t"
+"MF 5, 0\n\t"
+"MF 5, 1\n\t"
+"MF 5, 2\n\t"
+"MF 5, 3\n\t"
+"MF 6, 0\n\t"
+"MF 6, 1\n\t"
+"MF 6, 2\n\t"
+"MF 6, 3\n\t"
+"s_waitcnt lgkmcnt(0)\n\t"
+"MF 7, 0\n\t"
+"MF 7, 1\n\t"
+"MF 7, 2\n\t"
+"MF 7, 3\n\t"
+"s_waitcnt lgkmcnt(0)\n\t"
+"MF 0, 4\n\t"
+"RA 0, v65\n\t"
+"MF 0, 5\n\t"
+"RA 1, v65\n\t"
+"MF 0, 6\n\t"
+"RA 2, v65\n\t"
+"MF 0, 7\n\t"
+"RA 3, v65\n\t"
+"MF 1, 4\n\t"
+"RW 0, v73\n\t"
+"MF 1, 5\n\t"
+"MF 1, 6\n\t"
+"MF 1, 7\n\t"
+"MF 2, 4\n\t"
+"RW 1, v73\n\t"
+"MF 2, 5\n\t"
+"MF 2, 6\n\t"
+"MF 2, 7\n\t"
+"MF 3, 4\n\t"
+"RW 2, v73\n\t"
+"MF 3, 5\n\t"
+"MF 3, 6\n\t"
+"MF 3, 7\n\t"
+"MF 4, 4\n\t"
+"RW 3, v73\n\t"
+"MF 4, 5\n\t"
+"MF 4, 6\n\t"
+"MF 4, 7\n\t"
+"MF 5, 4\n\t"
+"RW 4, v73\n\t"
+"MF 5, 5\n\t"
+"MF 5, 6\n\t"
+"MF 5, 7\n\t"
+"MF 6, 4\n\t"
+"RW 5, v73\n\t"
+"MF 6, 5\n\t"
+"v_add_u32 v68, s42, v100\n\t"
+"MF 6, 6\n\t"
+"MF 6, 7\n\t"
+"v_add_u32 v69, s42, v101\n\t"
+"MF 7, 4\n\t"
+"RW 6, v73\n\t"
+"MF 7, 5\n\t"
+"MF 7, 6\n\t"
+"MF 7, 7\n\t"
+"s_mov_b32 s42, s43\n\t"
+"s_add_u32 s43, s43, 32768\n\t"
+"s_cmp_ge_u32 s43, 98304\n\t"
+"s_cselect_b32 s43, 0, s43\n\t"
+"s_waitcnt lgkmcnt(0)\n\t"
+"MF 0, 0\n\t"
+"RW 7, v73\n\t"
+"MF 0, 1\n\t"
+"RA 4, v65\n\t"
+"MF 0, 2\n\t"
+"RA 5, v65\n\t"
+"MF 0, 3\n\t"
+"RA 6, v65\n\t"
+"MF 1, 0\n\t"
+"RA 7, v65\n\t"
+"MF 1, 1\n\t"
+"MF 1, 2\n\t"
+"MF 1, 3\n\t"
+"MF 2, 0\n\t"
+"MF 2, 1\n\t"
+"MF 2, 2\n\t"
+"MF 2, 3\n\t"
+"MF 3, 0\n\t"
+"MF 3, 1\n\t"
+"MF 3, 2\n\t"
+"MF 3, 3\n\t"
+"MF 4, 0\n\t"
+"MF 4, 1\n\t"
+"MF 4, 2\n\t"
+"MF 4, 3\n\t"
+"MF 5, 0\n\t"
+"MF 5, 1\n\t"
+"MF 5, 2\n\t"
+"MF 5, 3\n\t"
+"MF 6, 0\n\t"
+"MF 6, 1\n\t"
+"MF 6, 2\n\t"
+"MF 6, 3\n\t"
+"s_waitcnt lgkmcnt(0)\n\t"
+"MF 7, 0\n\t"
+"MF 7, 1\n\t"
+"MF 7, 2\n\t"
+"MF 7, 3\n\t"
+"s_waitcnt vmcnt(0) lgkmcnt(0)\n\t"
+"s_barrier\n\t"
+"MF 0, 4\n\t"
+"RA 0, v68\n\t"
+"MF 0, 5\n\t"
+"RA 1, v68\n\t"
+"MF 0, 6\n\t"
+"RA 2, v68\n\t"
+"MF 0, 7\n\t"
+"RA 3, v68\n\t"
+"MF 1, 4\n\t"
+"RW 0, v76\n\t"
+"MF 1, 5\n\t"
+"MF 1, 6\n\t"
+"MF 1, 7\n\t"
+"MF 2, 4\n\t"
+"RW 1, v76\n\t"
+"MF 2, 5\n\t"
+"MF 2, 6\n\t"
+"MF 2, 7\n\t"
+"MF 3, 4\n\t"
+"RW 2, v76\n\t"
+"MF 3, 5\n\t"
+"MF 3, 6\n\t"
+"MF 3, 7\n\t"
+"MF 4, 4\n\t"
+"RW 3, v76\n\t"
+"MF 4, 5\n\t"
+"MF 4, 6\n\t"
+"MF 4, 7\n\t"
+"MF 5, 4\n\t"
+"RW 4, v76\n\t"
+"MF 5, 5\n\t"
+"MF 5, 6\n\t"
+"MF 5, 7\n\t"
+"MF 6, 4\n\t"
+"RW 5, v76\n\t"
+"MF 6, 5\n\t"
+"MF 6, 6\n\t"
+"MF 6, 7\n\t"
+"MF 7, 4\n\t"
+"RW 6, v76\n\t"
+"MF 7, 5\n\t"
+"MF 7, 6\n\t"
+"MF 7, 7\n\t"
+"s_waitcnt lgkmcnt(0)\n\t"
+"MF 0, 0\n\t"
+"RW 7, v76\n\t"
+"MF 0, 1\n\t"
+"RA 4, v68\n\t"
+"MF 0, 2\n\t"
+"RA 5, v68\n\t"
+"MF 0, 3\n\t"
+"RA 6, v68\n\t"
+"MF 1, 0\n\t"
+"RA 7, v68\n\t"
+"MF 1, 1\n\t"
+"MF 1, 2\n\t"
+"MF 1, 3\n\t"
+"MF 2, 0\n\t"
+"MF 2, 1\n\t"
+"MF 2, 2\n\t"
+"MF 2, 3\n\t"
+"MF 3, 0\n\t"
+"MF 3, 1\n\t"
+"MF 3, 2\n\t"
+"MF 3, 3\n\t"
+"MF 4, 0\n\t"
+"MF 4, 1\n\t"
+"MF 4, 2\n\t"
+"MF 4, 3\n\t"
+"MF 5, 0\n\t"
+"MF 5, 1\n\t"
+"MF 5, 2\n\t"
+"MF 5, 3\n\t"
+"MF 6, 0\n\t"
+"MF 6, 1\n\t"
+"MF 6, 2\n\t"
+"MF 6, 3\n\t"
+"s_waitcnt lgkmcnt(0)\n\t"
+"MF 7, 0\n\t"
+"MF 7, 1\n\t"
+"MF 7, 2\n\t"
+"MF 7, 3\n\t"
+"s_waitcnt lgkmcnt(0)\n\t"
+"MF 0, 4\n\t"
+"RA 0, v69\n\t"
+"MF 0, 5\n\t"
+"RA 1, v69\n\t"
+"MF 0, 6\n\t"
+"RA 2, v69\n\t"
+"MF 0, 7\n\t"
+"RA 3, v69\n\t"
+"MF 1, 4\n\t"
+"RW 0, v77\n\t"
+"MF 1, 5\n\t"
+"MF 1, 6\n\t"
+"MF 1, 7\n\t"
+"MF 2, 4\n\t"
+"RW 1, v77\n\t"
+"MF 2, 5\n\t"
+"MF 2, 6\n\t"
+"MF 2, 7\n\t"
+"MF 3, 4\n\t"
+"RW 2, v77\n\t"
+"MF 3, 5\n\t"
+"MF 3, 6\n\t"
+"MF 3, 7\n\t"
+"MF 4, 4\n\t"
+"RW 3, v77\n\t"
+"MF 4, 5\n\t"
+"MF 4, 6\n\t"
+"MF 4, 7\n\t"
+"MF 5, 4\n\t"
+"RW 4, v77\n\t"
+"MF 5, 5\n\t"
+"MF 5, 6\n\t"
+"MF 5, 7\n\t"
+"MF 6, 4\n\t"
+"RW 5, v77\n\t"
+"MF 6, 5\n\t"
+"MF 6, 6\n\t"
+"MF 6, 7\n\t"
+"MF 7, 4\n\t"
+"RW 6, v77\n\t"
+"MF 7, 5\n\t"
+"MF 7, 6\n\t"
+"MF 7, 7\n\t"
+"s_waitcnt lgkmcnt(0)\n\t"
+"MF 0, 0\n\t"
+"RW 7, v77\n\t"
+"MF 0, 1\n\t"
+"RA 4, v69\n\t"
+"MF 0, 2\n\t"
+"RA 5, v69\n\t"
+"MF 0, 3\n\t"
+"RA 6, v69\n\t"
+"MF 1, 0\n\t"
+"RA 7, v69\n\t"
+"MF 1, 1\n\t"
+"MF 1, 2\n\t"
+"MF 1, 3\n\t"
+"MF 2, 0\n\t"
+"MF 2, 1\n\t"
+"MF 2, 2\n\t"
+"MF 2, 3\n\t"
+"MF 3, 0\n\t"
+"MF 3, 1\n\t"
+"MF 3, 2\n\t"
+"MF 3, 3\n\t"
+"MF 4, 0\n\t"
+"MF 4, 1\n\t"
+"MF 4, 2\n\t"
+"MF 4, 3\n\t"
+"MF 5, 0\n\t"
+"MF 5, 1\n\t"
+"MF 5, 2\n\t"
+"MF 5, 3\n\t"
+"MF 6, 0\n\t"
+"MF 6, 1\n\t"
+"MF 6, 2\n\t"
+"MF 6, 3\n\t"
+"s_waitcnt lgkmcnt(0)\n\t"
+"MF 7, 0\n\t"
+"MF 7, 1\n\t"
+"MF 7, 2\n\t"
+"MF 7, 3\n\t"
+"s_waitcnt lgkmcnt(0)\n\t"
+"MF 0, 4\n\t"
+"MF 0, 5\n\t"
+"MF 0, 6\n\t"
+"MF 0, 7\n\t"
+"MF 1, 4\n\t"
+"MF 1, 5\n\t"
+"MF 1, 6\n\t"
+"MF 1, 7\n\t"
+"MF 2, 4\n\t"
+"MF 2, 5\n\t"
+"MF 2, 6\n\t"
+"MF 2, 7\n\t"
+"MF 3, 4\n\t"
+"MF 3, 5\n\t"
+"MF 3, 6\n\t"
+"MF 3, 7\n\t"
+"MF 4, 4\n\t"
+"MF 4, 5\n\t"
+"MF 4, 6\n\t"
+"MF 4, 7\n\t"
+"MF 5, 4\n\t"
+"MF 5, 5\n\t"
+"MF 5, 6\n\t"
+"MF 5, 7\n\t"
+"MF 6, 4\n\t"
+"MF 6, 5\n\t"
+"MF 6, 6\n\t"
+"MF 6, 7\n\t"
+"MF 7, 4\n\t"
+"MF 7, 5\n\t"
+"MF 7, 6\n\t"
+"MF 7, 7\n\t"
+"s_waitcnt vmcnt(0)\n\t"
+"s_nop 15\n\t"
+"s_nop 15\n\t"
+"s_cmp_lt_u32 s46, 2\n\t"
+"s_cbranch_scc1 L_g4_end_%=\n\t"
+"s_add_u32 s50, s44, 4096\n\t"
+"s_addc_u32 s51, s45, 0\n\t"
+"global_store_dwordx4 v98, a[0:3], s[50:51] offset:-4096 sc1\n\t"
+"global_store_dwordx4 v98, a[4:7], s[50:51] offset:-3072 sc1\n\t"
+"global_store_dwordx4 v98, a[8:11], s[50:51] offset:-2048 sc1\n\t"
+"global_store_dwordx4 v98, a[12:15], s[50:51] offset:-1024 sc1\n\t"
+"global_store_dwordx4 v98, a[16:19], s[50:51] offset:0 sc1\n\t"
+"global_store_dwordx4 v98, a[20:23], s[50:51] offset:1024 sc1\n\t"
+"global_store_dwordx4 v98, a[24:27], s[50:51] offset:2048 sc1\n\t"
+"global_store_dwordx4 v98, a[28:31], s[50:51] offset:3072 sc1\n\t"
+"s_add_u32 s50, s44, 12288\n\t"
+"s_addc_u32 s51, s45, 0\n\t"
+"global_store_dwordx4 v98, a[32:35], s[50:51] offset:-4096 sc1\n\t"
+"global_store_dwordx4 v98, a[36:39], s[50:51] offset:-3072 sc1\n\t"
+"global_store_dwordx4 v98, a[40:43], s[50:51] offset:-2048 sc1\n\t"
+"global_store_dwordx4 v98, a[44:47], s[50:51] offset:-1024 sc1\n\t"
+"global_store_dwordx4 v98, a[48:51], s[50:51] offset:0 sc1\n\t"
+"global_store_dwordx4 v98, a[52:55], s[50:51] offset:1024 sc1\n\t"
+"global_store_dwordx4 v98, a[56:59], s[50:51] offset:2048 sc1\n\t"
+"global_store_dwordx4 v98, a[60:63], s[50:51] offset:3072 sc1\n\t"
+"s_add_u32 s50, s44, 20480\n\t"
+"s_addc_u32 s51, s45, 0\n\t"
+"global_store_dwordx4 v98, a[64:67], s[50:51] offset:-4096 sc1\n\t"
+"global_store_dwordx4 v98, a[68:71], s[50:51] offset:-3072 sc1\n\t"
+"global_store_dwordx4 v98, a[72:75], s[50:51] offset:-2048 sc1\n\t"
+"global_store_dwordx4 v98, a[76:79], s[50:51] offset:-1024 sc1\n\t"
+"global_store_dwordx4 v98, a[80:83], s[50:51] offset:0 sc1\n\t"
+"global_store_dwordx4 v98, a[84:87], s[50:51] offset:1024 sc1\n\t"
+"global_store_dwordx4 v98, a[88:91], s[50:51] offset:2048 sc1\n\t"
+"global_store_dwordx4 v98, a[92:95], s[50:51] offset:3072 sc1\n\t"
+"s_add_u32 s50, s44, 28672\n\t"
+"s_addc_u32 s51, s45, 0\n\t"
+"global_store_dwordx4 v98, a[96:99], s[50:51] offset:-4096 sc1\n\t"
+"global_store_dwordx4 v98, a[100:103], s[50:51] offset:-3072 sc1\n\t"
+"global_store_dwordx4 v98, a[104:107], s[50:51] offset:-2048 sc1\n\t"
+"global_store_dwordx4 v98, a[108:111], s[50:51] offset:-1024 sc1\n\t"
+"global_store_dwordx4 v98, a[112:115], s[50:51] offset:0 sc1\n\t"
+"global_store_dwordx4 v98, a[116:119], s[50:51] offset:1024 sc1\n\t"
+"global_store_dwordx4 v98, a[120:123], s[50:51] offset:2048 sc1\n\t"
+"global_store_dwordx4 v98, a[124:127], s[50:51] offset:3072 sc1\n\t"
+"s_add_u32 s50, s44, 36864\n\t"
+"s_addc_u32 s51, s45, 0\n\t"
+"global_store_dwordx4 v98, a[128:131], s[50:51] offset:-4096 sc1\n\t"
+"global_store_dwordx4 v98, a[132:135], s[50:51] offset:-3072 sc1\n\t"
+"global_store_dwordx4 v98, a[136:139], s[50:51] offset:-2048 sc1\n\t"
+"global_store_dwordx4 v98, a[140:143], s[50:51] offset:-1024 sc1\n\t"
+"global_store_dwordx4 v98, a[144:147], s[50:51] offset:0 sc1\n\t"
+"global_store_dwordx4 v98, a[148:151], s[50:51] offset:1024 sc1\n\t"
+"global_store_dwordx4 v98, a[152:155], s[50:51] offset:2048 sc1\n\t"
+"global_store_dwordx4 v98, a[156:159], s[50:51] offset:3072 sc1\n\t"
+"s_add_u32 s50, s44, 45056\n\t"
+"s_addc_u32 s51, s45, 0\n\t"
+"global_store_dwordx4 v98, a[160:163], s[50:51] offset:-4096 sc1\n\t"
+"global_store_dwordx4 v98, a[164:167], s[50:51] offset:-3072 sc1\n\t"
+"global_store_dwordx4 v98, a[168:171], s[50:51] offset:-2048 sc1\n\t"
+"global_store_dwordx4 v98, a[172:175], s[50:51] offset:-1024 sc1\n\t"
+"global_store_dwordx4 v98, a[176:179], s[50:51] offset:0 sc1\n\t"
+"global_store_dwordx4 v98, a[180:183], s[50:51] offset:1024 sc1\n\t"
+"global_store_dwordx4 v98, a[184:187], s[50:51] offset:2048 sc1\n\t"
+"global_store_dwordx4 v98, a[188:191], s[50:51] offset:3072 sc1\n\t"
+"s_add_u32 s50, s44, 53248\n\t"
+"s_addc_u32 s51, s45, 0\n\t"
+"global_store_dwordx4 v98, a[192:195], s[50:51] offset:-4096 sc1\n\t"
+"global_store_dwordx4 v98, a[196:199], s[50:51] offset:-3072 sc1\n\t"
+"global_store_dwordx4 v98, a[200:203], s[50:51] offset:-2048 sc1\n\t"
+"global_store_dwordx4 v98, a[204:207], s[50:51] offset:-1024 sc1\n\t"
+"global_store_dwordx4 v98, a[208:211], s[50:51] offset:0 sc1\n\t"
+"global_store_dwordx4 v98, a[212:215], s[50:51] offset:1024 sc1\n\t"
+"global_store_dwordx4 v98, a[216:219], s[50:51] offset:2048 sc1\n\t"
+"global_store_dwordx4 v98, a[220:223], s[50:51] offset:3072 sc1\n\t"
+"s_add_u32 s50, s44, 61440\n\t"
+"s_addc_u32 s51, s45, 0\n\t"
+"global_store_dwordx4 v98, a[224:227], s[50:51] offset:-4096 sc1\n\t"
+"global_store_dwordx4 v98, a[228:231], s[50:51] offset:-3072 sc1\n\t"
+"global_store_dwordx4 v98, a[232:235], s[50:51] offset:-2048 sc1\n\t"
+"global_store_dwordx4 v98, a[236:239], s[50:51] offset:-1024 sc1\n\t"
+"global_store_dwordx4 v98, a[240:243], s[50:51] offset:0 sc1\n\t"
+"global_store_dwordx4 v98, a[244:247], s[50:51] offset:1024 sc1\n\t"
+"global_store_dwordx4 v98, a[248:251], s[50:51] offset:2048 sc1\n\t"
+"global_store_dwordx4 v98, a[252:255], s[50:51] offset:3072 sc1\n\t"
+"s_waitcnt vmcnt(0)\n\t"
+"L_g4_end_%=:\n\t"
+".purgem MF\n\t"
+".purgem MZ\n\t"
+".purgem RW\n\t"
+".purgem RA\n\t"
diff --git a/disentangled-subject-to-vid_amd/csrc/gemm_g4_regs.h b/disentangled-subject-to-vid_amd/csrc/gemm_g4_regs.h
--- a/disentangled-subject-to-vid_amd/csrc/gemm_g4_regs.h
+++ b/disentangled-subject-to-vid_amd/csrc/gemm_g4_regs.h
@@ -1,4 +1,10 @@
 #pragma once
+#define G4_MFMA 16
+#define G4_BLK 16
+#define G4_ACC_AT(i, j) (32 * (i) + 4 * (j))
+#define G4_ACC_ROW(l) ((l) & 15)
+#define G4_ACC_COL(r, l) (4 * ((l) >> 4) + (r))
+#define G4_FRAG_CHUNK(ks, l) (4 * (ks) + ((l) >> 4))
 #define G4_PF 0
 #define G4_LDS_BYTES 163840
 #define G4_A_STRIDE 32768
diff --git a/disentangled-subject-to-vid_amd/csrc/gen_gemm_g4.py b/disentangled-subject-to-vid_amd/csrc/gen_gemm_g4.py
--- a/disentangled-subject-to-vid_amd/csrc/gen_gemm_g4.py
+++ b/disentangled-subject-to-vid_amd/csrc/gen_gemm_g4.py
@@ -9,6 +9,9 @@
 W3 = os.environ.get("G4_W3", "0") == "1"
 A3 = os.environ.get("G4_A3", "1") == "1" and os.environ.get("G4_W3", "0") != "1" and os.environ.get("G4_STAGE", "dma") == "dma"
 assert not (A3 and W3)
+MFMA = int(os.environ.get("G4_MFMA", "16"))
+assert MFMA in (16, 32)
+M16 = MFMA == 16 and A3
 S_WNEXT, S_WDMA, S_WM0, WBASE = 42, 43, 48, 100
 A_STRIDE, W_BASE, W_STRIDE = (32768, 65536, 32768) if W3 else (32768, 98304, 32768) if A3 else (65536, 32768, 65536)
 A_POL = (" " + os.environ["G4_A_POL"]) if os.environ.get("G4_A_POL") else ""
@@ -37,6 +40,8 @@
 
 
 def ktile(emit, g, first=False, dma_w=True, dma_a=True, last=False, prefetch=False):
+    if M16:
+        return ktile_a3_m16(emit, g, first, dma_w, dma_a, last)
     if A3:
         return ktile_a3(emit, g, first, dma_w, dma_a, last)
     for s in range(4):
@@ -136,6 +141,76 @@
             emit(f"s_cmp_ge_u32 s{S_WDMA}, {3 * A_STRIDE}")
             emit(f"s_cselect_b32 s{S_WDMA}, 0, s{S_WDMA}")
         if s == 3 and dma_w:
+            emit(f"s_add_u32 s{S_W}, s{S_W}, 128")
+            emit(f"s_addc_u32 s{S_W + 1}, s{S_W + 1}, 0")
+
+
+def wf16(i):
+    return FRAG + 4 * i
+
+
+def af16(j):
+    return FRAG + 32 + 4 * j
+
+
+def m16_prologue_reads(emit):
+    for i in range(7):
+        emit(f"ds_read_b128 {vr(wf16(i), 4)}, {vr(vaddr(True, 0, 0))} offset:{i * 2048}")
+    for j in range(4):
+        emit(f"ds_read_b128 {vr(af16(j), 4)}, {vr(vaddr(False, 0, 0))} offset:{j * 2048}")
+
+
+def ktile_a3_m16(emit, g, first, dma_w, dma_a, last):
+    for ph in range(4):
+        ks, half = ph >> 1, ph & 1
+        if ph == 3 and not last:
+            emit(f"s_waitcnt vmcnt({8 if dma_a else 0}) lgkmcnt(0)")
+            emit("s_barrier")
+        else:
+            emit("s_waitcnt lgkmcnt(0)")
+        if ph == 0 and dma_a:
+            emit(f"s_add_u32 s{S_WM0}, s{S_M0W}, s{S_WDMA}")
+        gn, kn = (g, 1) if ks == 0 else (g ^ 1, 0)
+        for n in range(32):
+            i, j = n >> 2, 4 * half + (n & 3)
+            if half == 0 and n == 28:
+                emit("s_waitcnt lgkmcnt(0)")
+            acc = ar(ACC + 32 * i + 4 * j, 4)
+            c = "0" if (first and ks == 0) else acc
+            emit(f"v_mfma_f32_16x16x32_bf16 {acc}, {vr(wf16(i), 4)}, {vr(af16(j), 4)}, {c}")
+            if half == 0:
+                if n == 0:
+                    emit(f"ds_read_b128 {vr(wf16(7), 4)}, {vr(vaddr(True, g, ks))} offset:{7 * 2048}")
+                elif n <= 4:
+                    emit(f"ds_read_b128 {vr(af16(3 + n), 4)}, {vr(vaddr(False, g, ks))} offset:{(3 + n) * 2048}")
+            elif not (last and ph == 3):
+                if n < 4:
+                    emit(f"ds_read_b128 {vr(af16(n), 4)}, {vr(vaddr(False, gn, kn))} offset:{n * 2048}")
+                if n >= 4 and n & 3 == 0:
+                    emit(f"ds_read_b128 {vr(wf16(i - 1), 4)}, {vr(vaddr(True, gn, kn))} offset:{(i - 1) * 2048}")
+            p = n >> 2
+            if ph == 0 and dma_a:
+                if n & 3 == 1:
+                    emit(f"s_add_u32 m0, s{S_WM0}, {p * 4096}")
+                if n & 3 == 3:
+                    emit(f"global_load_lds_dwordx4 {vr(VOFF + p)}, s[{S_A}:{S_A + 1}]{A_POL}")
+            if ph == 1 and not last and n in (25, 27):
+                x = (n - 25) >> 1
+                emit(f"v_add_u32 {vr(vaddr(False, g ^ 1, x))}, s{S_WNEXT}, {vr(WBASE + x)}")
+            if ph == 3 and dma_w:
+                if n & 3 == 1:
+                    emit(f"s_add_u32 m0, s{S_M0W}, {W_BASE + g * W_STRIDE + p * 4096}")
+                if n & 3 == 3:
+                    emit(f"global_load_lds_dwordx4 {vr(VOFF + 8 + p)}, s[{S_W}:{S_W + 1}]{W_POL}")
+        if ph == 0 and dma_a:
+            emit(f"s_add_u32 s{S_A}, s{S_A}, 128")
+            emit(f"s_addc_u32 s{S_A + 1}, s{S_A + 1}, 0")
+        if ph == 1 and not last:
+            emit(f"s_mov_b32 s{S_WNEXT}, s{S_WDMA}")
+            emit(f"s_add_u32 s{S_WDMA}, s{S_WDMA}, {A_STRIDE}")
+            emit(f"s_cmp_ge_u32 s{S_WDMA}, {3 * A_STRIDE}")
+            emit(f"s_cselect_b32 s{S_WDMA}, 0, s{S_WDMA}")
+        if ph == 3 and dma_w:
             emit(f"s_add_u32 s{S_W}, s{S_W}, 128")
             emit(f"s_addc_u32 s{S_W + 1}, s{S_W + 1}, 0")
 
@@ -337,11 +412,13 @@
             emit(f"s_addc_u32 s{sp + 1}, s{sp + 1}, 0")
     emit(f"s_mov_b32 s{S_WNEXT}, {A_STRIDE}")
     emit(f"s_mov_b32 s{S_WDMA}, {2 * A_STRIDE}")
-    for x in range(4):
+    for x in range(2 if M16 else 4):
         emit(f"v_mov_b32 {vr(WBASE + x)}, {vr(vaddr(False, 0, x))}")
     emit("s_waitcnt vmcnt(16)")
     emit("s_barrier")
-    for n in range(8):
+    if M16:
+        m16_prologue_reads(emit)
+    for n in range(0 if M16 else 8):
         if n < 4:
             emit(f"ds_read_b128 {vr(wf(0, n), 4)}, {vr(vaddr(True, 0, 0))} offset:{n * 4096}")
         else:
@@ -423,15 +500,69 @@
     return out
 
 
+M16_MACROS = [
+    r'.macro MF i, j',
+    r'v_mfma_f32_16x16x32" G4_M16_T " a[32*\\i+4*\\j:32*\\i+4*\\j+3], v[4*\\i:4*\\i+3], v[32+4*\\j:32+4*\\j+3], a[32*\\i+4*\\j:32*\\i+4*\\j+3]',
+    r'.endm',
+    r'.macro MZ i, j',
+    r'v_mfma_f32_16x16x32" G4_M16_T " a[32*\\i+4*\\j:32*\\i+4*\\j+3], v[4*\\i:4*\\i+3], v[32+4*\\j:32+4*\\j+3], 0',
+    r'.endm',
+    r'.macro RW i, addr',
+    r'ds_read_b128 v[4*\\i:4*\\i+3], \\addr offset:2048*\\i',
+    r'.endm',
+    r'.macro RA j, addr',
+    r'ds_read_b128 v[32+4*\\j:32+4*\\j+3], \\addr offset:2048*\\j',
+    r'.endm',
+]
+
+
+def expand16(ln):
+    t = ln.replace(",", " ").split()
+    if t[0] in ("MF", "MZ"):
+        i, j = int(t[1]), int(t[2])
+        acc = ar(ACC + 32 * i + 4 * j, 4)
+        return f"v_mfma_f32_16x16x32_bf16 {acc}, {vr(wf16(i), 4)}, {vr(af16(j), 4)}, {acc if t[0] == 'MF' else '0'}"
+    if t[0] in ("RW", "RA"):
+        n = int(t[1])
+        return f"ds_read_b128 {vr(wf16(n) if t[0] == 'RW' else af16(n), 4)}, {t[2]} offset:{n * 2048}"
+    return ln
+
+
+def compact16(lines):
+    import re
+    out = []
+    for ln in lines:
+        m = re.fullmatch(r"v_mfma_f32_16x16x32_bf16 a\[(\d+):\d+\], v\[(\d+):\d+\], v\[(\d+):\d+\], (\S+)", ln)
+        r = re.fullmatch(r"ds_read_b128 v\[(\d+):\d+\], (v\d+) offset:(\d+)", ln)
+        if m:
+            i, j = (int(m.group(2)) - FRAG) // 4, (int(m.group(3)) - FRAG - 32) // 4
+            c = f"{'MZ' if m.group(4) == '0' else 'MF'} {i}, {j}"
+        elif r:
+            b = int(r.group(1)) - FRAG
+            c = f"RW {b // 4}, {r.group(2)}" if b < 32 else f"RA {(b - 32) // 4}, {r.group(2)}"
+        else:
+            c = ln
+        assert expand16(c) == ln, (ln, c)
+        out.append(c)
+    return [out[0]] + M16_MACROS + out[1:] + [".purgem MF", ".purgem MZ", ".purgem RW", ".purgem RA"]
+
+
 def main():
     here = os.environ.get("S2V_GEN_OUT") or os.path.dirname(os.path.abspath(__file__))
+    global M16
+    m16, M16 = M16, False
     body = gen_reg() if STAGE == "reg" else gen()
+    M16 = m16
     with open(os.path.join(here, "gemm_g4_body.inc"), "w") as f:
         for ln in body:
             f.write('"' + ln + '\\n\\t"\n')
     with open(os.path.join(here, "gemm_g4_body_f16.inc"), "w") as f:
         for ln in body:
             f.write('"' + ln.replace("v_mfma_f32_32x32x16_bf16", "v_mfma_f32_32x32x16_f16") + '\\n\\t"\n')
+    if M16:
+        with open(os.path.join(here, "gemm_g4_body_m16.inc"), "w") as f:
+            for ln in compact16(gen()):
+                f.write('"' + ln + '\\n\\t"\n')
     for name, body in (("gemm_g4_sk_sum.inc", gen_sk_sum()),):
         with open(os.path.join(here, name), "w") as f:
             for ln in body:
@@ -441,6 +572,13 @@
         clob += [f"v{WBASE + x}" for x in range(4)] + [f"s{S_WNEXT}", f"s{S_WDMA}", f"s{S_WM0}"]
     with open(os.path.join(here, "gemm_g4_regs.h"), "w") as f:
         f.write("// generated by gen_gemm_g4.py: the physical registers the K loop of gemm_g4 owns, and its LDS size\n#pragma once\n")
+        if M16:
+            f.write("#define G4_MFMA 16  // v_mfma_f32_16x16x32; without this line the loop is the 32x32x16 one\n")
+            f.write("#define G4_BLK 16                                // edge of an accumulator block = rows of a fragment\n")
+            f.write("#define G4_ACC_AT(i, j) (32 * (i) + 4 * (j))     // first of the 4 registers of block (i, j)\n")
+            f.write("#define G4_ACC_ROW(l) ((l) & 15)                 // lane l holds output row BLK j + this ...\n")
+            f.write("#define G4_ACC_COL(r, l) (4 * ((l) >> 4) + (r))  // ... and register r of the block output column BLK i + this\n")
+            f.write("#define G4_FRAG_CHUNK(ks, l) (4 * (ks) + ((l) >> 4))  // 16-byte chunk of fragment row G4_ACC_ROW(l) that lane l reads in k-step ks (of 2)\n")
         f.write(f"#define G4_PF {PF}\n#define G4_LDS_BYTES {163840 if (W3 or A3) else 131072}\n")
         f.write(f"#define G4_A_STRIDE {A_STRIDE}\n#define G4_W_BASE {W_BASE}\n#define G4_W_STRIDE {W_STRIDE}  // LDS map of the operand stages: A stage g at g * A_STRIDE, W stage h at W_BASE + h * W_STRIDE\n")
         for k in range(8):
```

New measurement: 1.574 (median of 6 runs). +1.4%, better.
